# CederGroupHub/sparse-lm

Hardware: AMD Instinct MI355X
Metric: fits/sec over 50-alpha Lasso path at n=100k p=5k (higher is better)
Workload: dtype f64

## Files before the change

sparse-lm_amd/csrc/engine.hip:

```cpp
#include "engine_internal.hpp"

static thread_local std::string g_last_error;

int fail(int code, const char* fmt, ...) {
  char buf[1024];
  va_list ap;
  va_start(ap, fmt);
  vsnprintf(buf, sizeof(buf), fmt, ap);
  va_end(ap);
  g_last_error = buf;
  return code;
}

RcclApi g_rccl;

int load_rccl() {
  if (g_rccl.lib) return SLM_OK;
  const char* names[] = {"librccl.so.1", "librccl.so", "/opt/rocm/lib/librccl.so.1"};
  void* lib = nullptr;
  for (const char* nm : names) {
    lib = dlopen(nm, RTLD_NOW | RTLD_GLOBAL);
    if (lib) break;
  }
  if (!lib) return fail(SLM_ERR_COMM, "cannot load librccl: %s", dlerror());
// ... 172 lines not shown
    return fail(SLM_ERR_NO_DEVICE, "no HIP device visible (%s); this engine has no CPU fallback",
                e == hipSuccess ? "device count is 0" : hipGetErrorString(e));
  if (device_id < 0 || device_id >= n)
    return fail(SLM_ERR_BAD_ARG, "device_id %d out of range [0, %d)", device_id, n);
  HIP_TRY(hipSetDevice(device_id));
  slm_engine* eng = new slm_engine();
  eng->device = device_id;
  e = hipGetDeviceProperties(&eng->prop, device_id);
  if (e != hipSuccess) {
    delete eng;
    return fail(SLM_ERR_HIP, "hipGetDeviceProperties: %s", hipGetErrorString(e));
  }
  if (strncmp(eng->prop.gcnArchName, "gfx950", 6) != 0 && !knobs().allow_any_arch) {
    std::string arch = eng->prop.gcnArchName;
    delete eng;
    return fail(SLM_ERR_NO_DEVICE, "device %d is %s; this library only carries gfx950 (MI355X) code",
                device_id, arch.c_str());
  }
  eng->cus = eng->prop.multiProcessorCount;
  e = hipStreamCreateWithFlags(&eng->stream, hipStreamNonBlocking);
  if (e != hipSuccess) {
    delete eng;
    return fail(SLM_ERR_HIP, "hipStreamCreate: %s", hipGetErrorString(e));
  }
  *out = eng;
  return SLM_OK;
}

extern "C" int slm_comm_destroy(slm_engine* eng);

extern "C" int slm_engine_destroy(slm_engine* eng) {
  if (!eng) return SLM_OK;
  (void)hipSetDevice(eng->device);
  if (eng->sharded()) (void)slm_comm_destroy(eng);
  if (eng->comm_ev) (void)hipEventDestroy(eng->comm_ev);
  if (eng->comm_stream) (void)hipStreamDestroy(eng->comm_stream);
  if (eng->stream) (void)hipStreamDestroy(eng->stream);
  {
    std::lock_guard<std::mutex> lk(g_pool.m);
    for (void* q : g_pool.book.retire_device(eng->device)) (void)hipFree(q);
  }
  delete eng;
  return SLM_OK;
}

extern "C" int slm_engine_synchronize(slm_engine* eng) {
  if (!eng) return fail(SLM_ERR_BAD_ARG, "engine is NULL");
  HIP_TRY(hipSetDevice(eng->device));
  HIP_TRY(hipStreamSynchronize(eng->stream));
  return SLM_OK;
}

extern "C" int slm_engine_device_info(slm_engine* eng, int64_t out[6], char* name_out, int name_len) {
  if (!eng || !out) return fail(SLM_ERR_BAD_ARG, "NULL argument");
  HIP_TRY(hipSetDevice(eng->device));
  size_t free_b = 0, total_b = 0;
  HIP_TRY(hipMemGetInfo(&free_b, &total_b));
  out[0] = eng->prop.multiProcessorCount;
  out[1] = (int64_t)eng->prop.maxSharedMemoryPerMultiProcessor;
  out[2] = (int64_t)total_b;
  out[3] = (int64_t)free_b;
  out[4] = eng->prop.warpSize;
  out[5] = eng->prop.clockRate;
  if (name_out && name_len > 0) {
    snprintf(name_out, (size_t)name_len, "%s (%s)", eng->prop.name, eng->prop.gcnArchName);
  }
  return SLM_OK;
}

static void dataset_free(slm_dataset* ds) {
  if (!ds) return;
  dfree(ds->X); dfree(ds->y); dfree(ds->rw); dfree(ds->yzero); dfree(ds->rw_lanes); dfree(ds->rvec);
  dfree(ds->order); dfree(ds->gid); dfree(ds->gstart);
  dfree(ds->partial); dfree(ds->loss_partial); dfree(ds->R);
  dfree(ds->g); dfree(ds->z); dfree(ds->beta); dfree(ds->zprev); dfree(ds->gprev);
  dfree(ds->u); dfree(ds->gscale); dfree(ds->a0); dfree(ds->b0); dfree(ds->d0);
  dfree(ds->lambda); dfree(ds->dctl);
  dfree(ds->pts); dfree(ds->betas_out); dfree(ds->gn_out); dfree(ds->infos);
  dfree(ds->ws_idx); dfree(ds->ws_pos); dfree(ds->ws_gs); dfree(ds->ws_gl);
  dfree(ds->ws_score); dfree(ds->ws_XW); dfree(ds->ws_part); dfree(ds->ws_G); dfree(ds->ws_Gx); dfree(ds->XT); dfree(ds->X32s); dfree(ds->ws_owner);
  dfree(ds->ws_nt); dfree(ds->stop_words); dfree(ds->sse_Z); dfree(ds->sse_part); dfree(ds->split_state);
  dfree(ds->cons_state); dfree(ds->cons_buf);
  dfree(ds->colnorm); dfree(ds->lt_dR); dfree(ds->lt_d2); dfree(ds->lt_part); dfree(ds->lt_cols); dfree(ds->lt_stamp);
  cov_pending_drop(ds);
  ds->cov.clear();
  ds->cov_all_hold.reset();
  ds->cov_all = nullptr;
  dfree(ds->cov_Z); dfree(ds->cov_fp); dfree(ds->cov_partial);
  mg_free(ds);
  if (ds->h_split) (void)hipHostFree(ds->h_split);
  if (ds->hctl) (void)hipHostFree(ds->hctl);
  if (ds->h_small_out) (void)hipHostFree(ds->h_small_out);
  if (ds->h_vec) (void)hipHostFree(ds->h_vec);
  if (ds->h_stage) (void)hipHostFree(ds->h_stage);
  if (ds->h_pts) (void)hipHostFree(ds->h_pts);
  for (auto& e : ds->ev)
    if (e) (void)hipEventDestroy(e);
  for (auto& e : ds->prof) (void)hipEventDestroy(e);
  delete ds;
}

int set_singleton_groups(slm_dataset* ds) {
  const int p = (int)ds->p;
  std::vector<int> ident(p), start(p + 1);
  std::iota(ident.begin(), ident.end(), 0);
  std::iota(start.begin(), start.end(), 0);
  dfree(ds->order); dfree(ds->gid); dfree(ds->gstart); dfree(ds->gscale);
  SLM_TRY(dalloc(&ds->order, p));
  SLM_TRY(dalloc(&ds->gid, p));
  SLM_TRY(dalloc(&ds->gstart, p + 1));
  SLM_TRY(dalloc(&ds->gscale, (size_t)ds->lane_cap * p));
  HIP_TRY(hipMemcpy(ds->order, ident.data(), sizeof(int) * p, hipMemcpyHostToDevice));
  HIP_TRY(hipMemcpy(ds->gid, ident.data(), sizeof(int) * p, hipMemcpyHostToDevice));
  HIP_TRY(hipMemcpy(ds->gstart, start.data(), sizeof(int) * (p + 1), hipMemcpyHostToDevice));
  ds->G = p;
  ds->singleton = 1;
  ds->team = 1;
  ds->max_group = 1;
  return SLM_OK;
}

static int dataset_alloc(const slm_host::Knobs& kn, slm_engine* eng, int64_t n, int64_t p, slm_dataset** out) {
  if (n <= 0 || p <= 0) return fail(SLM_ERR_BAD_ARG, "n and p must be positive (got %lld x %lld)",
                                    (long long)n, (long long)p);
  if (p > (int64_t)TAIL_THREADS * kMaxTailE)
    return fail(SLM_ERR_UNSUPPORTED, "p = %lld exceeds the supported %d columns", (long long)p,
                TAIL_THREADS * kMaxTailE);
  if (n > (int64_t)2000000000) return fail(SLM_ERR_UNSUPPORTED, "n too large");
  slm_dataset* ds = new slm_dataset();
  ds->eng = eng;
  ds->n = n;
  ds->p = p;
  ds->n_global = n;
  ds->ld = (p + 15) / 16 * 16;
  const int64_t ld = ds->ld;
  size_t partial_elems = 0, loss_elems = 0;
  for (int B = 1; B <= kMaxLanes; ++B) {
    const GradKernel* gk = pick_grad_kernel(kn, ld / 2, B);
    ds->gk[B - 1] = gk;
    if (!gk) continue;
    int occ = 2;
    if (gk->D >= 0) {
      hipError_t e = hipOccupancyMaxActiveBlocksPerMultiprocessor(&occ, (const void*)gk->fn, gk->W * 64, 0);
      if (e != hipSuccess || occ < 1) occ = 1;
    }
    int64_t nblk = (int64_t)eng->cus * occ;
    const int64_t steps = (n + gk->R - 1) / gk->R;
    nblk = std::max<int64_t>(1, std::min<int64_t>(nblk, steps));
    ds->nblk[B - 1] = (int)nblk;
    partial_elems = std::max(partial_elems, (size_t)nblk * B * (size_t)ld);
    loss_elems = std::max(loss_elems, (size_t)nblk * B);
  }
  if (!ds->gk[0]) {
    delete ds;
    return fail(SLM_ERR_UNSUPPORTED, "no gradient kernel covers p = %lld", (long long)p);
  }
  ds->sk = pick_split_kernel(kn, ld / 2);
  if (ds->sk) {
    ds->split_nblk = (int)std::max<int64_t>(1, std::min<int64_t>(eng->cus, n));
    partial_elems = std::max(partial_elems, (size_t)xtr_max_row_blocks(eng->cus, ld) * SPLIT_LANES * (size_t)ld);
    loss_elems = std::max(loss_elems, (size_t)ds->split_nblk * SPLIT_LANES * SPLIT_HALVES);
  }

  int rc = SLM_OK;
  auto A = [&](int r) { if (rc == SLM_OK) rc = r; };
  ds->lane_cap = (p <= SM_PMAX && (double)n * (double)ld <= 131072.0) ? kMaxCells : kMaxLanes;
// ... 492 lines not shown
```

sparse-lm_amd/csrc/engine_internal.hpp:

```cpp
#pragma once
#include <hip/hip_runtime.h>

#include <dlfcn.h>
#include <stdarg.h>
#include <stdio.h>
#include <stdlib.h>
#include <string.h>

#include <algorithm>
#include <cmath>
#include <chrono>
#include <condition_variable>
#include <memory>
#include <mutex>
#include <numeric>
#include <string>
#include <vector>

#include "../../include/slm_engine.h"
#include "host_logic.hpp"
#include "data_kernels.hpp"
#include "grad_kernel.hpp"
#include "tail_kernels.hpp"
#include "ws_kernels.hpp"
#include "split_kernels.hpp"
#include "sample_kernels.hpp"
#include "light_kernels.hpp"
#include "small_kernels.hpp"
#include "small_split_kernels.hpp"
#include "small_constrained_kernels.hpp"
#include "cov_kernels.hpp"
#include "mg_kernels.hpp"

using namespace slm;


int fail(int code, const char* fmt, ...);
slm_host::Knobs knobs();

#define HIP_TRY(expr)                                                                       \
  do {                                                                                      \
    hipError_t e__ = (expr);                                                                \
    if (e__ != hipSuccess)                                                                  \
      return fail(e__ == hipErrorOutOfMemory ? SLM_ERR_OOM : SLM_ERR_HIP, "%s failed: %s (%s:%d)", \
                  #expr, hipGetErrorString(e__), __FILE__, __LINE__);                       \
  } while (0)

#define SLM_TRY(expr)            \
  do {                           \
    int rc__ = (expr);           \
    if (rc__ != SLM_OK) return rc__; \
  } while (0)

typedef struct { char internal[SLM_COMM_ID_BYTES]; } rcclUniqueId_t;
typedef void* rcclComm_t;
struct RcclApi {
  void* lib = nullptr;
  int (*GetUniqueId)(rcclUniqueId_t*) = nullptr;
  int (*CommInitRank)(rcclComm_t*, int, rcclUniqueId_t, int) = nullptr;
  int (*AllReduce)(const void*, void*, size_t, int, int, rcclComm_t, hipStream_t) = nullptr;
  int (*CommDestroy)(rcclComm_t) = nullptr;
  int (*CommCount)(rcclComm_t, int*) = nullptr;
  int (*CommUserRank)(rcclComm_t, int*) = nullptr;
  const char* (*GetErrorString)(int) = nullptr;
};
extern RcclApi g_rccl;
static const int kNcclFloat64 = 8;
static const int kNcclSum = 0;
int load_rccl();

#define RCCL_TRY(expr)                                                                      \
  do {                                                                                      \
    int e__ = (expr);                                                                       \
    if (e__ != 0)                                                                           \
      return fail(SLM_ERR_COMM, "%s failed: %s", #expr,                                     \
                  g_rccl.GetErrorString ? g_rccl.GetErrorString(e__) : "rccl error");       \
  } while (0)

struct GradKernel {
  int W, C, R, B;
  int D;
  void (*fn)(GradArgs);
  const char* name;
};
struct SplitKernel {
  int W, C, B, D;
  void (*rowdot)(SplitArgs);
  void (*resid)(SplitArgs);
  const char* rowdot_name;
};
struct GradNames {
  const char* resid = nullptr;
  const char* ws_resid = nullptr;
  const char* product = nullptr;
  int cov_rows_ws = 0;
  int cov_row_blocks = 0;
};
static const int kMaxTailE = 64;
static const int64_t kMaxChunks = 64 * 8 * 10;
const SplitKernel* pick_split_kernel(const slm_host::Knobs& kn, int64_t p2);
int xtr_max_row_blocks(int cus, int64_t ld);
int launch_xtr(const slm_host::Knobs& kn, int cus, SplitArgs& a, hipStream_t s, bool sample = false, const char** name = nullptr);
const GradKernel* pick_grad_kernel(const slm_host::Knobs& kn, int64_t p2, int B);

struct LocalComm {
  static const int kMaxRanks = 8;
  int n_ranks = 0;
  int device = 0;
  size_t cap = 0;
  double* stage[kMaxRanks] = {};
  hipEvent_t ready[kMaxRanks][2] = {};
  hipEvent_t consumed[kMaxRanks][2] = {};
  std::mutex m;
  std::condition_variable cv;
  long arrived[2] = {0, 0};
  long round_of[kMaxRanks] = {};
  int refs = 0;
  double timeout_s = 30.0;
};

struct slm_engine {
  int device = 0;
  hipStream_t stream = nullptr;
  hipDeviceProp_t prop;
  int cus = 0;
  rcclComm_t comm = nullptr;
  LocalComm* local = nullptr;
  int rank = 0, n_ranks = 1;
  long collectives = 0;
  hipStream_t comm_stream = nullptr;
  hipEvent_t comm_ev = nullptr;
  bool sharded() const { return comm != nullptr || local != nullptr; }
};

int all_reduce_sum(slm_engine* eng, double* buf, size_t count, hipStream_t s = nullptr);

static const int kMaxLanes = SLM_MAX_LANES;
static const int kMaxCells = SLM_MAX_CELLS;

struct GlobalCtl {
  int32_t done;
  int32_t lanes_done;
  int32_t hard;
  int32_t done_local;
  int32_t diverged;
  int32_t pad_[3];
};
static const int kWsMaxBuilds = 24;
static const int kWsLateIters = 12;

static const int kSnapInfos = 64;
struct DevCtl {
  GlobalCtl g;
  MgCtl mg;
  LightCtl lt;
  WsCtl ws;
  PathCtl lane[SLM_MAX_CELLS];
  slm_point_info infos[kSnapInfos];
};
struct HostCtl {
  DevCtl c;
};

void pool_free(void* p);

constexpr size_t kSmallOutDoubles = 32768;

struct slm_dataset {
  slm_engine* eng = nullptr;
  int64_t n = 0, p = 0, ld = 0, n_global = 0;
  bool replicated = false;
  int lane_cap = SLM_MAX_LANES;
  double *X = nullptr, *y = nullptr, *rw = nullptr, *yzero = nullptr;
  double rw_max = 1.0;
  double* rw_lanes = nullptr;
  double* rvec = nullptr;
  int G = 0, singleton = 1, team = 1, max_group = 1;
  std::vector<int32_t> h_gid;
  int *order = nullptr, *gid = nullptr, *gstart = nullptr;
  WsCtl* ws_ctl = nullptr;
  int32_t *ws_idx = nullptr, *ws_pos = nullptr, *ws_gs = nullptr, *ws_gl = nullptr;
  double *ws_score = nullptr, *ws_XW = nullptr, *ws_part = nullptr, *ws_G = nullptr, *ws_Gx = nullptr;
  int32_t* ws_owner = nullptr;
  double* ws_nt = nullptr;
  double *sse_Z = nullptr, *sse_part = nullptr;
  size_t sse_cap = 0;
  PathCtl* h_stage = nullptr;
  double* h_vec = nullptr;
  slm_path_point* h_pts = nullptr;
  int64_t h_pts_cap = 0;
  struct CovBlocks {
    double *G = nullptr, *c = nullptr;
    ~CovBlocks() {
      if (G) pool_free(G);
      if (c) pool_free(c);
    }
  };
  struct CovEntry {
    std::shared_ptr<CovBlocks> hold;
    double *G = nullptr, *c = nullptr;
    double yy = 0.0, n_eff = 0.0, fp1 = 0.0, fp2 = 0.0;
  };
  std::vector<CovEntry> cov;
  struct CovPending;
  CovPending* cov_pend = nullptr;
  std::shared_ptr<CovBlocks> cov_all_hold;
  double* cov_all = nullptr;
  double* cov_Z = nullptr;
  double* cov_partial = nullptr;
  int cov_partial_sets = 0;
  size_t partial_elems = 0;
  double* cov_fp = nullptr;
  double* split_state = nullptr;
  double* h_split = nullptr;
  double* cons_state = nullptr;
  double* cons_buf = nullptr;
  size_t cons_buf_doubles = 0;
  double* stop_words = nullptr;
  double* XT = nullptr;
  bool XT_ready = false, XT_failed = false;
  float* X32s = nullptr;
  int64_t rows32 = 0, ld32 = 0;
  bool x32_failed = false, x32_lossy = false;
  double* colnorm = nullptr;
  bool colnorm_ready = false;
  double *lt_dR = nullptr, *lt_d2 = nullptr, *lt_part = nullptr;
  int32_t *lt_cols = nullptr, *lt_stamp = nullptr;
  struct MgEntry {
    float* G = nullptr;
    double fp1 = 0.0, fp2 = 0.0, n_eff = 0.0;
    bool own = false;
  };
  std::vector<MgEntry> mg;
  double* mg_vec = nullptr;
  double* mg_Z = nullptr;
  bool mg_failed = false;
  double mg_build_ms = 0.0;
  int ws_sets = 0;
  const GradKernel* gk[SLM_MAX_LANES] = {};
  int nblk[SLM_MAX_LANES] = {};
  const SplitKernel* sk = nullptr;
  int split_nblk = 0;
  double* R = nullptr;
  double *partial = nullptr, *loss_partial = nullptr;
  double *g = nullptr, *z = nullptr, *beta = nullptr, *zprev = nullptr, *gprev = nullptr;
  double *u = nullptr, *gscale = nullptr, *a0 = nullptr, *b0 = nullptr, *d0 = nullptr;
  double* lambda = nullptr;
  DevCtl* dctl = nullptr;
  PathCtl* ctl = nullptr;
  GlobalCtl* gctl = nullptr;
  HostCtl* hctl = nullptr;
  double* h_small_out = nullptr;
  hipEvent_t ev[2] = {nullptr, nullptr};
  int64_t cap_points = 0, cap_gn = 0;
  slm_path_point* pts = nullptr;
  double *betas_out = nullptr, *gn_out = nullptr;
  slm_point_info* infos = nullptr;
  std::vector<hipEvent_t> prof;
  double L = 0.0;
  int L_iters = 0;
  bool L_valid = false;
  bool sketch_valid = false;
  struct CarryLane {
    int64_t n_eff = 0;
    bool has_rw = false;
    double fp[2] = {0.0, 0.0};
    double loss = 0.0;
  };
  bool carry_valid = false;
  int carry_lanes = 0;
  bool ws_carry_valid = false;
  bool ws_carry_cov = false;
  int ws_carry_sets = 0;
  int ws_carry_set_of[SLM_MAX_LANES] = {};
  CarryLane carry_lane[SLM_MAX_LANES];
  std::vector<double> carry_out;
};

static inline bool row_sharded(const slm_dataset* ds) { return ds->eng->sharded() && !ds->replicated; }

hipError_t pool_malloc(void** out, size_t bytes);

template <typename T>
static int dalloc(T** out, size_t count) {
  *out = nullptr;
  if (count == 0) count = 1;
  HIP_TRY(pool_malloc((void**)out, count * sizeof(T)));
  return SLM_OK;
}
template <typename T>
static void dfree(T*& p) {
  if (p) pool_free(p);
  p = nullptr;
}

struct LaneSetup {
  int B = 1;
  const double* rw = nullptr;
  int64_t rw_stride = 0;
  double n_eff[SLM_MAX_CELLS] = {};
};
LaneSetup default_lanes(slm_dataset* ds, int B);
int enqueue_gradient(slm_dataset* ds, const LaneSetup& ls, const double* y, const int* done, hipEvent_t ev_start, hipEvent_t ev_stop,
                     int64_t n_rows = 0, const int* skip = nullptr, GradNames* names = nullptr);
int enqueue_gradient_split(const slm_host::Knobs& kn, slm_dataset* ds, const LaneSetup& ls, const double* y, const int* done, const PathCtl* ctl, const WsArgs* wa,
                           hipEvent_t ev_start, hipEvent_t ev_stop, int64_t n_rows = 0, bool unit_bracket = false, const int* skip = nullptr,
                           GradNames* names = nullptr);
bool split_usable(const slm_host::Knobs& kn, slm_dataset* ds);
int ensure_xt(const slm_host::Knobs& kn, slm_dataset* ds);
int ensure_x32s(slm_dataset* ds, int64_t n_rows, bool* usable);
void x32_drop(slm_dataset* ds);
int enqueue_sample_f32(slm_dataset* ds, int64_t n_rows, double n_eff, int n_lanes, const int* done, bool* queued);
int check_launch();
void launch_rowdot(const slm_host::Knobs& kn, slm_dataset* ds, const SplitKernel* sk, int nblk, int B, SplitArgs& a, hipStream_t s,
                  const char** name = nullptr);
int enqueue_gradient_cov(slm_dataset* ds, int B, const int* entry_of, const int* done, hipEvent_t ev_start, hipEvent_t ev_stop,
                         const PathCtl* ctl = nullptr, const WsArgs* wa = nullptr, GradNames* names = nullptr);
void launch_tail(const TailArgs& ta, hipStream_t s);
int64_t sketch_rows(int64_t n);
int power_iteration(const slm_host::Knobs& kn, slm_dataset* ds, const LaneSetup& ls_in, double* L_out , int iters, int64_t n_rows = 0);
int estimate_lipschitz(const slm_host::Knobs& kn, slm_dataset* ds, double* L_out, int iters);
int allow_big_lds(const void* fn, int device);
static const int kProfStride = 3;
static const int kPowerItersSolve = 2;
int cov_fingerprints(slm_dataset* ds, const double* const* w, int count, double* out );
int cov_find(const slm_dataset* ds, double fp1, double fp2, double n_eff);
void cov_pending_drop(slm_dataset* ds);
int set_singleton_groups(slm_dataset* ds);
static const int kMgEntries = 8;
bool mg_possible(const slm_host::Knobs& kn, const slm_dataset* ds);
int mg_ensure(const slm_host::Knobs& kn, slm_dataset* ds, const double* w, double n_eff, bool own, double fp1, double fp2, int* entry_out);
void mg_invalidate(slm_dataset* ds);
void mg_free(slm_dataset* ds);
int mg_enqueue_round(slm_dataset* ds, const TailArgs& ta, int n_lanes, int inner_iters, const int* done, int n_sets, const int* entry_of_set,
                     const int* set_of);
```

sparse-lm_amd/csrc/engine_path.hip:

```cpp
#include "engine_internal.hpp"
#include "ws_solve_kernels.hpp"

static int ws_policy(const slm_host::Knobs& kn, const slm_dataset* ds, uint32_t flags) {
  if (ds->max_group > WS_KCAP / 2 || ds->n < 4) return 0;
  if (kn.ws == 0 || (flags & SLM_FLAG_NO_WORKING_SET)) return 0;
  const bool big = (double)ds->n * (double)ds->ld >= 67108864.0;
  return (big || (flags & SLM_FLAG_WORKING_SET) || kn.ws == 1) ? 2 : 1;
}

static bool small_ok(const slm_host::Knobs& kn, const slm_dataset* ds, uint32_t flags) {
  if (!(flags & SLM_FLAG_ON_CHIP)) return false;
  if (flags & (SLM_FLAG_NO_RESTART | SLM_FLAG_PROFILE | SLM_FLAG_FISTA_ONLY | SLM_FLAG_WORKING_SET | SLM_FLAG_NO_WORKING_SET))
    return false;
  if (!kn.on_chip) return false;
  return ds->p <= SM_PMAX && (double)ds->n * (double)ds->ld <= 131072.0 && !row_sharded(ds);
}
static bool split_possible(const slm_dataset* ds) {
  return ds->sk != nullptr && (ds->sk->rowdot != nullptr || !ds->XT_failed);
}
static int max_lanes_for(const slm_host::Knobs& kn, const slm_dataset* ds, uint32_t flags) {
  if (small_ok(kn, ds, flags)) return ds->lane_cap;
  if ((ws_policy(kn, ds, flags) == 2 || (double)ds->n * (double)ds->ld >= 67108864.0) && split_possible(ds)) {
    if (ws_policy(kn, ds, flags) == 2 && !row_sharded(ds) && ds->sk->rowdot != nullptr && !ds->XT_failed)
      return kMaxLanes;
// ... 8 lines not shown
  if (want <= SPLIT_LANES || small_ok(kn, ds, flags)) return SLM_OK;
  HIP_TRY(hipSetDevice(ds->eng->device));
  SLM_TRY(ensure_xt(kn, ds));
  if (ds->XT == nullptr) *lanes_out = SPLIT_LANES;
  return SLM_OK;
}

static int solve_core(const slm_host::Knobs& kn, slm_dataset* ds, const slm_lane* lanes, int32_t n_lanes, const slm_solve_opts* opts,
                      slm_solve_stats* stats, bool shared_path, const slm_reweight* rules = nullptr, int32_t* rounds_out = nullptr);

static int solve_without_chip(const slm_host::Knobs& kn, slm_dataset* ds, const slm_lane* lanes, int32_t B, const slm_solve_opts& o, slm_solve_stats* stats,
                              bool shared_path) {
  slm_solve_opts again = o;
  again.flags &= ~SLM_FLAG_ON_CHIP;
  const int per_call = shared_path ? B : std::min<int>(B, max_lanes_for(kn, ds, again.flags));
  if (per_call >= B) return solve_core(kn, ds, lanes, B, &again, stats, shared_path);
  slm_solve_stats sum, part;
  memset(&sum, 0, sizeof(sum));
  for (int l0 = 0; l0 < B; l0 += per_call) {
    SLM_TRY(solve_core(kn, ds, lanes + l0, std::min(per_call, B - l0), &again, &part, false));
    sum.grad_launches += part.grad_launches;
    sum.wall_ms += part.wall_ms;
    sum.lipschitz_ms += part.lipschitz_ms;
    sum.ws_builds += part.ws_builds; sum.ws_appends += part.ws_appends; sum.ws_refined += part.ws_refined;
    sum.ws_misses += part.ws_misses; sum.ws_columns = std::max(sum.ws_columns, part.ws_columns);
    sum.ws_inner_iters += part.ws_inner_iters; sum.ws_direct_steps += part.ws_direct_steps;
  }
  if (stats) *stats = sum;
  return SLM_OK;
}

struct PathCall {
  explicit PathCall(const slm_host::Knobs& k) : kn(k) {}
  const slm_host::Knobs kn;
  slm_dataset* ds = nullptr;
  const slm_lane* lanes = nullptr;
  int B = 0;
  slm_solve_opts o;
  slm_solve_stats* stats = nullptr;
  bool shared_path = false;
  const slm_reweight* rules = nullptr;
  int32_t* rounds_out = nullptr;
  slm_engine* eng = nullptr;
  hipStream_t s = nullptr;
  int64_t n = 0, p = 0, ld = 0;
  int G = 0;
  bool big_x = false, split = false, want_cov = false, interleave = false, sharded = false, small = false, profile = false;
  int64_t total_points = 0;
  bool any_rw = false, any_gn = false, custom_scale = false;
  std::chrono::steady_clock::time_point t_begin;
  double tr[6] = {0, 0, 0, 0, 0, 0}, tr_rw = 0.0;
  double t_mark() const { return std::chrono::duration<double, std::milli>(std::chrono::steady_clock::now() - t_begin).count(); }
  LaneSetup ls;
  double wmax[SLM_MAX_CELLS];
  double rw_fp[SLM_MAX_CELLS][2];
  int cov_entry[SLM_MAX_CELLS];
  bool cov_on = false;
  double L[SLM_MAX_CELLS], L_factor[SLM_MAX_CELLS];
  double lipschitz_ms = 0.0;
  bool L_on_device = false;
  bool L_kept = false;
  bool carry = false, ws_carry = false;
  bool ws_begun = false;
  int ws_set_of[SLM_MAX_LANES], ws_set_lane[SLM_MAX_LANES], ws_n_sets = 0;
  PathCtl* h = nullptr;
  bool infos_in_snap = false;
  slm_point_info* d_infos = nullptr;
  TailArgs ta;
  bool use_ws = false, ws_late = false;
  WsArgs wa;
  const int* done_flag = nullptr;
  int ws_comm_rc = 0;
  bool mg_handover = false;
  bool fix_start = false;
  bool sample_f32 = false;
  int chunk = 0;
  int64_t max_total = 0, enq = 0, expected = 0, n_sample = 0, prof_off = 0;
  int64_t planned_end = 0;
  int slot = 0, final_slot = 0;
  bool pending[2] = {false, false};
  bool done = false, results_queued = false, results_final = false, deferred = false, trace3 = false;
  bool light_begun = false;
  const int* light_skip = nullptr;
  std::vector<char> prof_rec;
  bool mg_forced = false, mg_ok = false, mg_on = false;
  int mg_cap = 0, mg_inner = 20, mg_built = 0;
  double mg_build_ms = 0.0;
  int mg_entry_of_set[SLM_MAX_LANES];

  int run();
  int shape(const slm_solve_opts* opts);
  int stage_row_weights();
  int find_covariance();
  int kept_sketch();
  int seed_lipschitz();
  int stage_lanes();
  int enqueue_result_copies();
  int run_on_chip();
  int ws_setup(bool late);
  void ws_release();
  int prepare_working_set();
  int enqueue_pass_gradient(hipEvent_t e0, hipEvent_t e1);
  void enqueue_tail();
  void enqueue_refinement();
  void plan_queue();
  int mg_sets();
  bool mg_wanted(const DevCtl& c) const;
  int mg_consider(const DevCtl& c);
  void trace_pass(const DevCtl& now) const;
  bool light_eligible();
  int enqueue_light_attempt();
  int queue_chunk();
  int pass_loop();
  int finish();
  void report(const DevCtl& snap, int64_t passes);
};

static int solve_core(const slm_host::Knobs& kn, slm_dataset* ds, const slm_lane* lanes, int32_t n_lanes, const slm_solve_opts* opts,
                      slm_solve_stats* stats, bool shared_path, const slm_reweight* rules, int32_t* rounds_out) {
  if (!ds || !lanes) return fail(SLM_ERR_BAD_ARG, "NULL argument");
  HIP_TRY(hipSetDevice(ds->eng->device));
  std::unique_ptr<PathCall> c(new PathCall(kn));
  c->ds = ds; c->lanes = lanes; c->B = n_lanes; c->stats = stats; c->shared_path = shared_path; c->rules = rules; c->rounds_out = rounds_out;
  memset(&c->o, 0, sizeof(c->o));
  if (opts) c->o = *opts;
  memset(c->cov_entry, 0, sizeof(c->cov_entry));
  memset(c->rw_fp, 0, sizeof(c->rw_fp));
  memset(c->ws_set_of, 0, sizeof(c->ws_set_of));
  memset(c->ws_set_lane, 0, sizeof(c->ws_set_lane));
  memset(c->mg_entry_of_set, 0, sizeof(c->mg_entry_of_set));
  memset(&c->wa, 0, sizeof(c->wa));
  SLM_TRY(c->shape(opts));
  struct DrainOnExit {
    hipStream_t s;
    ~DrainOnExit() { (void)hipStreamSynchronize(s); }
  } drain_on_exit{c->s};
  return c->run();
}

int PathCall::run() {
  SLM_TRY(stage_row_weights());
  SLM_TRY(find_covariance());
  SLM_TRY(seed_lipschitz());
  SLM_TRY(stage_lanes());
  if (small) return run_on_chip();
  SLM_TRY(prepare_working_set());
  plan_queue();
  if (n_sample > 0 && !kn.sample_f64) SLM_TRY(ensure_x32s(ds, n_sample, &sample_f32));
  SLM_TRY(pass_loop());
  return finish();
}

int PathCall::shape(const slm_solve_opts* opts) {
  if (rules) {
    if (!rounds_out) return fail(SLM_ERR_BAD_ARG, "rounds_out is NULL");
    if (shared_path || !small_ok(kn, ds, opts ? opts->flags : 0u))
      return fail(SLM_ERR_UNSUPPORTED, "re-weighted rounds need a problem the on-chip solver takes (p <= %d, n * ld <= 131072)", SM_PMAX);
    for (int l = 0; l < B && l < SLM_MAX_CELLS; ++l) {
      const slm_reweight& r = rules[l];
      if (!(r.eps >= 0.0) || !(r.tol >= 0.0) || !std::isfinite(r.coef_scale) || !std::isfinite(r.numerator) || !std::isfinite(r.eps) ||
          r.n_coef < 0 || r.n_coef > ds->p || r.n_group < 0 || r.n_group > ds->G)
        return fail(SLM_ERR_BAD_ARG, "lane %d: bad re-weighting rule", l);
      if (r.group_scale)
        for (int g = 0; g < r.n_group; ++g)
          if (!(r.group_scale[g] >= 0.0) || !std::isfinite(r.group_scale[g]))
            return fail(SLM_ERR_BAD_ARG, "lane %d: group_scale[%d] is negative or not finite", l, g);
    }
  }
  {
    const int cap = small_ok(kn, ds, opts ? opts->flags : 0u) ? ds->lane_cap : kMaxLanes;
    if (B < 1 || B > cap) return fail(SLM_ERR_BAD_ARG, "n_lanes must be in [1, %d] (got %d)", cap, B);
  }
  big_x = (double)ds->n * (double)ds->ld >= 67108864.0;
  const bool wide = ds->sk != nullptr && ds->sk->rowdot == nullptr;
  const GradKernel* gk_B = B <= kMaxLanes ? ds->gk[B - 1] : nullptr;
  const bool two_pass_only = gk_B != nullptr && gk_B->D < 0;
  const bool want_split = (ws_policy(kn, ds, opts ? opts->flags : 0u) == 2 && (!wide || two_pass_only)) ? (big_x || !gk_B) : (big_x && !gk_B);
  want_cov = opts && (opts->flags & SLM_FLAG_COVARIANCE) && !ds->cov.empty() && !row_sharded(ds) && B <= kMaxLanes;
  split = (want_split || want_cov) && split_usable(kn, ds);
  interleave = shared_path && ds->singleton && ws_policy(kn, ds, opts ? opts->flags : 0u) == 2 &&
                          kn.interleave;
  if (!split && !gk_B && !small_ok(kn, ds, opts ? opts->flags : 0u))
    return fail(SLM_ERR_UNSUPPORTED, "no %d-lane gradient kernel covers p = %lld", B, (long long)ds->p);
  if (B > SPLIT_LANES && !small_ok(kn, ds, opts ? opts->flags : 0u) && (!split || row_sharded(ds) || ws_policy(kn, ds, opts ? opts->flags : 0u) != 2))
    return fail(SLM_ERR_UNSUPPORTED, "%d lanes: more than %d need a working-set solve on the split pass of an unsharded dataset", B, SPLIT_LANES);
  if (split && B > ROWDOT_LANES) SLM_TRY(ensure_xt(kn, ds));
  for (int l = 0; l < B; ++l) {
    const slm_lane& ln = lanes[l];
    if (!ln.points || !ln.betas_out) return fail(SLM_ERR_BAD_ARG, "lane %d: NULL points or betas_out", l);
    if (ln.n_points <= 0) return fail(SLM_ERR_BAD_ARG, "lane %d: n_points must be positive", l);
    for (int k = 0; k < ln.n_points; ++k) {
      const slm_path_point& q = ln.points[k];
      if (!(q.sa >= 0.0) || !(q.sb >= 0.0) || !(q.sd >= 0.0) || !std::isfinite(q.sa + q.sb + q.sd))
        return fail(SLM_ERR_BAD_ARG, "path point %d has a negative or non-finite scale", k);
      if (!std::isfinite(q.extrap) || std::fabs(q.extrap) > 1e3)
        return fail(SLM_ERR_BAD_ARG, "path point %d has an unreasonable extrapolation factor", k);
    }
    total_points += ln.n_points;
    any_rw = any_rw || ln.row_weight != nullptr;
    any_gn = any_gn || ln.group_norms_out != nullptr;
  }
  eng = ds->eng;
  sharded = row_sharded(ds);
  HIP_TRY(hipSetDevice(eng->device));
  s = eng->stream;
  t_begin = std::chrono::steady_clock::now();
  p = ds->p; ld = ds->ld; n = ds->n;
  G = ds->G;
  if (!(o.tol > 0.0)) o.tol = 1e-8;
  if (o.max_iter <= 0) o.max_iter = 10000;
  profile = (o.flags & SLM_FLAG_PROFILE) != 0;

  return SLM_OK;
}

int PathCall::stage_row_weights() {
  ls = default_lanes(ds, B);
  for (int l = 0; l < kMaxCells; ++l) wmax[l] = ds->rw ? ds->rw_max : 1.0;
  if (any_rw) {
    if (!ds->rw_lanes) SLM_TRY(dalloc(&ds->rw_lanes, (size_t)ds->lane_cap * n));
    for (int l = 0; l < B; ++l) {
      double* dst = ds->rw_lanes + (size_t)l * n;
      if (lanes[l].row_weight) {
        const double* w = lanes[l].row_weight;
        int same = -1;
        for (int m = 0; m < l && same < 0; ++m)
          if (lanes[m].row_weight == w) same = m;
        if (same >= 0) {
          wmax[l] = wmax[same];
          rw_fp[l][0] = rw_fp[same][0];
// ... 485 lines not shown
    ds->ws_sets = n_sets;
  }
  return ensure_xt(kn, ds);
}

static int ws_bind(const slm_host::Knobs& kn, slm_dataset* ds, const LaneSetup& ls, const int* set_of, const int* set_lane, int n_sets,
                   int nblk, bool sharded, WsArgs& wa, hipStream_t s) {
  const int B = ls.B;
  wa.ws = ds->ws_ctl;
  wa.idx = ds->ws_idx; wa.pos = ds->ws_pos; wa.gs = ds->ws_gs; wa.gl = ds->ws_gl;
  wa.score = ds->ws_score; wa.XW = ds->ws_XW; wa.part = ds->ws_part; wa.Gm = ds->ws_G;
  wa.nt = ds->ws_nt;
  if (sharded && !ds->ws_Gx) SLM_TRY(dalloc(&ds->ws_Gx, (size_t)ds->ws_sets * WS_KCAP * WS_KCAP + STOP_WORDS));
  wa.Gx = sharded ? ds->ws_Gx : nullptr;
  wa.X = ds->X; wa.XT = ds->XT; wa.n = ds->n; wa.ld = ds->ld;
  wa.rw = ls.rw; wa.rw_stride = ls.rw_stride;
  for (int l = 0; l < kMaxLanes; ++l) {
    wa.set_of[l] = l < B ? set_of[l] : 0;
    wa.set_lane[l] = l < n_sets ? set_lane[l] : 0;
    const int rep = wa.set_lane[l];
    wa.inv_n[l] = 1.0 / (ls.n_eff[rep] > 0 ? ls.n_eff[rep] : (double)ds->n_global);
  }
  wa.n_sets = n_sets;
  wa.nblk = nblk;
  wa.owner = nullptr;
  if (ls.rw != nullptr && !sharded && kn.gram_owner && nblk <= 512) {
    if (!ds->ws_owner) SLM_TRY(dalloc(&ds->ws_owner, (size_t)kMaxLanes * 512));
    hipLaunchKernelGGL(ws_block_owner_kernel, dim3((unsigned)nblk), dim3(256), 0, s, ls.rw, ls.rw_stride, wa, ds->ws_owner);
    wa.owner = ds->ws_owner;
  }
  return SLM_OK;
}

int PathCall::ws_setup(bool late) {
  const int n_sets = ws_n_sets;
  const WsBlocks wb = ws_row_blocks(ds, ls.rw != nullptr && !sharded && n_sets > 1, n_sets);
  SLM_TRY(ws_alloc(kn, ds, n_sets, wb.most, sharded));
  if (late) HIP_TRY(hipMemsetAsync(ds->ws_ctl, 0, sizeof(WsCtl), s));
  if (ws_carry && !late) hipLaunchKernelGGL(ws_ctl_carry_kernel, dim3(1), dim3(256), 0, s, ds->ws_ctl, kWsMaxBuilds);
  else if (late || !ws_begun) hipLaunchKernelGGL(ws_ctl_init_kernel, dim3(1), dim3(64), 0, s, ds->ws_ctl, kWsMaxBuilds);
  SLM_TRY(ws_bind(kn, ds, ls, ws_set_of, ws_set_lane, n_sets, wb.nblk, sharded, wa, s));
  wa.theta = kn.ws_theta;
  wa.lookahead = slm_host::kWsLookahead;
  wa.append_max = kn.ws_append;
  wa.k_init = kn.ws_kinit > 0 ? kn.ws_kinit : (ds->singleton ? (shared_path ? 112 : 256) : 384);
  wa.bb_steps = kn.ws_bb;
  wa.one_solver = kn.ws_one_solver;
  wa.hard_call = kn.hard_callwide;
  wa.power_iters = slm_host::kWsPowerIters;
  wa.miss_factor = kn.ws_miss_factor;
  wa.miss_div = kn.ws_miss_div;
  wa.fill = kn.ws_fill > 0.0 ? kn.ws_fill : ((ds->singleton && shared_path) ? 0.75 : 0.5);
  return SLM_OK;
}

void PathCall::ws_release() {
  ds->ws_carry_valid = false;
  dfree(ds->ws_idx); dfree(ds->ws_pos); dfree(ds->ws_gs); dfree(ds->ws_gl);
  dfree(ds->ws_score); dfree(ds->ws_XW); dfree(ds->ws_part); dfree(ds->ws_G); dfree(ds->ws_Gx); dfree(ds->ws_nt);
  ds->ws_sets = 0;
  (void)hipGetLastError();
}

int PathCall::prepare_working_set() {
  {
    const int pol = ws_policy(kn, ds, o.flags);
    use_ws = pol == 2;
    ws_late = pol == 1 && !sharded;
  }
  if (sharded && !ds->stop_words) SLM_TRY(dalloc(&ds->stop_words, STOP_WORDS));
  if (use_ws) {
    const int rc = ws_setup(false);
    if (rc == SLM_ERR_OOM && !split && !sharded) {
      ws_release();
      use_ws = false;
    } else if (rc != SLM_OK) {
      return rc;
    }
  }
  done_flag = &ds->gctl->done;
  return SLM_OK;
}

int PathCall::enqueue_pass_gradient(hipEvent_t e0, hipEvent_t e1) {
  if (cov_on) return enqueue_gradient_cov(ds, B, cov_entry, done_flag, e0, e1, ds->ctl, use_ws ? &wa : nullptr);
  if (split) return enqueue_gradient_split(kn, ds, ls, ds->y, done_flag, ds->ctl, &wa, e0, e1, 0, (o.flags & SLM_FLAG_PROFILE_UNIT) != 0, light_skip);
  return enqueue_gradient(ds, ls, ds->y, done_flag, e0, e1, 0, light_skip);
}

void PathCall::enqueue_tail() {
  launch_tail(ta, s);
  if (shared_path && !interleave) hipLaunchKernelGGL(steal_kernel, dim3(1), dim3(256), 0, s, ta);
  if (shared_path && interleave && mg_handover) hipLaunchKernelGGL(tail_handover_kernel, dim3(1), dim3(64), 0, s, ta);
  else if (shared_path && interleave && use_ws && !ws_late && !sharded && planned_end > 0 && kn.lag_handover)
    hipLaunchKernelGGL(lag_handover_kernel, dim3(1), dim3(64), 0, s, ta, &ds->ws_ctl->builds, &ds->ws_ctl->stale, (int)(planned_end - enq - 1));
  if (sharded) {
    if (use_ws && wa.Gx) {
      hipLaunchKernelGGL(stop_pack_kernel, dim3(1), dim3(64), 0, s, ta.gdone, ds->ctl, B,
                         wa.Gx + (size_t)wa.n_sets * WS_KCAP * WS_KCAP);
    } else {
      hipLaunchKernelGGL(stop_pack_kernel, dim3(1), dim3(64), 0, s, ta.gdone, ds->ctl, B, ds->stop_words);
      if (ws_comm_rc == 0) ws_comm_rc = all_reduce_sum(eng, ds->stop_words, STOP_WORDS);
      hipLaunchKernelGGL(stop_apply_kernel, dim3(1), dim3(64), 0, s, ta.gdone, ds->stop_words);
    }
  }
}

struct WsNames {
  const char* k[8];
  int n = 0;
  void add(const char* name) { if (n < 8) k[n++] = name; }
};
static void ws_enqueue_build(slm_dataset* ds, const WsArgs& wa, const CovSets* cs, bool xty, const int* done, int n_lanes, hipStream_t s,
                             WsNames* names = nullptr) {
  const int64_t n = ds->n;
  if (cs) {
    hipLaunchKernelGGL(ws_gram_cov_kernel, dim3(WS_TILES * WS_TILES, (unsigned)wa.n_sets), dim3(256), 0, s, wa, *cs);
    if (names) names->add("ws_gram_cov_kernel");
    return;
  }
  hipLaunchKernelGGL(ws_gather_kernel, dim3((unsigned)std::min<int64_t>((n + 31) / 32, 1024), WS_KCAP / 32), dim3(256), 0, s, wa);
  if (names) names->add("ws_gather_kernel");
  if (xty) {
    XtyArgs xa;
    xa.ws = wa.ws; xa.idx = wa.idx; xa.XW = wa.XW; xa.y = ds->y; xa.part = wa.part; xa.g = ds->g; xa.gprev = ds->gprev; xa.z = ds->z;
    xa.ctl = ds->ctl; xa.done = done; xa.n = n; xa.ld = ds->ld; xa.inv_n = 1.0 / (double)ds->n_global; xa.n_lanes = n_lanes;
    xa.nblk = (int)std::max<int64_t>(1, std::min<int64_t>(2 * ds->eng->cus, n / 64));
    hipLaunchKernelGGL(ws_xty_partial_kernel, dim3((unsigned)xa.nblk), dim3(512), 0, s, xa);
    hipLaunchKernelGGL(ws_xty_apply_kernel, dim3(WS_KCAP / 128), dim3(512), 0, s, xa);
    if (names) { names->add("ws_xty_partial_kernel"); names->add("ws_xty_apply_kernel"); }
  }
  hipLaunchKernelGGL(ws_gram_kernel, dim3((unsigned)wa.nblk, (unsigned)wa.n_sets, 1), dim3(WS_GRAM_THREADS), 0, s,
                     wa);
  if (wa.Gx)
    (void)hipMemsetAsync(wa.Gx, 0, sizeof(double) * (size_t)wa.n_sets * WS_KCAP * WS_KCAP, s);
  hipLaunchKernelGGL(ws_gram_reduce_kernel, dim3(WS_TILES * WS_TILES, (unsigned)wa.n_sets), dim3(256),
                     0, s, wa);
  if (names) { names->add("ws_gram_kernel"); names->add("ws_gram_reduce_kernel"); }
}

static void ws_enqueue_solvers(const slm_dataset* ds, const TailArgs& ta, const WsArgs& wa, int B, hipStream_t s, WsNames* names = nullptr) {
  if (wa.one_solver && wa.nt) {
  } else if (ds->singleton) {
    hipLaunchKernelGGL((ws_solve_kernel<false, 0>), dim3(B), dim3(WS_THREADS), 0, s, ta, wa);
    if (names) names->add("ws_solve_kernel<false,0>");
  } else {
    hipLaunchKernelGGL((ws_solve_kernel<true, 0>), dim3(B), dim3(WS_THREADS), 0, s, ta, wa);
    if (names) names->add("ws_solve_kernel<true,0>");
  }
  if (wa.nt) {
    if (ds->singleton) hipLaunchKernelGGL((ws_solve_kernel<false, 1>), dim3(B), dim3(WS_THREADS), 0, s, ta, wa);
    else hipLaunchKernelGGL((ws_solve_kernel<true, 1>), dim3(B), dim3(WS_THREADS), 0, s, ta, wa);
    if (names) names->add(ds->singleton ? "ws_solve_kernel<false,1>" : "ws_solve_kernel<true,1>");
  }
}

void PathCall::enqueue_refinement() {
  if (use_ws) {
    {
      const int bs = ds->singleton ? 256 : 64;
      const int64_t items = ds->singleton ? p : 16 * (int64_t)G;
      hipLaunchKernelGGL(ws_score_kernel, dim3((unsigned)((items + bs - 1) / bs)), dim3(bs), 0, s, ta, wa);
      hipLaunchKernelGGL(ws_select_kernel, dim3(1), dim3(WS_THREADS), 0, s, ta, wa);
    }
    if (cov_on) {
      CovSets cs;
      for (int st = 0; st < kMaxLanes; ++st) cs.G[st] = st < wa.n_sets ? ds->cov[(size_t)cov_entry[wa.set_lane[st]]].G : nullptr;
      ws_enqueue_build(ds, wa, &cs, false, done_flag, B, s);
    } else {
      ws_enqueue_build(ds, wa, nullptr, fix_start, done_flag, B, s);
    }
    if (wa.Gx) {
      const size_t gram_words = (size_t)wa.n_sets * WS_KCAP * WS_KCAP;
      if (ws_comm_rc == 0) ws_comm_rc = all_reduce_sum(eng, wa.Gx, gram_words + STOP_WORDS);
      hipLaunchKernelGGL(ws_publish_kernel, dim3(WS_PUBLISH_BLOCKS, (unsigned)wa.n_sets), dim3(256), 0, s, wa);
      hipLaunchKernelGGL(stop_apply_kernel, dim3(1), dim3(64), 0, s, ta.gdone, wa.Gx + gram_words);
    }
    ws_enqueue_solvers(ds, ta, wa, B, s);
  }
}

void PathCall::plan_queue() {
  chunk = o.check_every;
  if (chunk <= 0) {
    const double est_us = std::max(12.0, (double)n * (double)ld * 8.0 / 5.0e6);
    chunk = est_us > 150.0 ? 2 : 4;
  }
  if (use_ws) chunk = std::min(chunk, 8);
  int max_points = 0;
  for (int l = 0; l < B; ++l) max_points = std::max(max_points, (int)lanes[l].n_points);
  if (shared_path) max_points = (int)total_points;
  max_total = (int64_t)max_points * o.max_iter;

  tr[2] = t_mark();
  if (use_ws && !ws_late && o.check_every <= 0) {
    int64_t most = 0;
    for (int l = 0; l < B; ++l) {
      int64_t mine = lanes[l].n_points;
      if (shared_path && interleave) mine = slm_host::interleaved_points(slm_host::LaneWalk{h[l].pt_lo, h[l].n_points, h[l].stride, h[l].tail_pt});
      most = std::max<int64_t>(most, mine);
    }
    expected = 1 + most;
    planned_end = expected;
  }
  {
    bool cold = true;
    for (int l = 0; l < B; ++l) cold = cold && lanes[l].beta0 == nullptr;
    if (cold && shared_path && use_ws && !ws_late && !sharded && !cov_on && split && !any_rw && !ds->rw &&
        !custom_scale && expected > 0 && o.max_iter >= 4 && !(o.flags & SLM_FLAG_FISTA_ONLY) && kn.sample_start) {
      const int64_t least = kn.sample_min_rows;
      if (n >= least) n_sample = n / kn.sample_div;
    }
  }
  mg_forced = kn.mg == 2;
  mg_cap = slm_host::model_gram_cap(ld, 3.0e9, kMgEntries);
  mg_ok = use_ws && split && (big_x || mg_forced) && !sharded && !cov_on && !(o.flags & SLM_FLAG_NO_MODEL_GRAM) &&
                     (size_t)ds->lane_cap >= (size_t)kMaxLanes && ws_n_sets <= mg_cap && mg_possible(kn, ds);
  if (mg_ok && mg_forced) expected = 0;
  if (mg_ok && !mg_forced && !ds->mg.empty()) {
    bool all = ws_n_sets > 0;
    for (int st = 0; st < ws_n_sets && all; ++st) {
      const int l = ws_set_lane[st];
      all = lanes[l].row_weight == nullptr;
      const double ne = ls.n_eff[l] > 0 ? ls.n_eff[l] : (double)ds->n_global;
      bool have = false;
      for (const auto& e : ds->mg) have = have || (e.own && e.n_eff == ne);
      all = all && have;
    }
    if (all) wa.keep_full = 1;
  }
  prof_off = n_sample > 0 ? 1 : 0;
  trace3 = kn.trace == 3;
  if (trace3 && kn.trace_poll && expected > 0) expected = n_sample > 0 ? 2 : 1;
}

int PathCall::mg_sets() {
  const double* wdev[SLM_MAX_LANES];
  double fp[2 * SLM_MAX_LANES] = {};
  int n_fp = 0, fp_at[SLM_MAX_LANES];
  for (int st = 0; st < ws_n_sets; ++st) {
    const int l = ws_set_lane[st];
    fp_at[st] = -1;
    if (lanes[l].row_weight != nullptr) {
      fp_at[st] = n_fp;
      wdev[n_fp++] = ls.rw + (int64_t)l * ls.rw_stride;
    }
  }
  if (n_fp > 0) SLM_TRY(cov_fingerprints(ds, wdev, n_fp, fp));
  int missing = 0;
  for (int pass = 0; pass < 2; ++pass) {
    if (pass == 1 && (int)ds->mg.size() + missing > mg_cap) mg_invalidate(ds);
    if (pass == 1) mg_built += missing;
    for (int st = 0; st < ws_n_sets; ++st) {
      const int l = ws_set_lane[st];
      const bool own = lanes[l].row_weight == nullptr;
      const double ne = ls.n_eff[l] > 0 ? ls.n_eff[l] : (double)ds->n_global;
      const double f1 = own ? 0.0 : fp[2 * fp_at[st]], f2 = own ? 0.0 : fp[2 * fp_at[st] + 1];
      if (pass == 0) {
        bool have = false;
        for (const auto& e : ds->mg) have = have || (e.n_eff == ne && (own ? e.own : (!e.own && e.fp1 == f1 && e.fp2 == f2)));
        missing += have ? 0 : 1;
      } else {
        SLM_TRY(mg_ensure(kn, ds, own ? nullptr : ls.rw + (int64_t)l * ls.rw_stride, ne, own, f1, f2, &mg_entry_of_set[st]));
      }
    }
  }
  return SLM_OK;
}

bool PathCall::mg_wanted(const DevCtl& c) const {
  if (mg_forced) return true;
  return c.ws.outgrown > 0 || c.ws.overflows > 0 || c.ws.disabled != 0;
}

int PathCall::mg_consider(const DevCtl& c) {
  if (!mg_ok || mg_on || !mg_wanted(c)) return SLM_OK;
  const auto t0 = std::chrono::steady_clock::now();
  const int rc = mg_sets();
  if (rc == SLM_OK) {
    mg_on = true;
    mg_handover = kn.handover;
    wa.keep_full = 1;
    if (mg_built > 0) mg_build_ms += std::chrono::duration<double, std::milli>(std::chrono::steady_clock::now() - t0).count();
  } else if (rc != SLM_ERR_OOM) {
    return rc;
  }
  return SLM_OK;
}

void PathCall::trace_pass(const DevCtl& now) const {
  if (!trace3) return;
  fprintf(stderr, "[slm] pass %lld at %.3f ms: K %d builds %d appends %d misses %d stale %d refined %d | mg on %d rounds %d inner %d most %d rej %d | light %d of %d (last: %d columns, why %d, D %.3g) | lanes (point.iter/flags):",
          (long long)enq, t_mark(), now.ws.Kreal, now.ws.builds, now.ws.appends, now.ws.misses, now.ws.stale, now.ws.refined, (int)mg_on,
          now.mg.rounds, now.mg.inner_iters, now.mg.most_iters, now.mg.rejected, now.lt.used, now.lt.attempts, now.lt.n_cols, now.lt.why, now.lt.D[0]);
  for (int l = 0; l < B; ++l)
    fprintf(stderr, " %d.%d%s%s%s", now.lane[l].point, now.lane[l].iter, now.lane[l].done ? "d" : "", now.lane[l].zsup ? "w" : "",
            l < SLM_MAX_LANES && now.mg.lane[l].active ? "m" : "");
  fprintf(stderr, " | lt id %d ok %d | lanes (rejects/epoch/slack):", now.lt.id, now.lt.ok);
  for (int l = 0; l < B && l < SLM_MAX_LANES; ++l) fprintf(stderr, " %d/%d/%.3g", now.lane[l].rejects, now.lt.epoch[l], now.lt.slack[l]);
  fprintf(stderr, "\n");
}

bool PathCall::light_eligible() {
  if (!kn.light_pass || !shared_path || !use_ws || ws_late || cov_on || sharded || mg_on) return false;
  if (any_rw || ds->rw || custom_scale || B > kMaxLanes || !(expected > 0 && enq >= expected)) return false;
  return ds->XT != nullptr && ds->XT_ready && ds->colnorm != nullptr && ds->colnorm_ready;
}

int PathCall::enqueue_light_attempt() {
  const int nblk = (int)std::max<int64_t>(std::max<int64_t>(1, std::min<int64_t>(eng->cus, n)), (n + 959) / 960);
  if (!ds->lt_dR) SLM_TRY(dalloc(&ds->lt_dR, (size_t)n * LT_LANES));
  if (!ds->lt_d2) SLM_TRY(dalloc(&ds->lt_d2, (size_t)nblk * (LT_LANES + kMaxLanes)));
  if (!ds->lt_part) SLM_TRY(dalloc(&ds->lt_part, (size_t)nblk * LT_CAP * LT_LANES));
  if (!ds->lt_cols) SLM_TRY(dalloc(&ds->lt_cols, (size_t)LT_CAP));
  if (!ds->lt_stamp) SLM_TRY(dalloc(&ds->lt_stamp, (size_t)ld));
  if (!light_begun) {
    HIP_TRY(hipMemsetAsync(ds->lt_stamp, 0, sizeof(int32_t) * (size_t)ld, s));
    light_begun = true;
  }
  LightArgs la;
  memset(&la, 0, sizeof(la));
  la.lt = &ds->dctl->lt; la.ctl = ds->ctl; la.done = done_flag; la.pts = ds->pts; la.ws = wa.ws; la.idx = wa.idx; la.pos = wa.pos;
  la.XW = wa.XW; la.XT = ds->XT; la.Gm = wa.Gm; la.y = ds->y; la.colnorm = ds->colnorm;
  la.z = ds->z; la.zprev = ds->zprev; la.gprev = ds->gprev; la.a0 = ds->a0; la.b0 = ds->b0; la.g = ds->g;
  la.loss_partial = ds->lt_d2 + (size_t)nblk * LT_LANES; la.dR = ds->lt_dR; la.d2_part = ds->lt_d2; la.cols = ds->lt_cols; la.stamp = ds->lt_stamp; la.part = ds->lt_part;
  la.n = n; la.ld = ld; la.rows_base = n / nblk; la.rows_rem = n % nblk;
  la.p = (int)p; la.n_lanes = B; la.slots = SPLIT_LANES * ((B + SPLIT_LANES - 1) / SPLIT_LANES); la.nblk = nblk;
  la.inv_n = 1.0 / (double)ds->n_global;
  la.order = ds->order; la.gstart = ds->gstart; la.G = G; la.singleton = ds->singleton;
  hipLaunchKernelGGL(light_prepare_kernel, dim3(1), dim3(1024), 0, s, la);
  hipLaunchKernelGGL(light_resid_kernel, dim3((unsigned)nblk), dim3(LT_WAVES * 64), 0, s, la);
  hipLaunchKernelGGL(light_select_kernel, dim3(1), dim3(1024), 0, s, la);
  const size_t lds = sizeof(double) * (size_t)(la.rows_base + 1) * LT_LANES;
  hipLaunchKernelGGL(light_coldot_kernel, dim3((unsigned)nblk), dim3(256), lds, s, la);
  hipLaunchKernelGGL(light_assemble_kernel, dim3(LT_LANES), dim3(1024), 0, s, la);
  return SLM_OK;
}

int PathCall::queue_chunk() {
  const int this_chunk = mg_on ? 1 : (expected <= 0 ? chunk : (enq < expected ? (int)std::min<int64_t>(64, expected - enq) : 1));
  for (int i = 0; i < this_chunk; ++i) {
    hipEvent_t e0 = nullptr, e1 = nullptr;
    const bool light = light_eligible();
    if (profile && !light && enq >= prof_off && (enq - prof_off) % kProfStride == 0) {
      const int64_t slot_id = (enq - prof_off) / kProfStride;
      while ((int64_t)ds->prof.size() < 2 * (slot_id + 1)) {
        hipEvent_t ev;
        HIP_TRY(hipEventCreate(&ev));
        ds->prof.push_back(ev);
      }
      e0 = ds->prof[2 * slot_id];
      e1 = ds->prof[2 * slot_id + 1];
      if ((int64_t)prof_rec.size() <= slot_id) prof_rec.resize((size_t)slot_id + 1, 0);
      prof_rec[(size_t)slot_id] = 1;
    }
    if (light) SLM_TRY(enqueue_light_attempt());
    light_skip = light ? &ds->dctl->lt.ok : nullptr;
    ta.light = light ? 1 : 0;
    const bool sample_pass = n_sample > 0 && enq == 0;
    if (sample_pass) {
      LaneSetup part = ls;
      for (int l = 0; l < kMaxLanes; ++l) part.n_eff[l] = (double)ds->n_global * (double)n_sample / (double)n;
      bool on_image = false;
      if (sample_f32) SLM_TRY(enqueue_sample_f32(ds, n_sample, part.n_eff[0], B, done_flag, &on_image));
      if (!on_image) SLM_TRY(enqueue_gradient_split(kn, ds, part, ds->y, done_flag, ds->ctl, &wa, nullptr, nullptr, n_sample));
      TailArgs first = ta;
      first.provisional = 1;
      launch_tail(first, s);
    } else {
      if (!(carry && enq == 0)) SLM_TRY(enqueue_pass_gradient(e0, e1));
      enqueue_tail();
    }
    fix_start = sample_pass;
    ++enq;
    deferred = (expected > 0 && enq >= expected && enq < expected + 4 && !sharded) || mg_on;
    if (!deferred) enqueue_refinement();
    fix_start = false;
  }
  SLM_TRY(check_launch());
  if (ws_comm_rc != 0) return ws_comm_rc;
  HIP_TRY(hipMemcpyAsync(&ds->hctl[slot].c, ds->dctl, sizeof(DevCtl), hipMemcpyDeviceToHost, s));
  return SLM_OK;
}

int PathCall::pass_loop() {
  while (!done) {
    SLM_TRY(queue_chunk());
    const bool at_end = mg_on || (expected > 0 && enq >= expected && (enq < expected + 4 || (trace3 && kn.trace_poll)));
    HIP_TRY(hipEventRecord(ds->ev[slot], s));
    if (expected > 0 && enq == expected && !results_queued) {
      SLM_TRY(enqueue_result_copies());
      results_queued = true;
    }
    pending[slot] = true;
    const int other = slot ^ 1;
    if (at_end) {
      if (pending[other]) HIP_TRY(hipEventSynchronize(ds->ev[other]));
      const auto t_spin = std::chrono::steady_clock::now();
      for (;;) {
        const hipError_t q = hipEventQuery(ds->ev[slot]);
        if (q == hipSuccess) break;
        if (q != hipErrorNotReady) HIP_TRY(q);
        if (std::chrono::steady_clock::now() - t_spin > std::chrono::milliseconds(20)) {
          HIP_TRY(hipEventSynchronize(ds->ev[slot]));
          break;
        }
      }
      pending[slot] = pending[other] = false;
      if (ds->hctl[slot].c.g.done) {
        done = true;
        final_slot = slot;
        results_final = results_queued && enq == expected;
      } else {
        const DevCtl& now = ds->hctl[slot].c;
        trace_pass(now);
        SLM_TRY(mg_consider(now));
        if (deferred) {
          bool ws_serves = !(mg_on && now.ws.stale != 0 && wa.keep_full != 0);
          for (int l = 0; l < B && !ws_serves; ++l) ws_serves = !now.lane[l].done && !now.lane[l].idle && now.lane[l].zsup != 0;
          if (ws_serves) enqueue_refinement();
          deferred = false;
        }
        if (mg_on) {
          if (now.mg.rounds > 0) mg_inner = now.mg.most_iters >= mg_inner ? std::min(96, 2 * mg_inner) : std::max(6, std::min(96, (int)now.mg.most_iters + 2));
          SLM_TRY(mg_enqueue_round(ds, ta, B, mg_inner, done_flag, ws_n_sets, mg_entry_of_set, ws_set_of));
        }
      }
    } else if (pending[other]) {
      HIP_TRY(hipEventSynchronize(ds->ev[other]));
      pending[other] = false;
      if (ds->hctl[other].c.g.done) {
        done = true;
        final_slot = other;
      }
      if (!done) SLM_TRY(mg_consider(ds->hctl[other].c));
      if (!done && ws_late && ds->hctl[other].c.g.hard >= kWsLateIters) {
        const int rc = ws_setup(true);
        ws_late = false;
        if (rc == SLM_OK) {
          use_ws = true;
          chunk = std::min(chunk, 8);
        } else if (rc == SLM_ERR_OOM) {
          ws_release();
        } else {
          return rc;
        }
      }
    }
    slot = other;
    if (!done && enq >= max_total + 2 * (int64_t)chunk) {
      HIP_TRY(hipStreamSynchronize(s));
      return fail(SLM_ERR_HIP, "internal error: path state machine did not terminate");
    }
  }
  return SLM_OK;
}

int PathCall::finish() {
  if (!results_final) SLM_TRY(enqueue_result_copies());
  HIP_TRY(hipStreamSynchronize(s));
  tr[3] = t_mark();
  const DevCtl& snap = ds->hctl[final_slot].c;
  if (sharded && snap.g.diverged)
    return fail(SLM_ERR_COMM, "row-sharded solve aborted: the ranks' solver states differ (different arguments on "
                "different ranks, or an all-reduce that is not bit-identical on every rank)");
  const PathCtl* fin = snap.lane;
  if (infos_in_snap) {
    int64_t at = 0;
    for (int l = 0; l < B; ++l) {
      if (lanes[l].infos) memcpy(lanes[l].infos, snap.infos + at, sizeof(slm_point_info) * (size_t)lanes[l].n_points);
      at += lanes[l].n_points;
    }
  }
  int64_t passes = 0;
  bool nonfinite = false;
  for (int l = 0; l < B; ++l) {
    passes = std::max<int64_t>(passes, fin[l].total_iter);
    nonfinite = nonfinite || fin[l].nonfinite;
  }
  if (stats) {
    stats->grad_launches = passes - (carry ? 1 : 0) - prof_off - snap.lt.used;
    stats->light_passes = snap.lt.used;
    stats->light_columns = snap.lt.cols_total;
    stats->grad_ms_total = 0.0;
    stats->grad_timed = 0;
    if (profile) {
      double tot = 0.0;
      int64_t cnt = 0;
      for (int64_t k = 0; k * kProfStride < passes - prof_off && 2 * k + 1 < (int64_t)ds->prof.size(); ++k) {
        if (k >= (int64_t)prof_rec.size() || !prof_rec[(size_t)k]) continue;
        float ms = 0.f;
        if (hipEventElapsedTime(&ms, ds->prof[2 * k], ds->prof[2 * k + 1]) == hipSuccess) {
          tot += ms;
          ++cnt;
        }
      }
      stats->grad_ms_total = tot;
      stats->grad_timed = cnt;
    }
    stats->lipschitz_ms = lipschitz_ms;
    stats->ws_builds = stats->ws_appends = stats->ws_refined = stats->ws_misses = stats->ws_columns = 0;
    stats->ws_inner_iters = stats->ws_direct_steps = 0;
    stats->mg_rounds = snap.mg.rounds;
    stats->mg_inner_iters = snap.mg.inner_iters;
    stats->mg_rejected = snap.mg.rejected;
    stats->mg_build_ms = mg_build_ms;
    if (use_ws) {
      const WsCtl& wc = snap.ws;
      stats->ws_builds = wc.builds;
      stats->ws_appends = wc.appends;
      stats->ws_refined = wc.refined;
      stats->ws_misses = wc.misses;
      stats->ws_columns = wc.Kreal;
      stats->ws_inner_iters = wc.inner_iters;
      stats->ws_direct_steps = wc.newton_steps;
      if (kn.trace == 2) {
        fprintf(stderr, "[slm] working set: %d model-solver iterations over %d refinements, %d direct steps (%d refused, %d of them not positive definite), K = %d, lambda_max bound of the first Gram %.4g (seed L %.4g)\n",
                wc.inner_iters, wc.refined, wc.newton_steps, wc.newton_fails, wc.newton_nopd, wc.K, wc.Lw[0], fin[0].L);
        fprintf(stderr, "[slm] model solver, lane 0, ms over the solve: set-up %.3f, lambda_max of a new Gram %.3f, start value %.3f, "
                "iteration %.3f, acceptance + write-back %.3f\n", wc.solve_ticks[0] * 1e-5, wc.solve_ticks[1] * 1e-5,
                wc.solve_ticks[2] * 1e-5, wc.solve_ticks[3] * 1e-5, wc.solve_ticks[4] * 1e-5);
        fprintf(stderr, "[slm] model solves by iterations:");
        for (int i = 0; i < 32; ++i)
          if (wc.iters_hist[i]) fprintf(stderr, " %d:%d", i, wc.iters_hist[i]);
        fprintf(stderr, "\n");
        fprintf(stderr, "[slm] model solver, ms per lane over the solve:");
        for (int l = 0; l < B; ++l) fprintf(stderr, " %.3f", wc.lane_ticks[l] * 1e-5);
        fprintf(stderr, "\n");
        if (wc.newton_factors) {
          fprintf(stderr, "[slm] direct steps: accepted at t = 1: %d, 1/2: %d, 1/4: %d, first sign change: %d; %d factorisations, %.0f unknowns on average\n",
                  wc.newton_trial[0], wc.newton_trial[1], wc.newton_trial[2], wc.newton_trial[3], wc.newton_factors,
                  (double)wc.newton_unknowns / wc.newton_factors);
          fprintf(stderr, "[slm] direct steps without a usable segment: t = 0: %d, slope <= 0: %d, curvature <= 0: %d; no decrease on it: %d\n",
                  wc.newton_ref[0], wc.newton_ref[1], wc.newton_ref[2], wc.newton_ref[3]);
          int worst = 0;
          double worst_ms = -1.0;
          for (int l = 0; l < B; ++l) {
            double t = 0.0;
            for (int k = 0; k < 6; ++k) t += wc.nt_ticks[l][k] * 1e-5;
            if (t > worst_ms) {
              worst_ms = t;
              worst = l;
            }
          }
          const unsigned long long* tk = wc.nt_ticks[worst];
// ... 40 lines not shown
  return SLM_OK;
}

extern "C" int slm_solve_lanes(slm_dataset* ds, const slm_lane* lanes, int32_t n_lanes,
                               const slm_solve_opts* opts, slm_solve_stats* stats) {
  return solve_core(knobs(), ds, lanes, n_lanes, opts, stats, false);
}

extern "C" int slm_solve_lanes_reweighted(slm_dataset* ds, const slm_lane* lanes, const slm_reweight* rules, int32_t n_lanes,
                                          const slm_solve_opts* opts, slm_solve_stats* stats, int32_t* rounds_out) {
  if (!rules) return fail(SLM_ERR_BAD_ARG, "rules is NULL");
  return solve_core(knobs(), ds, lanes, n_lanes, opts, stats, false, rules, rounds_out);
}

static int auto_lanes(const slm_host::Knobs& kn, const slm_dataset* ds, int32_t n_points, uint32_t fl) {
  const int cap = max_lanes_for(kn, ds, fl);
  const bool big = ws_policy(kn, ds, fl) == 2 && (double)ds->n * (double)ds->ld >= 67108864.0 && !small_ok(kn, ds, fl);
  const bool interleaved = ds->singleton && kn.interleave;
  int B = slm_host::auto_path_lanes(n_points, cap, big, !interleaved);
  if (kn.auto_lanes > 0) B = std::max(1, std::min<int>(std::min(kn.auto_lanes, cap), n_points));
  return B;
}
extern "C" int slm_dataset_path_lanes(slm_dataset* ds, int32_t n_points, uint32_t flags, int32_t* lanes_out) {
  if (!ds || !lanes_out) return fail(SLM_ERR_BAD_ARG, "NULL argument");
  if (n_points <= 0) return fail(SLM_ERR_BAD_ARG, "n_points must be positive");
  *lanes_out = auto_lanes(knobs(), ds, n_points, flags);
  return SLM_OK;
}

extern "C" int slm_solve_path_lanes(slm_dataset* ds, const slm_penalty* pen, const slm_path_point* points,
                                    int32_t n_points, int32_t n_lanes, const slm_solve_opts* opts,
                                    const double* beta0, double* betas_out, double* group_norms_out,
                                    slm_point_info* infos, slm_solve_stats* stats) {
  if (!ds || !points || !betas_out) return fail(SLM_ERR_BAD_ARG, "NULL argument");
  if (n_points <= 0) return fail(SLM_ERR_BAD_ARG, "n_points must be positive");
  const uint32_t fl = opts ? opts->flags : 0u;
  const slm_host::Knobs kn = knobs();
  int B;
  if (n_lanes == 0) {
    B = auto_lanes(kn, ds, n_points, fl);
  } else {
    B = std::max(1, std::min<int>(std::min<int>(n_lanes, kMaxLanes), n_points));
    B = std::min(B, max_lanes_for(kn, ds, fl));
  }
  SLM_TRY(lanes_with_copy(kn, ds, fl, B, &B));
  slm_lane lanes[SLM_MAX_LANES];
  memset(lanes, 0, sizeof(lanes));
  int64_t lo = 0;
  for (int l = 0; l < B; ++l) {
    const int64_t hi = (int64_t)n_points * (l + 1) / B;
    lanes[l].pen = pen;
    lanes[l].points = points + lo;
    lanes[l].n_points = (int32_t)(hi - lo);
    lanes[l].beta0 = (l == 0) ? beta0 : nullptr;
    lanes[l].betas_out = betas_out + lo * ds->p;
    lanes[l].group_norms_out = group_norms_out ? group_norms_out + lo * ds->G : nullptr;
    lanes[l].infos = infos ? infos + lo : nullptr;
    lo = hi;
  }
  return solve_core(kn, ds, lanes, B, opts, stats, B > 1);
}

extern "C" int slm_solve_path(slm_dataset* ds, const slm_penalty* pen, const slm_path_point* points,
                              int32_t n_points, const slm_solve_opts* opts, const double* beta0,
                              double* betas_out, double* group_norms_out, slm_point_info* infos,
                              slm_solve_stats* stats) {
  if (!ds || !points || !betas_out) return fail(SLM_ERR_BAD_ARG, "NULL argument");
  slm_lane lane;
  memset(&lane, 0, sizeof(lane));
  lane.pen = pen;
  lane.points = points;
  lane.n_points = n_points;
  lane.beta0 = beta0;
  lane.betas_out = betas_out;
  lane.group_norms_out = group_norms_out;
  lane.infos = infos;
  return slm_solve_lanes(ds, &lane, 1, opts, stats);
}

extern "C" int slm_working_set_lanes(slm_dataset* ds, const slm_ws_lanes_opts* o, double* G_out, double* loss_out, int32_t* set_of_out,
                                     int32_t* n_sets_out, double* gram_out, double* xw_out, double* xty_out, char* kernels_out,
                                     int32_t kernels_len) {
  if (!ds || !o || !o->Z || !o->cols || !o->k_end || !G_out) return fail(SLM_ERR_BAD_ARG, "NULL argument");
  const int route = o->route, B = o->n_lanes, nb = o->n_builds;
  const bool gather_x = (o->flags & SLM_WSL_GATHER_X) != 0, xty = (o->flags & SLM_WSL_XTY) != 0;
  if (route != 1 && route != 2) return fail(SLM_ERR_BAD_ARG, "route must be 1 (split pass) or 2 (covariance), got %d", route);
  if (B < 1 || B > kMaxLanes) return fail(SLM_ERR_BAD_ARG, "between 1 and %d lanes, got %d", kMaxLanes, B);
  if (o->flags & ~(SLM_WSL_GATHER_X | SLM_WSL_XTY)) return fail(SLM_ERR_BAD_ARG, "unknown flags %#x", o->flags);
  if (xty != (xty_out != nullptr)) return fail(SLM_ERR_BAD_ARG, "xty_out goes with SLM_WSL_XTY");
  if (row_sharded(ds)) return fail(SLM_ERR_UNSUPPORTED, "slm_working_set_lanes: row-sharded datasets");
  if (B > ds->lane_cap) return fail(SLM_ERR_UNSUPPORTED, "%d lanes: the dataset holds %d", B, ds->lane_cap);
  const int64_t n = ds->n, p = ds->p, ld = ds->ld;
  if (nb < 1) return fail(SLM_ERR_BAD_ARG, "at least one build");
  for (int b = 0; b < nb; ++b)
    if (o->k_end[b] <= (b > 0 ? o->k_end[b - 1] : 0) || o->k_end[b] > WS_KCAP)
      return fail(SLM_ERR_BAD_ARG, "k_end must increase from above 0 to at most %d (build %d: %d)", WS_KCAP, b, o->k_end[b]);
  const int kreal = o->k_end[nb - 1];
  const int K = std::max(16, (kreal + 15) & ~15);
  std::vector<int32_t> pos((size_t)ld, -1);
  for (int k = 0; k < kreal; ++k) {
    const int32_t j = o->cols[k];
    if (j < 0 || j >= p) return fail(SLM_ERR_BAD_ARG, "cols[%d] = %d outside [0, %lld)", k, j, (long long)p);
    if (pos[(size_t)j] >= 0) return fail(SLM_ERR_BAD_ARG, "cols[%d] = %d repeats cols[%d]", k, j, pos[(size_t)j]);
    pos[(size_t)j] = k;
  }
  std::vector<int32_t> zzero((size_t)B, 1);
  for (int l = 0; l < B; ++l)
    for (int64_t j = 0; j < p; ++j) {
      const double v = o->Z[(size_t)l * p + j];
      if (!std::isfinite(v)) return fail(SLM_ERR_BAD_ARG, "Z contains a non-finite value");
      if (v != 0.0) {
        zzero[(size_t)l] = 0;
        if (o->on_ws && o->on_ws[l] && pos[(size_t)j] < 0)
          return fail(SLM_ERR_BAD_ARG, "lane %d is marked on the working set but Z[%d][%lld] != 0 is outside it", l, l, (long long)j);
      }
    }
  if (o->row_weights)
    for (int64_t k = 0; k < (int64_t)B * n; ++k)
      if (!(o->row_weights[k] >= 0.0) || !std::isfinite(o->row_weights[k]))
        return fail(SLM_ERR_BAD_ARG, "row_weights[%lld] is negative or not finite", (long long)k);
  if (o->n_eff)
    for (int l = 0; l < B; ++l)
      if (!(o->n_eff[l] > 0.0) || !std::isfinite(o->n_eff[l])) return fail(SLM_ERR_BAD_ARG, "n_eff[%d] must be positive and finite", l);
  if (route == 2) {
    if (o->row_weights || o->n_eff) return fail(SLM_ERR_UNSUPPORTED, "route 2 takes its rows from the covariance entries: no row_weights or n_eff");
    if (gather_x || xty || xw_out) return fail(SLM_ERR_UNSUPPORTED, "route 2 gathers no columns: no XW, no X_W^T y");
    if (ds->cov.empty()) return fail(SLM_ERR_UNSUPPORTED, "route 2: the dataset has no covariance entries");
    if (!o->cov_index) return fail(SLM_ERR_BAD_ARG, "route 2 needs cov_index");
    for (int l = 0; l < B; ++l)
      if (o->cov_index[l] < 0 || o->cov_index[l] >= (int32_t)ds->cov.size())
        return fail(SLM_ERR_BAD_ARG, "cov_index[%d] = %d: the dataset has %d entries", l, o->cov_index[l], (int)ds->cov.size());
  }
  const slm_host::Knobs kn = knobs();
  HIP_TRY(hipSetDevice(ds->eng->device));
  hipStream_t s = ds->eng->stream;
  if (route == 1) {
    if (!ds->sk) return fail(SLM_ERR_UNSUPPORTED, "route 1: no split pass for p = %lld", (long long)p);
    SLM_TRY(ensure_xt(kn, ds));
    if (!split_usable(kn, ds) || (B > SPLIT_LANES && !(ds->XT && ds->XT_ready)))
      return fail(SLM_ERR_UNSUPPORTED, "route 1: no residual kernel for %d lanes at p = %lld without the column-major copy", B, (long long)p);
    if (!gather_x && !(ds->XT && ds->XT_ready)) return fail(SLM_ERR_UNSUPPORTED, "no column-major copy of X to gather from");
  }
  auto put = [&](void* dst, const void* src, size_t bytes) -> int {
    HIP_TRY(hipMemcpyAsync(dst, src, bytes, hipMemcpyHostToDevice, s));
    HIP_TRY(hipStreamSynchronize(s));
    return SLM_OK;
  };
  auto get = [&](void* dst, const void* src, size_t bytes) -> int {
    HIP_TRY(hipMemcpyAsync(dst, src, bytes, hipMemcpyDeviceToHost, s));
    HIP_TRY(hipStreamSynchronize(s));
    return SLM_OK;
  };
  LaneSetup ls = default_lanes(ds, B);
  if (o->row_weights) {
    if (!ds->rw_lanes) SLM_TRY(dalloc(&ds->rw_lanes, (size_t)ds->lane_cap * n));
    SLM_TRY(put(ds->rw_lanes, o->row_weights, sizeof(double) * (size_t)B * n));
    ls.rw = ds->rw_lanes;
    ls.rw_stride = n;
  }
  if (o->n_eff)
    for (int l = 0; l < B; ++l) ls.n_eff[l] = o->n_eff[l];
  int set_of[kMaxLanes], set_lane[kMaxLanes], n_sets = 0;
  for (int l = 0; l < B; ++l) {
    int found = -1;
    for (int m = 0; m < l && found < 0; ++m) {
      const bool same = route == 2 ? o->cov_index[m] == o->cov_index[l]
                                   : ls.n_eff[m] == ls.n_eff[l] &&
                                         (!o->row_weights || memcmp(o->row_weights + (size_t)m * n, o->row_weights + (size_t)l * n,
                                                                    sizeof(double) * (size_t)n) == 0);
// ... 6 lines not shown
    set_of[l] = found;
  }
  const WsBlocks wb = ws_row_blocks(ds, ls.rw != nullptr && n_sets > 1, n_sets);
  SLM_TRY(ws_alloc(kn, ds, n_sets, wb.most, false));
  WsArgs wa;
  memset(&wa, 0, sizeof(wa));
  SLM_TRY(ws_bind(kn, ds, ls, set_of, set_lane, n_sets, wb.nblk, false, wa, s));
  if (gather_x) wa.XT = nullptr;
  std::string names;
  auto named = [&](const char* k) {
    if (!names.empty()) names += ';';
    names += k;
  };
  if (wa.owner) named("ws_block_owner_kernel");
  CovSets cs;
  memset(&cs, 0, sizeof(cs));
  if (route == 2)
    for (int st = 0; st < n_sets; ++st) cs.G[st] = ds->cov[(size_t)o->cov_index[set_lane[st]]].G;
  HIP_TRY(hipMemsetAsync(ds->ws_XW, 0xff, sizeof(double) * (size_t)n * WS_KCAP, s));
  HIP_TRY(hipMemsetAsync(ds->ws_G, 0xff, sizeof(double) * (size_t)n_sets * WS_KCAP * WS_KCAP, s));
  HIP_TRY(hipMemsetAsync(ds->g, 0xff, sizeof(double) * (size_t)(ld + 16) * B, s));
  HIP_TRY(hipMemsetAsync(&ds->gctl->done, 0, sizeof(int32_t), s));
  WsCtl* h = new WsCtl;
  std::unique_ptr<WsCtl> h_hold(h);
  memset(h, 0, sizeof(WsCtl));
  h->request = 1;
  h->max_builds = kWsMaxBuilds;
  for (int l = 0; l < SLM_MAX_LANES; ++l) h->last_point[l] = -1;
  std::vector<int32_t> h_idx(WS_KCAP), h_gs(WS_KCAP), h_gl(WS_KCAP, 1), h_pos((size_t)ld, -1);
  for (int k = 0; k < WS_KCAP; ++k) h_gs[(size_t)k] = k;
  for (int b = 0; b < nb; ++b) {
    const int k_old = b > 0 ? o->k_end[b - 1] : 0, kr = o->k_end[b];
    for (int k = 0; k < WS_KCAP; ++k) h_idx[(size_t)k] = k < kr ? o->cols[k] : -1;
    for (int k = k_old; k < kr; ++k) h_pos[(size_t)o->cols[k]] = k;
    h->Kreal = kr;
    h->K = std::max(16, (kr + 15) & ~15);
    h->k_new = k_old;
    h->building = 1;
    h->valid = 0;
    h->stale = 0;
    h->counter = 0;
    if (b > 0) h->appends += 1;
    else h->builds += 1;
    SLM_TRY(put(ds->ws_idx, h_idx.data(), sizeof(int32_t) * WS_KCAP));
    SLM_TRY(put(ds->ws_gs, h_gs.data(), sizeof(int32_t) * WS_KCAP));
    SLM_TRY(put(ds->ws_gl, h_gl.data(), sizeof(int32_t) * WS_KCAP));
    SLM_TRY(put(ds->ws_pos, h_pos.data(), sizeof(int32_t) * (size_t)ld));
    SLM_TRY(put(ds->ws_ctl, h, sizeof(WsCtl)));
    WsNames wn;
    ws_enqueue_build(ds, wa, route == 2 ? &cs : nullptr, xty, &ds->gctl->done, B, s, &wn);
    for (int u = 0; u < wn.n; ++u) named(wn.k[u]);
    SLM_TRY(check_launch());
    SLM_TRY(get(h, ds->ws_ctl, sizeof(WsCtl)));
    if (h->valid != 1 || h->building != 0 || h->counter != 0)
      return fail(SLM_ERR_HIP, "build %d: the Gram was not published (valid %d, building %d, counter %d)", b, h->valid, h->building,
                  h->counter);
  }
  if (gram_out)
    for (int st = 0; st < n_sets; ++st)
      HIP_TRY(hipMemcpy2DAsync(gram_out + (size_t)st * K * K, sizeof(double) * K, ds->ws_G + (size_t)st * WS_KCAP * WS_KCAP,
                               sizeof(double) * WS_KCAP, sizeof(double) * K, K, hipMemcpyDeviceToHost, s));
  if (xw_out)
    HIP_TRY(hipMemcpy2DAsync(xw_out, sizeof(double) * K, ds->ws_XW, sizeof(double) * WS_KCAP, sizeof(double) * K, n,
                             hipMemcpyDeviceToHost, s));
  if (xty) {
    std::vector<double> g0((size_t)ld + 16);
    SLM_TRY(get(g0.data(), ds->g, sizeof(double) * (size_t)(ld + 16)));
    for (int k = 0; k < kreal; ++k) xty_out[k] = g0[(size_t)o->cols[k]];
    xty_out[kreal] = g0[(size_t)ld];
  }
  HIP_TRY(hipStreamSynchronize(s));
  std::vector<PathCtl> hc((size_t)B);
  memset(hc.data(), 0, sizeof(PathCtl) * (size_t)B);
  for (int l = 0; l < B; ++l) {
    hc[(size_t)l].zsup = (o->on_ws && o->on_ws[l]) ? 1 : 0;
    hc[(size_t)l].zzero = zzero[(size_t)l];
    hc[(size_t)l].tail_pt = -1;
  }
  SLM_TRY(put(ds->ctl, hc.data(), sizeof(PathCtl) * (size_t)B));
  const int slots = SPLIT_LANES * ((B + SPLIT_LANES - 1) / SPLIT_LANES);
  HIP_TRY(hipMemsetAsync(ds->z, 0, sizeof(double) * (size_t)slots * ld, s));
  HIP_TRY(hipMemcpy2DAsync(ds->z, sizeof(double) * ld, o->Z, sizeof(double) * p, sizeof(double) * p, B, hipMemcpyHostToDevice, s));
  GradNames gn;
  if (route == 1) {
    SLM_TRY(enqueue_gradient_split(kn, ds, ls, ds->y, nullptr, ds->ctl, &wa, nullptr, nullptr, 0, false, nullptr, &gn));
  } else {
    if (!ds->cov_Z) SLM_TRY(dalloc(&ds->cov_Z, (size_t)ld * SPLIT_RSTRIDE * SPLIT_HALVES));
    SLM_TRY(enqueue_gradient_cov(ds, B, o->cov_index, nullptr, nullptr, nullptr, ds->ctl, &wa, &gn));
  }
  SLM_TRY(check_launch());
  HIP_TRY(hipStreamSynchronize(s));
  const size_t lane_bytes = sizeof(double) * (size_t)(ld + 16);
  HIP_TRY(hipMemcpy2D(G_out, sizeof(double) * p, ds->g, lane_bytes, sizeof(double) * p, B, hipMemcpyDeviceToHost));
  if (loss_out) HIP_TRY(hipMemcpy2D(loss_out, sizeof(double), ds->g + ld, lane_bytes, sizeof(double), B, hipMemcpyDeviceToHost));
  if (set_of_out)
    for (int l = 0; l < B; ++l) set_of_out[l] = set_of[l];
  if (n_sets_out) *n_sets_out = n_sets;
  if (route == 1) {
    if (gn.resid) named(gn.resid);
    if (gn.ws_resid) named(gn.ws_resid);
    if (gn.product) named(gn.product);
  } else if (gn.product) {
    bool listed = gn.cov_rows_ws > 0 && (int64_t)gn.cov_rows_ws * gn.cov_row_blocks >= K;
    for (int l = 0; l < B; ++l) listed = listed && o->on_ws && o->on_ws[l];
    named(gn.product);
    if (listed) names += "+listed";
  }
  if (kernels_out && kernels_len > 0) snprintf(kernels_out, (size_t)kernels_len, "%s", names.c_str());
  return SLM_OK;
}

extern "C" int slm_working_set_model_solve(slm_dataset* ds, const slm_ws_model_opts* o, slm_ws_model_out* out) {
  if (!ds || !o || !out) return fail(SLM_ERR_BAD_ARG, "NULL argument");
  if (!o->cols || !o->gram || !o->zprev || !o->gprev || !o->z || !o->a0 || !o->b0 || !o->d0 || !o->points || !o->tol || !o->mode)
    return fail(SLM_ERR_BAD_ARG, "NULL input");
  if (!out->z || !out->beta || !out->served || !out->mu || !out->zsup || !out->t || !out->have_base || !out->zzero ||
      !out->want_full || !out->repeats || !out->hard_lane || !out->last_point || !out->Lw || !out->counters)
    return fail(SLM_ERR_BAD_ARG, "NULL output");
  const uint32_t known = SLM_WMS_DIRECT | SLM_WMS_HARD | SLM_WMS_INVALID | SLM_WMS_BUILDING | SLM_WMS_DISABLED | SLM_WMS_STALE |
                         SLM_WMS_NONFINITE;
  if (o->flags & ~known) return fail(SLM_ERR_BAD_ARG, "unknown flags %#x", o->flags);
  const int B = o->n_lanes, kreal = o->kreal, n_sets = o->n_sets;
  if (B < 1 || B > kMaxLanes) return fail(SLM_ERR_BAD_ARG, "between 1 and %d lanes, got %d", kMaxLanes, B);
  if (kreal < 1 || kreal > WS_KCAP) return fail(SLM_ERR_BAD_ARG, "between 1 and %d columns, got %d", WS_KCAP, kreal);
  if (n_sets < 1 || n_sets > B) return fail(SLM_ERR_BAD_ARG, "between 1 and n_lanes Grams, got %d", n_sets);
  if (row_sharded(ds)) return fail(SLM_ERR_UNSUPPORTED, "slm_working_set_model_solve: row-sharded datasets");
  if (B > ds->lane_cap) return fail(SLM_ERR_UNSUPPORTED, "%d lanes: the dataset holds %d", B, ds->lane_cap);
  const int64_t p = ds->p, ld = ds->ld;
  const int G = ds->singleton ? (int)p : ds->G;
  const int K = std::max(16, (kreal + 15) & ~15);
  const bool loose = (o->flags & SLM_WMS_NONFINITE) != 0;
  std::vector<int32_t> h_pos((size_t)ld, -1), h_idx(WS_KCAP, -1), h_gs(WS_KCAP), h_gl(WS_KCAP, 1);
  for (int k = 0; k < WS_KCAP; ++k) h_gs[(size_t)k] = k;
  for (int k = 0; k < kreal; ++k) {
    const int32_t j = o->cols[k];
    if (j < 0 || j >= p) return fail(SLM_ERR_BAD_ARG, "cols[%d] = %d outside [0, %lld)", k, j, (long long)p);
    if (h_pos[(size_t)j] >= 0) return fail(SLM_ERR_BAD_ARG, "cols[%d] = %d repeats cols[%d]", k, j, h_pos[(size_t)j]);
    h_pos[(size_t)j] = k;
    h_idx[(size_t)k] = j;
  }
  if (!ds->singleton) {
    std::vector<int> size((size_t)G, 0);
    for (int64_t j = 0; j < p; ++j) size[(size_t)ds->h_gid[(size_t)j]] += 1;
    for (int k = 0; k < kreal;) {
      const int g = ds->h_gid[(size_t)o->cols[k]], len = size[(size_t)g];
      if (k + len > kreal) return fail(SLM_ERR_BAD_ARG, "cols: group %d (%d members) is split at position %d", g, len, k);
      for (int m = 0; m < len; ++m) {
        if (ds->h_gid[(size_t)o->cols[k + m]] != g) return fail(SLM_ERR_BAD_ARG, "cols: group %d (%d members) is split at position %d", g, len, k + m);
        h_gs[(size_t)(k + m)] = k;
        h_gl[(size_t)(k + m)] = len;
      }
      k += len;
    }
  }
  auto finite = [](const double* v, size_t count) {
    for (size_t e = 0; e < count; ++e)
      if (!std::isfinite(v[e])) return false;
    return true;
  };
  if (!loose && (!finite(o->gram, (size_t)n_sets * K * K) || !finite(o->gprev, (size_t)B * p)))
    return fail(SLM_ERR_BAD_ARG, "gram / gprev contain a non-finite value");
  if (!finite(o->zprev, (size_t)B * p) || !finite(o->z, (size_t)B * p) || !finite(o->a0, (size_t)B * p) ||
      !finite(o->b0, (size_t)B * G) || !finite(o->d0, (size_t)B * G) || !finite(o->points, (size_t)B * 3) || !finite(o->tol, (size_t)B))
    return fail(SLM_ERR_BAD_ARG, "zprev / z / a0 / b0 / d0 / points / tol contain a non-finite value");
  if (o->Lw && !finite(o->Lw, (size_t)n_sets)) return fail(SLM_ERR_BAD_ARG, "Lw contains a non-finite value");
  for (int st = 0; st < n_sets; ++st)
    for (int r = 0; r < K; ++r)
// ... 146 lines not shown
```

sparse-lm_amd/csrc/engine_solve.hip:

```cpp
#include "engine_internal.hpp"

#define SLM_GK(W, C, R, B) {W, C, R, B, 0, grad_fused_kernel<W, C, R, B>, "grad_fused_kernel<" #W "," #C "," #R "," #B ">"}
#define SLM_RK(W, C, B, D) {W, C, 1, B, D, grad_ring_kernel<W, C, B, D>, "grad_ring_kernel<" #W "," #C "," #B "," #D ">"}
static const GradKernel kGradRing[] = {
    SLM_RK(8, 1, 1, 3), SLM_RK(8, 2, 1, 3), SLM_RK(8, 3, 1, 3), SLM_RK(8, 4, 1, 3), SLM_RK(8, 5, 1, 2),
    SLM_RK(8, 1, 2, 3), SLM_RK(8, 2, 2, 3), SLM_RK(8, 3, 2, 3), SLM_RK(8, 4, 2, 3), SLM_RK(8, 5, 2, 2),
    SLM_RK(8, 1, 3, 3), SLM_RK(8, 2, 3, 3), SLM_RK(8, 3, 3, 3), SLM_RK(8, 4, 3, 3), SLM_RK(8, 5, 3, 2),
    SLM_RK(8, 1, 4, 3), SLM_RK(8, 2, 4, 3), SLM_RK(8, 3, 4, 3), SLM_RK(8, 4, 4, 3), SLM_RK(8, 5, 4, 2),
    SLM_RK(8, 1, 5, 3), SLM_RK(8, 2, 5, 3), SLM_RK(8, 3, 5, 3), SLM_RK(8, 4, 5, 3),
    SLM_RK(8, 1, 6, 3), SLM_RK(8, 2, 6, 3), SLM_RK(8, 3, 6, 3),
};
static const GradKernel kGradDefault[] = {
    SLM_GK(1, 1, 4, 1), SLM_GK(2, 1, 4, 1), SLM_GK(4, 1, 4, 1), SLM_GK(8, 1, 4, 1), SLM_GK(8, 2, 4, 1),
    SLM_GK(8, 3, 4, 1), SLM_GK(8, 4, 2, 1), SLM_GK(8, 5, 2, 1), SLM_GK(8, 6, 2, 1), SLM_GK(8, 8, 2, 1),
    SLM_GK(8, 10, 1, 1),
    SLM_GK(1, 1, 4, 2), SLM_GK(2, 1, 4, 2), SLM_GK(4, 1, 4, 2), SLM_GK(8, 1, 4, 2), SLM_GK(8, 2, 4, 2),
    SLM_GK(8, 3, 4, 2), SLM_GK(8, 4, 2, 2), SLM_GK(8, 5, 2, 2), SLM_GK(8, 6, 2, 2), SLM_GK(8, 8, 1, 2),
    SLM_GK(1, 1, 4, 3), SLM_GK(2, 1, 4, 3), SLM_GK(4, 1, 4, 3), SLM_GK(8, 1, 4, 3), SLM_GK(8, 2, 4, 3),
    SLM_GK(8, 3, 4, 3), SLM_GK(8, 4, 2, 3), SLM_GK(8, 5, 2, 3), SLM_GK(8, 6, 1, 3),
    SLM_GK(1, 1, 4, 4), SLM_GK(2, 1, 4, 4), SLM_GK(4, 1, 4, 4), SLM_GK(8, 1, 4, 4), SLM_GK(8, 2, 4, 4),
    SLM_GK(8, 3, 2, 4), SLM_GK(8, 4, 2, 4), SLM_GK(8, 5, 1, 4),
};
static const GradKernel kGradExtra[] = {
    SLM_GK(8, 5, 1, 1), SLM_GK(8, 5, 3, 1), SLM_GK(8, 5, 4, 1), SLM_GK(8, 4, 4, 1), SLM_GK(8, 6, 1, 1),
    SLM_GK(8, 8, 1, 1), SLM_GK(8, 5, 1, 2), SLM_GK(8, 5, 1, 3), SLM_GK(8, 4, 4, 2), SLM_GK(8, 6, 1, 2),
};

static const int kTwoPassC = 4;
static const GradKernel kGradTwoPass = {8, 4, 2, 1, -1, nullptr, "rowdot_kernel;xtr_kernel<4>"};
static_assert(kTwoPassC == 4, "the name of kGradTwoPass");

#define SLM_SK(C, D)                                                                                   \
  {8, C, SPLIT_LANES, D, rowdot_ring_kernel<8, C, ROWDOT_LANES, D>, resid_ws_kernel<SPLIT_LANES>, "rowdot_ring_kernel<8," #C ",5," #D ">"}
static_assert(ROWDOT_LANES == 5 && SPLIT_LANES == 16, "the names of kSplit and of its residual kernel");
static const SplitKernel kSplit[] = {SLM_SK(1, 3), SLM_SK(2, 3), SLM_SK(3, 3), SLM_SK(4, 3), SLM_SK(5, 2)};
static const SplitKernel kSplitAnyWidth = {8, 0, SPLIT_LANES, 0, nullptr, resid_ws_kernel<SPLIT_LANES>, nullptr};
const SplitKernel* pick_split_kernel(const slm_host::Knobs& kn, int64_t p2) {
  if (!kn.split) return nullptr;
  for (const auto& k : kSplit)
    if (64LL * k.W * k.C >= p2) return &k;
  return &kSplitAnyWidth;
}

int xtr_max_row_blocks(int cus, int64_t ld) {
  return slm_host::xtr_row_blocks_most(cus, ld, XTR_CB);
}
int launch_xtr(const slm_host::Knobs& kn, int cus, SplitArgs& a, hipStream_t s, bool sample, const char** name) {
  double per_cu = kn.xtr_wgs_per_cu;
  const bool wide = a.lane_slots > SPLIT_LANES;
  if (wide) per_cu = 1.0;
  const slm_host::XtrGrid g = slm_host::xtr_grid(a.n, a.ld, XTR_CB, (int64_t)(xtr_max_row_blocks(cus, a.ld) * per_cu / 2.0));
  const int xb = g.xb, yb = g.yb;
  a.xrows = g.rows;
  const int extra = wide ? a.n_lanes - SPLIT_LANES : 0;
  const char* nm;
  if (wide && extra >= 1 && extra <= 2) {
    if (sample) { hipLaunchKernelGGL(xtr18_sample_kernel, dim3(xb, yb), dim3(XTR_WAVES * 64), 0, s, a); nm = "xtr18_sample_kernel"; }
    else { hipLaunchKernelGGL(xtr18_mfma_kernel, dim3(xb, yb), dim3(XTR_WAVES * 64), 0, s, a); nm = "xtr18_mfma_kernel"; }
  } else if (wide && extra >= 3 && extra <= 4) {
    if (sample) { hipLaunchKernelGGL(xtr20_sample_kernel, dim3(xb, yb), dim3(XTR_WAVES * 64), 0, s, a); nm = "xtr20_sample_kernel"; }
    else { hipLaunchKernelGGL(xtr20_mfma_kernel, dim3(xb, yb), dim3(XTR_WAVES * 64), 0, s, a); nm = "xtr20_mfma_kernel"; }
  } else if (wide) {
    if (sample) { hipLaunchKernelGGL(xtr32_sample_kernel, dim3(xb, yb), dim3(XTR_WAVES * 64), 0, s, a); nm = "xtr32_sample_kernel"; }
    else { hipLaunchKernelGGL(xtr32_mfma_kernel, dim3(xb, yb), dim3(XTR_WAVES * 64), 0, s, a); nm = "xtr32_mfma_kernel"; }
  } else {
    if (sample) { hipLaunchKernelGGL(xtr_sample_kernel, dim3(xb, yb), dim3(XTR_WAVES * 64), 0, s, a); nm = "xtr_sample_kernel"; }
    else { hipLaunchKernelGGL(xtr_mfma_kernel, dim3(xb, yb), dim3(XTR_WAVES * 64), 0, s, a); nm = "xtr_mfma_kernel"; }
  }
  if (name) *name = nm;
  return yb;
}

static int launch_cov_gz(int cus, SplitArgs& a, hipStream_t s, const CovBatch& cb, int n_sets, GradNames* names) {
  const slm_host::XtrGrid g = slm_host::xtr_grid(a.n, a.ld, XTR_CB, xtr_max_row_blocks(cus, a.ld) / 2);
  const int xb = g.xb, yb = g.yb;
  a.xrows = g.rows;
  const int per = ((WS_KCAP + yb - 1) / yb + 3) / 4 * 4;
  a.xrows_ws = (a.ctl != nullptr && per <= 32) ? per : 0;
  if (names) {
    names->product = a.r_plane != 0 ? "cov_gz32_mfma_kernel" : "cov_gz_mfma_kernel";
    names->cov_rows_ws = a.xrows_ws;
    names->cov_row_blocks = yb;
  }
  if (a.r_plane != 0) hipLaunchKernelGGL(cov_gz32_mfma_kernel, dim3(xb, yb, (unsigned)n_sets), dim3(XTR_WAVES * 64), 0, s, a, cb);
  else hipLaunchKernelGGL(cov_gz_mfma_kernel, dim3(xb, yb, (unsigned)n_sets), dim3(XTR_WAVES * 64), 0, s, a, cb);
  return yb;
}

const GradKernel* pick_grad_kernel(const slm_host::Knobs& kn, int64_t p2, int B) {
  if (p2 > kMaxChunks) return B == 1 ? &kGradTwoPass : nullptr;
  const bool ring_off = kn.grad_ring == 0, ring_all = kn.grad_ring == 1;
  if (!ring_off && p2 > 256 && (B >= 3 || ring_all)) {
    for (const auto& k : kGradRing)
      if (k.B == B && 64LL * k.W * k.C >= p2) return &k;
  }
  if (kn.grad_cfg[0] > 0) {
    const int W = kn.grad_cfg[0], C = kn.grad_cfg[1], R = kn.grad_cfg[2];
    for (const auto& k : kGradDefault)
      if (k.B == B && k.W == W && k.C == C && k.R == R && 64LL * W * C >= p2) return &k;
    for (const auto& k : kGradExtra)
      if (k.B == B && k.W == W && k.C == C && k.R == R && 64LL * W * C >= p2) return &k;
  }
  for (const auto& k : kGradDefault)
    if (k.B == B && 64LL * k.W * k.C >= p2) return &k;
  return nullptr;
}

LaneSetup default_lanes(slm_dataset* ds, int B) {
  LaneSetup ls;
  ls.B = B;
  ls.rw = ds->rw;
  ls.rw_stride = 0;
  for (int l = 0; l < kMaxCells; ++l) ls.n_eff[l] = (double)ds->n_global;
  return ls;
}

int enqueue_gradient(slm_dataset* ds, const LaneSetup& ls, const double* y, const int* done,
                     hipEvent_t ev_start, hipEvent_t ev_stop, int64_t n_rows, const int* skip, GradNames* names) {
  hipStream_t s = ds->eng->stream;
  const int B = ls.B;
  const GradKernel* gk = ds->gk[B - 1];
  if (!gk) return fail(SLM_ERR_UNSUPPORTED, "no %d-lane gradient kernel covers p = %lld", B, (long long)ds->p);
  if (names) names->product = gk->name;
  const int nblk = ds->nblk[B - 1];
  GradArgs a;
  a.X = ds->X;
  a.y = y;
  a.rw = ls.rw;
  a.z = ds->z;
  a.partial = ds->partial;
  a.loss_partial = ds->loss_partial;
  a.done = done;
  a.skip = skip;
  const int64_t nr = n_rows > 0 ? n_rows : ds->n;
  a.n = nr;
  a.ld = ds->ld;
  a.rows_base = nr / nblk;
  a.rows_rem = nr % nblk;
  a.rw_stride = ls.rw_stride;
  a.p2 = (int)(ds->ld / 2);
  if (ev_start) HIP_TRY(hipEventRecord(ev_start, s));
  if (gk->D >= 0) {
    hipLaunchKernelGGL(gk->fn, dim3(nblk), dim3(gk->W * 64), 0, s, a);
  } else {
    TwoPassArgs t;
    t.X = ds->X; t.y = y; t.rw = ls.rw; t.z = a.z; t.r = ds->rvec; t.partial = a.partial;
    t.loss_partial = a.loss_partial; t.done = done; t.skip = skip; t.n = nr; t.ld = ds->ld;
    t.rows_base = a.rows_base; t.rows_rem = a.rows_rem; t.p2 = a.p2;
    hipLaunchKernelGGL(rowdot_kernel, dim3(nblk), dim3(256), 0, s, t);
    const unsigned tiles = (unsigned)((a.p2 + 512 * kTwoPassC - 1) / (512 * kTwoPassC));
    hipLaunchKernelGGL(xtr_kernel<kTwoPassC>, dim3(nblk, tiles), dim3(512), 0, s, t);
  }
  if (ev_stop) HIP_TRY(hipEventRecord(ev_stop, s));
  ReduceArgs ra;
  ra.partial = a.partial;
  ra.loss_partial = a.loss_partial;
  ra.g = ds->g;
  ra.done = done;
  ra.skip = skip;
  ra.nblk = nblk;
  ra.nblk_loss = nblk;
  ra.n_lanes = B;
  ra.ld = ds->ld;
  for (int l = 0; l < kMaxLanes; ++l) {
    const double ne = ls.n_eff[l] > 0 ? ls.n_eff[l] : (double)ds->n_global;
    ra.scale[l] = 1.0 / ne;
    ra.loss_scale[l] = 0.5 / ne;
  }
  hipLaunchKernelGGL(reduce_partials_kernel, dim3((unsigned)(ds->ld / 16 + 1), B), dim3(256), 0, s, ra);
  if (row_sharded(ds))
    SLM_TRY(all_reduce_sum(ds->eng, ds->g, (size_t)B * (size_t)(ds->ld + 16)));
  return SLM_OK;
}

void launch_rowdot(const slm_host::Knobs& kn, slm_dataset* ds, const SplitKernel* sk, int nblk, int B, SplitArgs& a, hipStream_t s,
                  const char** name) {
  const int halves = (B + SPLIT_LANES - 1) / SPLIT_LANES;
  const bool ring = sk->rowdot != nullptr && halves == 1 && (kn.rowdot_ring >= 0 ? kn.rowdot_ring == 1 : B <= ROWDOT_LANES);
  a.lane0 = 0;
  if ((!ring || sk->rowdot == nullptr) && ds->XT && ds->XT_ready) {
    a.XT = ds->XT;
    const bool extras = halves == 2 && B <= SPLIT_LANES + 4;
    const char* nm;
    if (extras && B <= SPLIT_LANES + 2) { hipLaunchKernelGGL(rowdot18_mfma_kernel, dim3(nblk, 1), dim3(XZ_WAVES * 64), 0, s, a); nm = "rowdot18_mfma_kernel"; }
    else if (extras) { hipLaunchKernelGGL(rowdot20_mfma_kernel, dim3(nblk, 1), dim3(XZ_WAVES * 64), 0, s, a); nm = "rowdot20_mfma_kernel"; }
    else if (halves == 2) { hipLaunchKernelGGL(rowdot32_mfma_kernel, dim3(nblk, 1), dim3(XZ_WAVES * 64), 0, s, a); nm = "rowdot32_mfma_kernel"; }
    else { hipLaunchKernelGGL(rowdot_mfma_kernel, dim3(nblk, halves), dim3(XZ_WAVES * 64), 0, s, a); nm = "rowdot_mfma_kernel"; }
    if (name) *name = nm;
  } else if (sk->rowdot != nullptr) {
    hipLaunchKernelGGL(sk->rowdot, dim3(nblk, (B + ROWDOT_LANES - 1) / ROWDOT_LANES), dim3(sk->W * 64), 0, s, a);
    if (name) *name = sk->rowdot_name;
  }
}

bool split_usable(const slm_host::Knobs& kn, slm_dataset* ds) {
  if (!ds->sk) return false;
  if (ds->sk->rowdot != nullptr) return true;
  if (ensure_xt(kn, ds) != SLM_OK) return false;
  return ds->XT != nullptr;
}

int enqueue_gradient_split(const slm_host::Knobs& kn, slm_dataset* ds, const LaneSetup& ls, const double* y, const int* done,
                           const PathCtl* ctl, const WsArgs* wa, hipEvent_t ev_start,
                           hipEvent_t ev_stop, int64_t n_rows, bool unit_bracket, const int* skip, GradNames* names) {
  hipStream_t s = ds->eng->stream;
  const SplitKernel* sk = ds->sk;
  const int nblk = ds->split_nblk;
  if (!ds->R) {
    SLM_TRY(dalloc(&ds->R, (size_t)ds->n * SPLIT_RSTRIDE * SPLIT_HALVES));
    HIP_TRY(hipMemsetAsync(ds->R, 0, sizeof(double) * (size_t)ds->n * SPLIT_RSTRIDE * SPLIT_HALVES, s));
  }
  const int halves = (ls.B + SPLIT_LANES - 1) / SPLIT_LANES;
  if (halves > 1 && !(ds->XT && ds->XT_ready)) return fail(SLM_ERR_UNSUPPORTED, "more than %d lanes need the column-major copy of X", SPLIT_LANES);
  SplitArgs a;
  memset(&a, 0, sizeof(a));
  a.X = ds->X; a.y = y; a.rw = ls.rw; a.rw_stride = ls.rw_stride; a.z = ds->z; a.R = ds->R;
  a.lane_slots = SPLIT_LANES * halves; a.r_plane = (int64_t)ds->n * SPLIT_RSTRIDE;
  a.partial = ds->partial; a.loss_partial = ds->loss_partial; a.done = done; a.ctl = ctl; a.skip = skip;
  if (wa) { a.XW = wa->XW; a.idx = wa->idx; a.ws = wa->ws; }
  const int64_t nr = n_rows > 0 ? n_rows : ds->n;
  a.n = nr; a.ld = ds->ld; a.rows_base = nr / nblk; a.rows_rem = nr % nblk;
  a.p2 = (int)(ds->ld / 2);
  a.n_lanes = ls.B;
  const bool unit = ev_start != nullptr && unit_bracket;
  if (unit) HIP_TRY(hipEventRecord(ev_start, s));
  launch_rowdot(kn, ds, sk, nblk, ls.B, a, s, names ? &names->resid : nullptr);
  if (wa && ctl) {
    const char* nm;
    if (kn.resid_vec && halves == 1) { hipLaunchKernelGGL(sk->resid, dim3(nblk), dim3(256), 0, s, a); nm = "resid_ws_kernel<16>"; }
    else if (halves == 2) { hipLaunchKernelGGL(resid32_mfma_kernel, dim3(nblk, 1), dim3(RM_WAVES * 64), 0, s, a); nm = "resid32_mfma_kernel"; }
    else { hipLaunchKernelGGL(resid_mfma_kernel, dim3(nblk, halves), dim3(RM_WAVES * 64), 0, s, a); nm = "resid_mfma_kernel"; }
    if (names) names->ws_resid = nm;
  }
  if (ev_start && !unit) HIP_TRY(hipEventRecord(ev_start, s));
  const int xblk = launch_xtr(kn, ds->eng->cus, a, s, n_rows > 0 && ctl != nullptr,
                              names ? &names->product : nullptr);
  if (ev_stop) HIP_TRY(hipEventRecord(ev_stop, s));
  ReduceArgs ra;
  ra.partial = ds->partial;
  ra.loss_partial = ds->loss_partial;
  ra.g = ds->g;
  ra.done = done;
  ra.nblk = xblk;
  ra.nblk_loss = nblk;
  ra.skip = skip;
  ra.n_lanes = a.lane_slots;
  ra.ld = ds->ld;
  for (int l = 0; l < kMaxLanes; ++l) {
    const double ne = ls.n_eff[l] > 0 ? ls.n_eff[l] : (double)ds->n_global;
    ra.scale[l] = 1.0 / ne;
    ra.loss_scale[l] = 0.5 / ne;
  }
  hipLaunchKernelGGL(reduce_partials_kernel, dim3((unsigned)(ds->ld / 16 + 1), ls.B), dim3(256), 0, s, ra);
  if (row_sharded(ds))
    SLM_TRY(all_reduce_sum(ds->eng, ds->g, (size_t)ls.B * (size_t)(ds->ld + 16)));
  return SLM_OK;
}

int enqueue_gradient_cov(slm_dataset* ds, int B, const int* entry_of, const int* done, hipEvent_t ev_start,
                         hipEvent_t ev_stop, const PathCtl* ctl, const WsArgs* wa, GradNames* names) {
  hipStream_t s = ds->eng->stream;
  const int64_t ld = ds->ld;
  const int halves = (B + SPLIT_LANES - 1) / SPLIT_LANES;
  hipLaunchKernelGGL(cov_pack_kernel, dim3((unsigned)((ld * SPLIT_RSTRIDE + 255) / 256), (unsigned)halves), dim3(256), 0, s, ds->z, ld, B, ds->cov_Z, done);
  if (ev_start) HIP_TRY(hipEventRecord(ev_start, s));
  CovBatch cb;
  memset(&cb, 0, sizeof(cb));
  int n_sets = 0, entry_of_set[SLM_MAX_LANES];
  for (int l = 0; l < B; ++l) {
    int st = -1;
    for (int k = 0; k < n_sets && st < 0; ++k)
      if (entry_of_set[k] == entry_of[l]) st = k;
    if (st < 0) {
      st = n_sets++;
      entry_of_set[st] = entry_of[l];
      const slm_dataset::CovEntry& e = ds->cov[(size_t)entry_of[l]];
      cb.G[st] = e.G; cb.c[st] = e.c; cb.yy[st] = e.yy;
    }
    cb.set_of[l] = st;
  }
  const int64_t blocks_most = std::max<int64_t>(1, xtr_max_row_blocks(ds->eng->cus, ld) / 2);
  cb.part_stride = blocks_most * SPLIT_LANES * ld;
  cb.half_stride = (int64_t)n_sets * cb.part_stride;
  const int blocks = halves * n_sets;
  double* partial = ds->partial;
  if ((size_t)blocks * (size_t)cb.part_stride > ds->partial_elems) {
    if (ds->cov_partial_sets < blocks) {
      dfree(ds->cov_partial);
      ds->cov_partial_sets = 0;
      SLM_TRY(dalloc(&ds->cov_partial, (size_t)blocks * (size_t)cb.part_stride));
      ds->cov_partial_sets = blocks;
    }
    partial = ds->cov_partial;
  }
  SplitArgs a;
  memset(&a, 0, sizeof(a));
  a.R = ds->cov_Z; a.partial = partial; a.done = done;
  a.n = ld; a.ld = ld; a.p2 = (int)(ld / 2); a.n_lanes = B;
  if (ctl && wa && wa->ws) { a.ctl = ctl; a.ws = wa->ws; a.idx = wa->idx; }
  a.lane0 = 0;
  a.r_plane = halves > 1 ? ld * SPLIT_RSTRIDE : 0;
  const int xblk = launch_cov_gz(ds->eng->cus, a, s, cb, n_sets, names);
  CovFinishArgs f;
  f.partial = partial; f.z = ds->z; f.g = ds->g; f.done = done; f.nblk = xblk; f.ld = ld;
  hipLaunchKernelGGL(cov_reduce_kernel, dim3((unsigned)(ld / 16), (unsigned)B), dim3(256), 0, s, f, cb);
  hipLaunchKernelGGL(cov_loss_kernel, dim3((unsigned)B), dim3(256), 0, s, f, cb);
  if (ev_stop) HIP_TRY(hipEventRecord(ev_stop, s));
  return SLM_OK;
}

int cov_fingerprints(slm_dataset* ds, const double* const* w, int count, double* out ) {
  hipStream_t s = ds->eng->stream;
  if (!ds->cov_fp) SLM_TRY(dalloc(&ds->cov_fp, 2 * (size_t)kMaxLanes + 2));
  CovFpArgs fa;
  memset(&fa, 0, sizeof(fa));
  for (int u = 0; u < count; ++u) fa.w[u] = w[u];
  hipLaunchKernelGGL(cov_fingerprint_kernel, dim3((unsigned)count), dim3(1024), 0, s, fa, ds->n, ds->cov_fp);
  HIP_TRY(hipMemcpyAsync(out, ds->cov_fp, sizeof(double) * 2 * (size_t)count, hipMemcpyDeviceToHost, s));
  HIP_TRY(hipStreamSynchronize(s));
  return SLM_OK;
}

int cov_find(const slm_dataset* ds, double fp1, double fp2, double n_eff) { return slm_host::find_by_fingerprint(ds->cov, fp1, fp2, n_eff); }

void launch_tail(const TailArgs& ta, hipStream_t s) {
  const int E = (ta.p + TAIL_THREADS - 1) / TAIL_THREADS;
  const dim3 grid(ta.n_lanes);
#define SLM_TAIL_LAUNCH(N) hipLaunchKernelGGL(fista_tail_kernel<N>, grid, dim3(TAIL_THREADS), 0, s, ta)
  switch (E) {
    case 1: SLM_TAIL_LAUNCH(1); break;
    case 2: SLM_TAIL_LAUNCH(2); break;
    case 3: SLM_TAIL_LAUNCH(3); break;
    case 4: SLM_TAIL_LAUNCH(4); break;
    case 5: SLM_TAIL_LAUNCH(5); break;
    case 6: SLM_TAIL_LAUNCH(6); break;
    case 7: hipLaunchKernelGGL(fista_tail_stream_kernel<7>, grid, dim3(TAIL_THREADS), 0, s, ta); break;
// ... 149 lines not shown
    LaneSetup part = default_lanes(ds, 1);
    for (int l = 0; l < kMaxLanes; ++l) part.n_eff[l] = (double)ds->n_global * (double)n_s / (double)ds->n;
    bool usable = false, on_image = false;
    if (!kn.sample_f64 && !ds->rw) SLM_TRY(ensure_x32s(ds, n_s, &usable));
    if (usable) SLM_TRY(enqueue_sample_f32(ds, n_s, part.n_eff[0], 1, nullptr, &on_image));
    if (!on_image) {
      if (split_usable(kn, ds)) SLM_TRY(enqueue_gradient_split(kn, ds, part, ds->y, nullptr, nullptr, nullptr, nullptr, nullptr, n_s));
      else SLM_TRY(enqueue_gradient(ds, part, ds->y, nullptr, nullptr, nullptr, n_s));
    }
    SLM_TRY(check_launch());
    HIP_TRY(hipStreamSynchronize(s));
    if (g_out) HIP_TRY(hipMemcpy(g_out, ds->g, sizeof(double) * ds->p, hipMemcpyDeviceToHost));
    if (loss_out) HIP_TRY(hipMemcpy(loss_out, ds->g + ds->ld, sizeof(double), hipMemcpyDeviceToHost));
    if (ms_out) *ms_out = 0.0;
    return SLM_OK;
  }
  if (z) HIP_TRY(hipMemcpyAsync(ds->z, z, sizeof(double) * ds->p, hipMemcpyHostToDevice, s));
  const bool use_split = o.route == 1 && split_usable(kn, ds);
  if (use_split) SLM_TRY(ensure_xt(kn, ds));
  int lanes_run = 1, lane_out = 0;
  if (use_split && ds->XT && ds->XT_ready && (size_t)ds->lane_cap >= (size_t)kMaxLanes) {
    lanes_run = std::max(1, (int)o.n_lanes);
    lane_out = std::min(lanes_run - 1, std::max(0, (int)o.lane_out));
  }
  auto spread_z = [&](int B) -> int {
    for (int l = 1; l < B; ++l)
      HIP_TRY(hipMemcpyAsync(ds->z + (size_t)l * ds->ld, ds->z, sizeof(double) * ds->ld, hipMemcpyDeviceToDevice, s));
    return SLM_OK;
  };
  const LaneSetup ls = default_lanes(ds, lanes_run);
  SLM_TRY(spread_z(lanes_run));
  if (use_split) SLM_TRY(enqueue_gradient_split(kn, ds, ls, ds->y, nullptr, nullptr, nullptr, nullptr, nullptr));
  else SLM_TRY(enqueue_gradient(ds, ls, ds->y, nullptr, nullptr, nullptr));
  SLM_TRY(check_launch());
  HIP_TRY(hipStreamSynchronize(s));
  const double* g_lane = ds->g + (size_t)lane_out * (size_t)(ds->ld + 16);
  if (g_out) HIP_TRY(hipMemcpy(g_out, g_lane, sizeof(double) * ds->p, hipMemcpyDeviceToHost));
  if (loss_out) HIP_TRY(hipMemcpy(loss_out, g_lane + ds->ld, sizeof(double), hipMemcpyDeviceToHost));
  if (!ms_out) return SLM_OK;
  *ms_out = 0.0;
  if (reps < 1) reps = 1;
  const int B = std::max(1, (int)o.probe_lanes);
  SLM_TRY(spread_z(B));
  const LaneSetup lb = default_lanes(ds, B);
  if (use_split) {
    SLM_TRY(enqueue_gradient_split(kn, ds, lb, ds->y, nullptr, nullptr, nullptr, nullptr, nullptr));
    SplitArgs a;
    memset(&a, 0, sizeof(a));
    a.X = ds->X; a.y = ds->y; a.rw = lb.rw; a.rw_stride = 0; a.z = ds->z; a.R = ds->R;
    a.partial = ds->partial; a.loss_partial = ds->loss_partial;
    a.n = ds->n; a.ld = ds->ld; a.rows_base = ds->n / ds->split_nblk; a.rows_rem = ds->n % ds->split_nblk;
    a.p2 = (int)(ds->ld / 2); a.n_lanes = B;
    a.lane_slots = SPLIT_LANES * ((B + SPLIT_LANES - 1) / SPLIT_LANES); a.r_plane = (int64_t)ds->n * SPLIT_RSTRIDE;
    return timed_launches(s, reps, ms_out, [&]() -> int {
      if (!o.xtr_only) launch_rowdot(kn, ds, ds->sk, ds->split_nblk, B, a, s);
      (void)launch_xtr(kn, ds->eng->cus, a, s);
      return SLM_OK;
    });
  }
  const GradKernel* gk = ds->gk[B - 1];
  if (!gk) return fail(SLM_ERR_UNSUPPORTED, "no %d-lane kernel for p = %lld", B, (long long)ds->p);
  if (gk->D < 0)
    return timed_launches(s, reps, ms_out, [&]() -> int { return enqueue_gradient(ds, lb, ds->y, nullptr, nullptr, nullptr); });
  const int nblk = ds->nblk[B - 1];
  GradArgs a;
  a.X = ds->X; a.y = ds->y; a.rw = lb.rw; a.z = ds->z; a.partial = ds->partial;
  a.loss_partial = ds->loss_partial; a.done = nullptr; a.n = ds->n; a.ld = ds->ld;
  a.rows_base = ds->n / nblk; a.rows_rem = ds->n % nblk; a.rw_stride = 0; a.p2 = (int)(ds->ld / 2);
  hipLaunchKernelGGL(gk->fn, dim3(nblk), dim3(gk->W * 64), 0, s, a);
  return timed_launches(s, reps, ms_out, [&]() -> int {
    hipLaunchKernelGGL(gk->fn, dim3(nblk), dim3(gk->W * 64), 0, s, a);
    return SLM_OK;
  });
}

extern "C" int slm_gradient(slm_dataset* ds, const double* z, double* g_out, double* loss_out, int32_t reps, double* ms_out) {
  return slm_gradient_ex(ds, z, nullptr, g_out, loss_out, reps, ms_out);
}

extern "C" int slm_gradient_lanes(slm_dataset* ds, int32_t route, int32_t n_lanes, const double* Z, const double* row_weights,
                                  const double* n_eff, const int32_t* cov_index, int64_t n_rows, double* G_out, double* loss_out,
                                  char* kernels_out, int32_t kernels_len) {
  if (!ds || !Z || !G_out) return fail(SLM_ERR_BAD_ARG, "NULL argument");
  if (route < 0 || route > 2) return fail(SLM_ERR_BAD_ARG, "route must be 0 (fused), 1 (split pass) or 2 (covariance), got %d", route);
  if (n_lanes < 1 || n_lanes > kMaxLanes) return fail(SLM_ERR_BAD_ARG, "between 1 and %d lanes, got %d", kMaxLanes, n_lanes);
  if (n_rows < 0 || n_rows > ds->n) return fail(SLM_ERR_BAD_ARG, "n_rows = %lld outside [0, %lld]", (long long)n_rows, (long long)ds->n);
  if (row_sharded(ds)) return fail(SLM_ERR_UNSUPPORTED, "slm_gradient_lanes: row-sharded datasets");
  if (n_lanes > ds->lane_cap) return fail(SLM_ERR_UNSUPPORTED, "%d lanes: the dataset holds %d", n_lanes, ds->lane_cap);
  const int B = n_lanes;
  const int64_t n = ds->n, p = ds->p, ld = ds->ld;
  for (int64_t k = 0; k < (int64_t)B * p; ++k)
    if (!std::isfinite(Z[k])) return fail(SLM_ERR_BAD_ARG, "Z contains a non-finite value");
  if (row_weights)
    for (int64_t k = 0; k < (int64_t)B * n; ++k)
      if (!(row_weights[k] >= 0.0) || !std::isfinite(row_weights[k]))
        return fail(SLM_ERR_BAD_ARG, "row_weights[%lld] is negative or not finite", (long long)k);
  if (n_eff)
    for (int l = 0; l < B; ++l)
      if (!(n_eff[l] > 0.0) || !std::isfinite(n_eff[l])) return fail(SLM_ERR_BAD_ARG, "n_eff[%d] must be positive and finite", l);
  if (route == 2) {
    if (row_weights || n_rows > 0) return fail(SLM_ERR_UNSUPPORTED, "route 2 takes its rows from the covariance entries: no row_weights or n_rows");
    if (ds->cov.empty()) return fail(SLM_ERR_UNSUPPORTED, "route 2: the dataset has no covariance entries");
    if (!cov_index) return fail(SLM_ERR_BAD_ARG, "route 2 needs cov_index");
    for (int l = 0; l < B; ++l)
      if (cov_index[l] < 0 || cov_index[l] >= (int32_t)ds->cov.size())
        return fail(SLM_ERR_BAD_ARG, "cov_index[%d] = %d: the dataset has %d entries", l, cov_index[l], (int)ds->cov.size());
  }
  const slm_host::Knobs kn = knobs();
  HIP_TRY(hipSetDevice(ds->eng->device));
  hipStream_t s = ds->eng->stream;
  if (route == 0 && !ds->gk[B - 1]) return fail(SLM_ERR_UNSUPPORTED, "route 0: no %d-lane kernel covers p = %lld", B, (long long)p);
  if (route == 1) {
    if (!ds->sk) return fail(SLM_ERR_UNSUPPORTED, "route 1: no split pass for p = %lld", (long long)p);
    SLM_TRY(ensure_xt(kn, ds));
    if (!split_usable(kn, ds) || (B > SPLIT_LANES && !(ds->XT && ds->XT_ready)))
      return fail(SLM_ERR_UNSUPPORTED, "route 1: no residual kernel for %d lanes at p = %lld without the column-major copy", B, (long long)p);
  }
  const int slots = route == 0 ? B : SPLIT_LANES * ((B + SPLIT_LANES - 1) / SPLIT_LANES);
  HIP_TRY(hipMemsetAsync(ds->z, 0, sizeof(double) * (size_t)slots * ld, s));
  HIP_TRY(hipMemcpy2DAsync(ds->z, sizeof(double) * ld, Z, sizeof(double) * p, sizeof(double) * p, B, hipMemcpyHostToDevice, s));
  LaneSetup ls = default_lanes(ds, B);
  if (row_weights) {
    if (!ds->rw_lanes) SLM_TRY(dalloc(&ds->rw_lanes, (size_t)ds->lane_cap * n));
    HIP_TRY(hipMemcpyAsync(ds->rw_lanes, row_weights, sizeof(double) * (size_t)B * n, hipMemcpyHostToDevice, s));
    ls.rw = ds->rw_lanes;
    ls.rw_stride = n;
  }
  if (n_eff)
    for (int l = 0; l < B; ++l) ls.n_eff[l] = n_eff[l];
  GradNames names;
  if (route == 0) {
    SLM_TRY(enqueue_gradient(ds, ls, ds->y, nullptr, nullptr, nullptr, n_rows, nullptr, &names));
  } else if (route == 1) {
    SLM_TRY(enqueue_gradient_split(kn, ds, ls, ds->y, nullptr, nullptr, nullptr, nullptr, nullptr, n_rows, false, nullptr, &names));
  } else {
    if (!ds->cov_Z) SLM_TRY(dalloc(&ds->cov_Z, (size_t)ld * SPLIT_RSTRIDE * SPLIT_HALVES));
    SLM_TRY(enqueue_gradient_cov(ds, B, cov_index, nullptr, nullptr, nullptr, nullptr, nullptr, &names));
  }
  SLM_TRY(check_launch());
  HIP_TRY(hipStreamSynchronize(s));
  const size_t lane_bytes = sizeof(double) * (size_t)(ld + 16);
  HIP_TRY(hipMemcpy2D(G_out, sizeof(double) * p, ds->g, lane_bytes, sizeof(double) * p, B, hipMemcpyDeviceToHost));
  if (loss_out) HIP_TRY(hipMemcpy2D(loss_out, sizeof(double), ds->g + ld, lane_bytes, sizeof(double), B, hipMemcpyDeviceToHost));
  if (kernels_out && kernels_len > 0) {
    if (names.resid && names.product) snprintf(kernels_out, (size_t)kernels_len, "%s;%s", names.resid, names.product);
    else snprintf(kernels_out, (size_t)kernels_len, "%s", names.resid ? names.resid : names.product ? names.product : "");
  }
  return SLM_OK;
}

extern "C" int slm_dataset_read_ceiling(slm_dataset* ds, int32_t reps, double* gbs_out, double* ms_out) {
  if (!ds || !gbs_out) return fail(SLM_ERR_BAD_ARG, "NULL argument");
  if (reps < 1) reps = 1;
  HIP_TRY(hipSetDevice(ds->eng->device));
  hipStream_t s = ds->eng->stream;
  const int64_t count2 = ds->n * ds->ld / 2;
  const int cus = ds->eng->cus;
  double* sink = nullptr;
  SLM_TRY(dalloc(&sink, (size_t)cus * 16));
  hipEvent_t e0, e1;
  HIP_TRY(hipEventCreate(&e0));
  HIP_TRY(hipEventCreate(&e1));
  typedef void (*Kernel)(const double*, int64_t, double*);
  struct Form { Kernel fn; int per_cu; const char* name; };
  const Form forms[] = {
      {read_stream_kernel<8, true>, 1, "1 workgroup per CU, 8 loads in flight, non-temporal"},
      {read_stream_kernel<8, true>, 2, "2 per CU, 8, non-temporal"},
      {read_stream_kernel<8, true>, 4, "4 per CU, 8, non-temporal"},
      {read_stream_kernel<16, true>, 1, "1 per CU, 16, non-temporal"},
      {read_stream_kernel<16, true>, 2, "2 per CU, 16, non-temporal"},
      {read_stream_kernel<8, false>, 2, "2 per CU, 8, cached"},
      {read_stream_kernel<8, false>, 4, "4 per CU, 8, cached"},
      {read_stream_kernel<4, true>, 8, "8 per CU, 4, non-temporal"},
      {read_stream_kernel<8, true, true>, 1, "1 per CU, 8, non-temporal, chunks in turn"},
      {read_stream_kernel<8, true, true>, 2, "2 per CU, 8, non-temporal, chunks in turn"},
      {read_stream_kernel<8, true, true>, 4, "4 per CU, 8, non-temporal, chunks in turn"},
      {read_stream_kernel<16, true, true>, 2, "2 per CU, 16, non-temporal, chunks in turn"},
      {read_stream_kernel<4, false, true>, 8, "8 per CU, 4, cached, chunks in turn"},
  };
  double best = 1e300;
  const char* best_name = "";
  const bool trace = knobs().trace != 0;
  for (const Form& f : forms) {
    const int blocks = cus * f.per_cu;
    hipLaunchKernelGGL(f.fn, dim3(blocks), dim3(256), 0, s, (const double*)ds->X, count2, sink);
    HIP_TRY(hipEventRecord(e0, s));
    for (int r = 0; r < reps; ++r) hipLaunchKernelGGL(f.fn, dim3(blocks), dim3(256), 0, s, (const double*)ds->X, count2, sink);
    HIP_TRY(hipEventRecord(e1, s));
    HIP_TRY(hipEventSynchronize(e1));
    float ms = 0.f;
    HIP_TRY(hipEventElapsedTime(&ms, e0, e1));
    const double per = (double)ms / reps;
    if (trace) fprintf(stderr, "[slm] read stream, %s: %.4f ms per sweep = %.0f GB/s\n", f.name, per, 16.0 * (double)count2 / (per * 1e-3) / 1e9);
    if (per < best) {
      best = per;
      best_name = f.name;
    }
  }
  (void)best_name;
  (void)hipEventDestroy(e0);
  (void)hipEventDestroy(e1);
  dfree(sink);
  SLM_TRY(check_launch());
  if (ms_out) *ms_out = best;
  *gbs_out = 16.0 * (double)count2 / (best * 1e-3) / 1e9;
  return SLM_OK;
}

extern "C" int slm_eval_sse(slm_dataset* ds, const double* Z, int32_t m, const double* row_weight,
                            double* sse_out) {
  if (!ds || !Z || !sse_out) return fail(SLM_ERR_BAD_ARG, "NULL argument");
  if (m <= 0) return fail(SLM_ERR_BAD_ARG, "m must be positive");
  const slm_host::Knobs kn = knobs();
  HIP_TRY(hipSetDevice(ds->eng->device));
  hipStream_t s = ds->eng->stream;
  const int64_t n = ds->n, p = ds->p, ld = ds->ld;
  for (int64_t k = 0; k < (int64_t)m * p; ++k)
    if (!std::isfinite(Z[k])) return fail(SLM_ERR_BAD_ARG, "Z contains a non-finite value");
  LaneSetup ls = default_lanes(ds, 1);
  if (row_weight) {
    for (int64_t i = 0; i < n; ++i)
      if (!(row_weight[i] >= 0.0) || !std::isfinite(row_weight[i]))
        return fail(SLM_ERR_BAD_ARG, "row_weight[%lld] is negative or not finite", (long long)i);
    if (!ds->rw_lanes) SLM_TRY(dalloc(&ds->rw_lanes, (size_t)ds->lane_cap * n));
    HIP_TRY(hipMemcpyAsync(ds->rw_lanes, row_weight, sizeof(double) * n, hipMemcpyHostToDevice, s));
    HIP_TRY(hipStreamSynchronize(s));
    ls.rw = ds->rw_lanes;
    ls.rw_stride = 0;
  }
  for (int l = 0; l < kMaxLanes; ++l) ls.n_eff[l] = 0.5;
  int maxB = SPLIT_LANES;
  while (maxB > 1 && !ds->gk[maxB - 1]) --maxB;
  std::vector<double> losses(kMaxLanes);
  if (m > maxB && ds->sk != nullptr && !row_sharded(ds) && split_usable(kn, ds) && !kn.eval_fused &&
      (ds->sk->rowdot != nullptr || (ensure_xt(kn, ds) == SLM_OK && ds->XT && ds->XT_ready))) {
    const int nblk = ds->split_nblk;
    if (!ds->R) {
      SLM_TRY(dalloc(&ds->R, (size_t)n * SPLIT_RSTRIDE * SPLIT_HALVES));
      HIP_TRY(hipMemsetAsync(ds->R, 0, sizeof(double) * (size_t)n * SPLIT_RSTRIDE * SPLIT_HALVES, s));
    }
    for (int32_t k0 = 0; k0 < m; k0 += SPLIT_LANES) {
      const int B = std::min<int32_t>(SPLIT_LANES, m - k0);
      HIP_TRY(hipMemsetAsync(ds->z, 0, sizeof(double) * SPLIT_LANES * ld, s));
      HIP_TRY(hipMemcpy2DAsync(ds->z, sizeof(double) * ld, Z + (size_t)k0 * p, sizeof(double) * p, sizeof(double) * p, B, hipMemcpyHostToDevice, s));
      SplitArgs a;
      memset(&a, 0, sizeof(a));
      a.X = ds->X; a.y = ds->y; a.rw = ls.rw; a.rw_stride = ls.rw_stride; a.z = ds->z; a.R = ds->R;
      a.partial = ds->partial; a.loss_partial = ds->loss_partial;
      a.n = n; a.ld = ld; a.rows_base = n / nblk; a.rows_rem = n % nblk;
      a.p2 = (int)(ld / 2);
      a.n_lanes = B;
      a.lane_slots = SPLIT_LANES; a.r_plane = (int64_t)n * SPLIT_RSTRIDE;
      launch_rowdot(kn, ds, ds->sk, nblk, B, a, s);
      hipLaunchKernelGGL(sse_from_blocks_kernel, dim3(1), dim3(64), 0, s, ds->loss_partial, nblk, SPLIT_LANES, ds->partial);
      SLM_TRY(check_launch());
      HIP_TRY(hipMemcpyAsync(losses.data(), ds->partial, sizeof(double) * SPLIT_LANES, hipMemcpyDeviceToHost, s));
      HIP_TRY(hipStreamSynchronize(s));
      for (int l = 0; l < B; ++l) sse_out[k0 + l] = losses[l];
    }
    return SLM_OK;
  }
  for (int32_t k0 = 0; k0 < m; k0 += maxB) {
    const int B = std::min<int32_t>(maxB, m - k0);
    ls.B = B;
    HIP_TRY(hipMemsetAsync(ds->z, 0, sizeof(double) * SPLIT_LANES * ld, s));
    for (int l = 0; l < B; ++l)
      HIP_TRY(hipMemcpyAsync(ds->z + (size_t)l * ld, Z + (size_t)(k0 + l) * p, sizeof(double) * p,
                             hipMemcpyHostToDevice, s));
    SLM_TRY(enqueue_gradient(ds, ls, ds->y, nullptr, nullptr, nullptr));
    SLM_TRY(check_launch());
    for (int l = 0; l < B; ++l)
      HIP_TRY(hipMemcpyAsync(&losses[l], ds->g + (size_t)l * (ld + 16) + ld, sizeof(double),
                             hipMemcpyDeviceToHost, s));
    HIP_TRY(hipStreamSynchronize(s));
    for (int l = 0; l < B; ++l) sse_out[k0 + l] = losses[l];
  }
  return SLM_OK;
}

int ensure_xt(const slm_host::Knobs& kn, slm_dataset* ds) {
  hipStream_t s = ds->eng->stream;
  const int64_t n = ds->n, ld = ds->ld;
  const int64_t row_tiles = (n + 31) / 32;
  if (!ds->XT && !ds->XT_failed) {
    if (pool_malloc((void**)&ds->XT, sizeof(double) * (size_t)ld * (size_t)row_tiles * 32) != hipSuccess) {
      (void)hipGetLastError();
      ds->XT = nullptr;
      ds->XT_failed = true;
    }
  }
  if (ds->XT && !ds->XT_ready) {
    ds->XT_ready = true;
    ds->colnorm_ready = false;
    const dim3 grid((unsigned)row_tiles, (unsigned)((ld + 31) / 32));
    hipLaunchKernelGGL(tile_columns_kernel, grid, dim3(256), 0, s, (const double*)ds->X, n, ld, ds->XT);
  }
  if (ds->XT && ds->XT_ready && !ds->colnorm_ready && !ds->rw && !row_sharded(ds) && kn.light_pass) {
    if (!ds->colnorm && pool_malloc((void**)&ds->colnorm, sizeof(double) * (size_t)ld) != hipSuccess) {
      (void)hipGetLastError();
      ds->colnorm = nullptr;
    }
    if (ds->colnorm) {
      hipLaunchKernelGGL(colnorm_kernel, dim3((unsigned)((ld + 7) / 8)), dim3(256), 0, s, (const double*)ds->XT, n, ld, 1.0 / (double)ds->n_global,
                         ds->colnorm);
      ds->colnorm_ready = true;
    }
  }
  return SLM_OK;
}

void x32_drop(slm_dataset* ds) {
  dfree(ds->X32s);
  ds->rows32 = 0;
  ds->ld32 = 0;
  ds->x32_lossy = false;
}
int ensure_x32s(slm_dataset* ds, int64_t n_rows, bool* usable) {
  *usable = false;
  if (ds->x32_failed || ds->x32_lossy || n_rows < 1 || n_rows > ds->n) return SLM_OK;
  if (ds->X32s && ds->rows32 >= n_rows) {
    *usable = true;
    return SLM_OK;
  }
  hipStream_t s = ds->eng->stream;
  HIP_TRY(hipStreamSynchronize(s));
  x32_drop(ds);
  const int64_t ld32 = slm_host::sample_ld32(ds->p);
  unsigned int* lost = nullptr;
  if (pool_malloc((void**)&ds->X32s, sizeof(float) * (size_t)ld32 * (size_t)n_rows) != hipSuccess ||
      pool_malloc((void**)&lost, sizeof(unsigned int)) != hipSuccess) {
    (void)hipGetLastError();
    if (lost) pool_free(lost);
    lost = nullptr;
    dfree(ds->X32s);
    ds->x32_failed = true;
    return SLM_OK;
  }
  unsigned int host = 0;
  hipError_t e = hipMemsetAsync(lost, 0, sizeof(unsigned int), s);
  if (e == hipSuccess) {
    const int64_t work = n_rows * (ld32 / 4);
    const unsigned blocks = (unsigned)std::max<int64_t>(1, std::min<int64_t>((int64_t)ds->eng->cus * 8, (work + 255) / 256));
    hipLaunchKernelGGL(x32_convert_kernel, dim3(blocks), dim3(256), 0, s, (const double*)ds->X, n_rows, ds->ld, ld32, ds->X32s, lost);
    e = hipGetLastError();
  }
  if (e == hipSuccess) e = hipMemcpyAsync(&host, lost, sizeof(unsigned int), hipMemcpyDeviceToHost, s);
  if (e == hipSuccess) e = hipStreamSynchronize(s);
  pool_free(lost);
  if (e != hipSuccess) {
    dfree(ds->X32s);
    return fail(SLM_ERR_HIP, "fp32 image of the sample rows: %s", hipGetErrorString(e));
  }
  if (host != 0) {
    dfree(ds->X32s);
    ds->x32_lossy = true;
    return SLM_OK;
  }
  ds->rows32 = n_rows;
  ds->ld32 = ld32;
  *usable = true;
  return SLM_OK;
}

int enqueue_sample_f32(slm_dataset* ds, int64_t n_rows, double n_eff, int n_lanes, const int* done, bool* queued) {
  *queued = false;
  if (!ds->X32s || n_rows < 1 || n_rows > ds->rows32 || n_lanes < 1 || n_lanes > ds->lane_cap) return SLM_OK;
  const slm_host::SamplePlan g = slm_host::sample_plan(n_rows, ds->p, ds->ld32, ds->eng->cus);
  if ((size_t)g.yb * (size_t)ds->ld + (size_t)g.yb > ds->partial_elems) return SLM_OK;
  SampleArgs a;
  a.X32 = ds->X32s; a.y = ds->y; a.partial = ds->partial; a.g = ds->g; a.done = done;
  a.n_s = n_rows; a.ld32 = ds->ld32; a.ld = ds->ld; a.rows = g.rows; a.pstride = ds->ld;
  a.p = (int)ds->p; a.yb = g.yb; a.n_lanes = n_lanes;
  a.scale = 1.0 / n_eff;
  hipStream_t s = ds->eng->stream;
  hipLaunchKernelGGL(sample_xty_kernel<8>, dim3((unsigned)g.xb, (unsigned)g.yb), dim3(slm_host::kSampleThreads), 0, s, a);
  hipLaunchKernelGGL(sample_finish_kernel, dim3((unsigned)(ds->ld / 16 + 1)), dim3(256), 0, s, a);
  *queued = true;
  return SLM_OK;
}

// ... 298 lines not shown
```

sparse-lm_amd/csrc/host_logic.hpp:

```cpp
#pragma once
#include <stddef.h>
#include <math.h>
#include <stdint.h>
#include <stdio.h>
#include <stdlib.h>

#include <algorithm>
#include <utility>
#include <vector>

#if defined(__HIPCC__)
#define SLM_HD __host__ __device__
#else
#define SLM_HD
#endif

namespace slm_host {

struct PoolLedger {
  struct Idle { int dev; size_t bytes; void* block; };
  struct Live { void* block; int dev; size_t bytes; };
  std::vector<Idle> idle;
  std::vector<Live> live;
  size_t idle_bytes = 0;
// ... 88 lines not shown
      if (lane >= F) {
        w.n_points = (int32_t)B;
      } else {
        w.n_points = (int32_t)(B + F);
        const int64_t t = B + F + lane;
        if (t < total) w.tail_pt = (int32_t)t;
      }
      return w;
    }
  }
  if (tail_band && rem > 0 && n_reg >= 2 * (int64_t)B) {
    w.n_points = (int32_t)n_reg;
    if (lane >= B - rem) w.tail_pt = (int32_t)(n_reg + (lane - (B - rem)));
  }
  return w;
}
inline int64_t interleaved_points(const LaneWalk& w) {
  const int64_t regular = w.n_points > w.first ? ((int64_t)w.n_points - w.first + w.stride - 1) / w.stride : 0;
  return regular + (w.tail_pt >= 0 ? 1 : 0);
}

struct XtrGrid { int xb, yb, rows; };
inline int auto_path_lanes(int64_t n_points, int cap, bool big, bool wide_ok) {
  if (n_points < 1) n_points = 1;
  const int narrow = (int)std::min<int64_t>(std::min(cap, 16), n_points);
  if (!big || cap < 20 || n_points <= 16) return narrow;
  int best = narrow;
  double best_cost = 1.45 * (double)((n_points + 15) / 16);
  auto offer = [&](int64_t lanes) {
    lanes = std::min(lanes, n_points);
    if (lanes <= 16 || lanes > cap) return;
    const int64_t passes = (n_points + lanes - 1) / lanes;
    const double cost = (double)passes * ((lanes <= 20 ? 1.03 : 1.22) + 0.45);
    if (cost < best_cost - 1e-9) {
      best_cost = cost;
      best = (int)lanes;
    }
  };
  offer(18);
  offer(20);
  if (wide_ok)
    for (int64_t passes = 1; passes <= (n_points + 20) / 21; ++passes) {
      const int64_t lanes = (n_points + passes - 1) / passes;
      if (lanes > 20 && lanes <= 32) offer(lanes);
    }
  return best;
}

inline int xtr_row_blocks_most(int cus, int64_t ld, int col_block) {
  const int xb = (int)((ld + col_block - 1) / col_block);
  return std::max(1, 2 * cus / xb);
}
inline XtrGrid xtr_grid(int64_t n, int64_t ld, int col_block, int64_t want) {
  XtrGrid g;
  g.xb = (int)((ld + col_block - 1) / col_block);
  if (want < 1) want = 1;
  int64_t rows = (n + want - 1) / want;
  rows = (rows + 7) / 8 * 8;
  g.rows = (int)rows;
  g.yb = (int)((n + rows - 1) / rows);
  return g;
}

constexpr int kSampleThreads = 256;
constexpr int kSampleWgsPerCu = 4;
constexpr int kSampleMinRows = 16;
struct SamplePlan {
  int xb, yb;
  int64_t rows;
  int64_t ld32;
};
inline int64_t sample_ld32(int64_t p) { return (p + 3) / 4 * 4; }
inline SamplePlan sample_plan(int64_t n_s, int64_t p, int64_t ld32, int cus) {
  SamplePlan g;
  g.ld32 = ld32;
  (void)p;
  const int64_t quads = ld32 / 4;
  g.xb = (int)std::max<int64_t>(1, (quads + kSampleThreads - 1) / kSampleThreads);
  if (n_s < 1) n_s = 1;
  const int64_t want = std::max<int64_t>(1, (int64_t)kSampleWgsPerCu * std::max(1, cus) / g.xb);
  g.rows = std::max<int64_t>(kSampleMinRows, (n_s + want - 1) / want);
  g.yb = (int)((n_s + g.rows - 1) / g.rows);
  return g;
}

template <typename Entry>
inline int find_by_fingerprint(const std::vector<Entry>& entries, double fp1, double fp2, double n_eff) {
  for (size_t i = 0; i < entries.size(); ++i)
    if (entries[i].fp1 == fp1 && entries[i].fp2 == fp2 && entries[i].n_eff == n_eff) return (int)i;
  return -1;
}

inline void triangle_tile(int t, int* I_out, int* J_out) {
  int I = 0;
  while ((I + 1) * (I + 2) / 2 <= t) ++I;
  *I_out = I;
  *J_out = t - I * (I + 1) / 2;
}
inline int triangle_tiles(int side) { return side * (side + 1) / 2; }
SLM_HD inline void triangle_tile_fast(int t, int* I_out, int* J_out) {
  int I = (int)((sqrtf(8.0f * (float)t + 1.0f) - 1.0f) * 0.5f);
  while (I * (I + 1) / 2 > t) --I;
  while ((I + 1) * (I + 2) / 2 <= t) ++I;
  *I_out = I;
  *J_out = t - I * (I + 1) / 2;
}

inline int model_gram_cap(int64_t ld, double budget_bytes, int most) {
  const double each = 4.0 * (double)ld * (double)ld;
  return (int)std::max<double>(1.0, std::min<double>((double)most, budget_bytes / each));
}

constexpr int kSketchPowerIters = 1;
constexpr int kSketchRowDiv = 32;
constexpr int kWsLookahead = 2;
constexpr int kWsPowerIters = 10;

struct Knobs {
  bool split = true;
  double xtr_wgs_per_cu = 1.0;
  int grad_ring = -1;
  int grad_cfg[3] = {0, 0, 0};
  int rowdot_ring = -1;
  bool resid_vec = false;
  int cov_tile = 0;
  int power_iters = 0;
  int ws = -1;
  bool on_chip = true;
  int auto_lanes = 0;
  bool interleave = true;
  bool tail_band = true;
  bool carry = true;
  bool ws_carry = true;
  bool eval_fused = false;
  double ws_theta = 0.85;
  int ws_append = 48;
  int ws_kinit = 0;
  int ws_bb = 1;
  int ws_one_solver = 0;
  bool hard_callwide = false;
  int ws_miss_factor = 4;
  int ws_miss_div = 8;
  double ws_fill = 0.0;
  bool sample_start = true;
  int64_t sample_min_rows = 65536;
  int sample_div = 4;
  bool sample_f64 = false;
  int mg = -1;
  bool handover = true;
  bool light_pass = true;
  bool lag_handover = true;
  bool gram_owner = true;
  double device_pool_gb = -1.0;
  bool allow_any_arch = false;
  int trace = 0;
  bool trace_poll = false;

  template <typename Get>
  static Knobs from(Get get) {
    Knobs k;
    auto text = [&](const char* name) -> const char* { return get(name); };
    auto is_set = [&](const char* name) { return text(name) != nullptr; };
    auto first = [&](const char* name) -> char { const char* e = text(name); return e ? e[0] : '\0'; };
    auto as_int = [&](const char* name, int lo, int hi, int* out) {
      if (const char* e = text(name)) *out = std::max(lo, std::min(hi, atoi(e)));
    };
    k.split = first("SLM_SPLIT") != '0';
    if (const char* e = text("SLM_XTR_WGS_PER_CU")) {
      const double f = atof(e);
      if (f > 0.0 && f <= 2.0) k.xtr_wgs_per_cu = f;
    }
    if (const char c = first("SLM_GRAD_RING")) k.grad_ring = c == '0' ? 0 : (c == '1' ? 1 : -1);
    if (const char* e = text("SLM_GRAD_CONFIG")) {
      int W = 0, C = 0, R = 0;
      if (sscanf(e, "%d,%d,%d", &W, &C, &R) == 3) { k.grad_cfg[0] = W; k.grad_cfg[1] = C; k.grad_cfg[2] = R; }
    }
    if (const char c = first("SLM_ROWDOT_RING")) k.rowdot_ring = c == '1' ? 1 : 0;
    k.resid_vec = first("SLM_RESID_VEC") == '1';
    if (const char* e = text("SLM_COV_TILE")) k.cov_tile = atoi(e);
    if (const char* e = text("SLM_POWER_ITERS")) k.power_iters = std::max(2, atoi(e));
    if (const char c = first("SLM_WS")) k.ws = c == '0' ? 0 : (c == '1' ? 1 : -1);
    k.on_chip = first("SLM_ON_CHIP") != '0';
    if (const char* e = text("SLM_AUTO_LANES")) k.auto_lanes = std::max(1, atoi(e));
    k.interleave = !is_set("SLM_NO_INTERLEAVE");
    k.tail_band = !is_set("SLM_NO_TAIL_BAND");
    k.carry = !is_set("SLM_NO_CARRY");
    k.ws_carry = !is_set("SLM_NO_WS_CARRY");
    k.eval_fused = is_set("SLM_EVAL_FUSED");
    if (const char* e = text("SLM_WS_THETA")) {
      const double v = atof(e);
      if (v > 0.0 && v <= 1.0) k.ws_theta = v;
    }
    as_int("SLM_WS_APPEND", 1, 512, &k.ws_append);
    as_int("SLM_WS_KINIT", 16, 512, &k.ws_kinit);
    if (const char* e = text("SLM_WS_BB")) k.ws_bb = atoi(e) != 0;
    if (const char* e = text("SLM_WS_ONE_SOLVER")) k.ws_one_solver = atoi(e) != 0;
    k.hard_callwide = is_set("SLM_HARD_CALLWIDE");
    as_int("SLM_WS_MISS_FACTOR", 1, 8, &k.ws_miss_factor);
    as_int("SLM_WS_MISS_DIV", 1, 4096, &k.ws_miss_div);
    if (const char* e = text("SLM_WS_FILL")) k.ws_fill = std::max(0.1, std::min(1.0, atof(e)));
    k.sample_start = !is_set("SLM_NO_SAMPLE_START");
    if (const char* e = text("SLM_SAMPLE_START_MIN_ROWS")) k.sample_min_rows = std::max<int64_t>(64, atoll(e));
    as_int("SLM_SAMPLE_DIV", 1, 64, &k.sample_div);
    k.sample_f64 = first("SLM_SAMPLE_F64") == '1';
    if (const char c = first("SLM_MG")) k.mg = c == '0' ? 0 : (c == '2' ? 2 : -1);
    k.handover = !is_set("SLM_NO_HANDOVER");
    k.light_pass = !is_set("SLM_NO_LIGHT_PASS");
    k.gram_owner = !is_set("SLM_NO_GRAM_OWNER");
    k.lag_handover = !is_set("SLM_NO_LAG_HANDOVER");
    if (const char* e = text("SLM_DEVICE_POOL_GB")) k.device_pool_gb = std::max(0.0, atof(e));
    k.allow_any_arch = is_set("SLM_ALLOW_ANY_ARCH");
    if (const char c = first("SLM_TRACE")) k.trace = (c >= '1' && c <= '3') ? c - '0' : 1;
    k.trace_poll = is_set("SLM_TRACE_POLL");
    return k;
  }
};

}
```

sparse-lm_amd/csrc/light_ctl.hpp:

```cpp
#pragma once
#include <stdint.h>

#include "../../include/slm_engine.h"

namespace slm {

constexpr int LT_CAP = 1024;
constexpr int LT_LANES = 8;

struct LightCtl {
  int32_t ok;
  int32_t n_cols;
  int32_t n_live;
  int32_t lane_of[LT_LANES];
  int32_t attempts;
  int32_t used;
  int32_t cols_total;
  int32_t why;
  int32_t id;
  int32_t epoch[SLM_MAX_LANES];
  int32_t pend_epoch[SLM_MAX_LANES];
  double pend_slack[SLM_MAX_LANES];
  double D[LT_LANES];
  double slack[SLM_MAX_LANES];
};

}
```

sparse-lm_amd/sparselm_amd/_engine.py:

```python

from __future__ import annotations

import ctypes as C
import os
import sys
import threading
import weakref

import numpy as np

_LIB_NAME = "libslm_hip.so"
_LIB_DIR = os.path.join(os.path.dirname(os.path.abspath(__file__)), "_lib")

SLM_OK = 0
SLM_ERR_BAD_ARG = 1
SLM_ERR_OOM = 2
SLM_ERR_HIP = 3
SLM_ERR_NO_DEVICE = 4
SLM_ERR_COMM = 5
SLM_ERR_NOT_CONVERGED = 6
SLM_ERR_NON_FINITE = 7
SLM_ERR_UNSUPPORTED = 8

FLAG_NO_RESTART = 1
# ... 673 lines not shown
        eng = Engine(self.engine.device_id) if engine is None else engine
        h = C.c_void_p()
        _check(self._lib.slm_dataset_clone(self._h, eng._h, C.byref(h)))
        return Dataset(eng, h, self.n, self.p)

    def set_targets(self, y):
        yv = _f64(y, "y", (self.n,))
        _check(self._lib.slm_dataset_set_targets(self._h, _ptr(yv)))

    def set_global_rows(self, n_global: int):
        _check(self._lib.slm_dataset_set_global_rows(self._h, int(n_global)))

    def set_groups(self, gidx, n_groups=None):
        if gidx is None:
            _check(self._lib.slm_dataset_set_groups(self._h, None, 0))
            self.n_groups = self.p
            return
        g = np.ascontiguousarray(gidx, dtype=np.int32)
        if g.shape != (self.p,):
            raise ValueError(f"gidx must have shape ({self.p},)")
        G = int(g.max()) + 1 if n_groups is None else int(n_groups)
        _check(self._lib.slm_dataset_set_groups(self._h, _ptr(g), G))
        self.n_groups = G

    def max_lanes(self, flags: int = 0) -> int:
        _sync_knobs()
        out = C.c_int32()
        _check(self._lib.slm_dataset_max_lanes(self._h, int(flags), C.byref(out)))
        return int(out.value)

    def path_lanes(self, n_points: int, flags: int = 0) -> int:
        _sync_knobs()
        out = C.c_int32()
        _check(self._lib.slm_dataset_path_lanes(self._h, int(n_points), int(flags), C.byref(out)))
        return int(out.value)

    def lipschitz(self) -> float:
        _sync_knobs()
        L = C.c_double()
        _check(self._lib.slm_dataset_lipschitz(self._h, C.byref(L)))
        return L.value

    def gradient(self, z=None, reps: int = 0, split: bool = False, lanes: int = 1, lane: int = 0, probe_lanes: int = 1,
                 xtr_only: bool = False):
        _sync_knobs()
        zz = None if z is None else _f64(z, "z", (self.p,))
        g = np.empty(self.p)
        loss = C.c_double()
        ms = C.c_double()
        if not split and lanes == 1 and probe_lanes == 1:
            _check(self._lib.slm_gradient(self._h, _ptr(zz), _ptr(g), C.byref(loss), int(reps), C.byref(ms) if reps > 0 else None))
        else:
            o = _GradientOpts(1 if split else 0, int(lanes), int(lane), int(probe_lanes), 1 if xtr_only else 0)
            _check(self._lib.slm_gradient_ex(self._h, _ptr(zz), C.byref(o), _ptr(g), C.byref(loss), int(reps),
                                             C.byref(ms) if reps > 0 else None))
        return (g, loss.value, ms.value) if reps > 0 else (g, loss.value)

    def sample_product(self):
        _sync_knobs()
        g = np.empty(self.p)
        loss = C.c_double()
        o = _GradientOpts(2, 1, 0, 1, 0)
        _check(self._lib.slm_gradient_ex(self._h, None, C.byref(o), _ptr(g), C.byref(loss), 0, None))
        return g, loss.value

    def gradient_lanes(self, Z, row_weights=None, n_eff=None, route: int = 0, cov_index=None, n_rows: int = 0):
        _sync_knobs()
        Z = _f64(np.atleast_2d(Z), "Z")
        B = Z.shape[0]
        if Z.shape[1] != self.p:
            raise ValueError(f"Z must have {self.p} columns")
        rw = None if row_weights is None else _f64(row_weights, "row_weights", (B, self.n))
        ne = None if n_eff is None else _f64(n_eff, "n_eff", (B,))
        ci = None if cov_index is None else np.ascontiguousarray(cov_index, dtype=np.int32)
        if ci is not None and ci.shape != (B,):
            raise ValueError(f"cov_index has shape {ci.shape}, expected {(B,)}")
        G = np.empty((B, self.p))
        loss = np.empty(B)
        names = C.create_string_buffer(512)
        _check(self._lib.slm_gradient_lanes(self._h, int(route), B, _ptr(Z), _ptr(rw), _ptr(ne), _ptr(ci), int(n_rows),
                                            _ptr(G), _ptr(loss), names, len(names)))
        return G, loss, names.value.decode()

    def working_set_lanes(self, Z, cols, k_end, on_ws=None, row_weights=None, n_eff=None, route: int = 1, cov_index=None,
                          gather_from_x: bool = False, xty: bool = False, want_xw: bool = False):
        import types

        _sync_knobs()
        Z = _f64(np.atleast_2d(Z), "Z")
        B = Z.shape[0]
        if Z.shape[1] != self.p:
            raise ValueError(f"Z must have {self.p} columns")
        cols = np.ascontiguousarray(cols, dtype=np.int32)
        k_end = np.ascontiguousarray(np.atleast_1d(k_end), dtype=np.int32)
        if k_end.size == 0 or cols.size < int(k_end[-1]):
            raise ValueError("cols must hold k_end[-1] feature indices")
        kreal = int(k_end[-1])
        K = max(16, (kreal + 15) // 16 * 16)
        ow = None if on_ws is None else np.ascontiguousarray(np.broadcast_to(np.asarray(on_ws, dtype=np.int32), (B,)))
        rw = None if row_weights is None else _f64(row_weights, "row_weights", (B, self.n))
        ne = None if n_eff is None else _f64(n_eff, "n_eff", (B,))
        ci = None if cov_index is None else np.ascontiguousarray(cov_index, dtype=np.int32)
        if ci is not None and ci.shape != (B,):
            raise ValueError(f"cov_index has shape {ci.shape}, expected {(B,)}")
        opts = _WsLanesOpts(int(route), B, _ptr(Z), _ptr(ow), _ptr(rw), _ptr(ne), _ptr(ci), _ptr(cols), _ptr(k_end),
                            int(k_end.size), (WSL_GATHER_X if gather_from_x else 0) | (WSL_XTY if xty else 0))
        G = np.empty((B, self.p))
        loss = np.empty(B)
        set_of = np.empty(B, dtype=np.int32)
        n_sets = C.c_int32(0)
        gram = np.empty((B, K, K))
        XW = np.empty((self.n, K)) if want_xw else None
        xt = np.empty(kreal + 1) if xty else None
        names = C.create_string_buffer(4096)
        _check(self._lib.slm_working_set_lanes(self._h, C.byref(opts), _ptr(G), _ptr(loss), _ptr(set_of), C.byref(n_sets),
                                               _ptr(gram), _ptr(XW), _ptr(xt), names, len(names)))
        ns = n_sets.value
        return types.SimpleNamespace(G=G, loss=loss, gram=gram[:ns], set_of=set_of, n_sets=ns, K=K, XW=XW,
                                     xty=None if xt is None else xt[:kreal], yy=None if xt is None else float(xt[kreal]),
                                     kernels=names.value.decode())

    def working_set_model_solve(self, cols, gram, zprev, gprev, z, a0, b0, d0, points, tol, mode, set_of=None, Lw=None,
                                direct: bool = True, hard: bool = False, invalid: bool = False, building: bool = False,
                                disabled: bool = False, stale: bool = False, allow_nonfinite: bool = False, repeats=None,
                                last_point=None, last_cols=None, flags: int = 0):
        import types

        _sync_knobs()
        z = _f64(np.atleast_2d(z), "z")
        B = z.shape[0]
        if z.shape[1] != self.p:
            raise ValueError(f"z must have {self.p} columns")
        cols = np.ascontiguousarray(cols, dtype=np.int32).reshape(-1)
        kreal = int(cols.size)
        K = max(16, (kreal + 15) // 16 * 16)
        gram = _f64(gram, "gram")
        if gram.ndim == 2:
            gram = gram[None]
        if gram.ndim != 3 or gram.shape[1:] != (K, K):
            raise ValueError(f"gram has shape {gram.shape}, expected (sets, {K}, {K})")
        gram = np.ascontiguousarray(gram)
        ns = gram.shape[0]
        zprev = _f64(zprev, "zprev", (B, self.p))
        gprev = _f64(gprev, "gprev", (B, self.p))
        a0 = _f64(a0, "a0", (B, self.p))
        b0 = _f64(np.atleast_2d(b0), "b0")
        d0 = _f64(np.atleast_2d(d0), "d0")
        if b0.shape != d0.shape or b0.shape[0] != B:
            raise ValueError("b0 and d0 must have shape (lanes, groups)")
        points = _f64(points, "points", (B, 3))
        tol = _f64(np.broadcast_to(np.asarray(tol, dtype=np.float64), (B,)), "tol", (B,))

        def ints(v, count):
            return None if v is None else np.ascontiguousarray(np.broadcast_to(np.asarray(v, dtype=np.int32), (count,)))

        mode = ints(mode, B)
        so, rp, lp, lc = ints(set_of, B), ints(repeats, B), ints(last_point, B), ints(last_cols, B)
        lw = None if Lw is None else _f64(np.broadcast_to(np.asarray(Lw, dtype=np.float64), (ns,)), "Lw", (ns,))
        fl = int(flags) | (WMS_DIRECT if direct else 0) | (WMS_HARD if hard else 0) | (WMS_INVALID if invalid else 0) | \
            (WMS_BUILDING if building else 0) | (WMS_DISABLED if disabled else 0) | (WMS_STALE if stale else 0) | \
            (WMS_NONFINITE if allow_nonfinite else 0)
        opts = _WsModelOpts(B, kreal, _ptr(cols), ns, fl, _ptr(gram), _ptr(so), _ptr(zprev), _ptr(gprev), _ptr(z), _ptr(a0),
                            _ptr(b0), _ptr(d0), _ptr(points), _ptr(tol), _ptr(mode), _ptr(lw), _ptr(rp), _ptr(lp), _ptr(lc))
        o = types.SimpleNamespace(z=np.empty((B, self.p)), beta=np.empty((B, self.p)))
        for name in ("served", "zsup", "have_base", "zzero", "want_full", "repeats", "hard_lane", "last_point"):
            setattr(o, name, np.zeros(B, dtype=np.int32))
# ... 491 lines not shown
```

Measured before the change: 17110.

## Run X^T R gradient passes on fp32 image with exact f64 patch for borderline columns

```diff
diff --git a/sparse-lm_amd/csrc/engine.hip b/sparse-lm_amd/csrc/engine.hip
--- a/sparse-lm_amd/csrc/engine.hip
+++ b/sparse-lm_amd/csrc/engine.hip
@@ -278,6 +278,7 @@
   dfree(ds->ws_nt); dfree(ds->stop_words); dfree(ds->sse_Z); dfree(ds->sse_part); dfree(ds->split_state);
   dfree(ds->cons_state); dfree(ds->cons_buf);
   dfree(ds->colnorm); dfree(ds->lt_dR); dfree(ds->lt_d2); dfree(ds->lt_part); dfree(ds->lt_cols); dfree(ds->lt_stamp);
+  dfree(ds->pf_list); dfree(ds->pf_part);
   cov_pending_drop(ds);
   ds->cov.clear();
   ds->cov_all_hold.reset();
diff --git a/sparse-lm_amd/csrc/engine_internal.hpp b/sparse-lm_amd/csrc/engine_internal.hpp
--- a/sparse-lm_amd/csrc/engine_internal.hpp
+++ b/sparse-lm_amd/csrc/engine_internal.hpp
@@ -26,6 +26,7 @@
 #include "split_kernels.hpp"
 #include "sample_kernels.hpp"
 #include "light_kernels.hpp"
+#include "pass_f32_kernels.hpp"
 #include "small_kernels.hpp"
 #include "small_split_kernels.hpp"
 #include "small_constrained_kernels.hpp"
@@ -101,6 +102,7 @@
 const SplitKernel* pick_split_kernel(const slm_host::Knobs& kn, int64_t p2);
 int xtr_max_row_blocks(int cus, int64_t ld);
 int launch_xtr(const slm_host::Knobs& kn, int cus, SplitArgs& a, hipStream_t s, bool sample = false, const char** name = nullptr);
+int launch_xtr_f32(const slm_host::Knobs& kn, int cus, SplitArgs& a, const float* X32, int64_t ld32, hipStream_t s, const char** name = nullptr);
 const GradKernel* pick_grad_kernel(const slm_host::Knobs& kn, int64_t p2, int B);
 
 struct LocalComm {
@@ -154,6 +156,7 @@
   GlobalCtl g;
   MgCtl mg;
   LightCtl lt;
+  PassF32Ctl pf;
   WsCtl ws;
   PathCtl lane[SLM_MAX_CELLS];
   slm_point_info infos[kSnapInfos];
@@ -226,6 +229,8 @@
   bool colnorm_ready = false;
   double *lt_dR = nullptr, *lt_d2 = nullptr, *lt_part = nullptr;
   int32_t *lt_cols = nullptr, *lt_stamp = nullptr;
+  int32_t* pf_list = nullptr;
+  double* pf_part = nullptr;
   struct MgEntry {
     float* G = nullptr;
     double fp1 = 0.0, fp2 = 0.0, n_eff = 0.0;
@@ -303,9 +308,14 @@
 LaneSetup default_lanes(slm_dataset* ds, int B);
 int enqueue_gradient(slm_dataset* ds, const LaneSetup& ls, const double* y, const int* done, hipEvent_t ev_start, hipEvent_t ev_stop,
                      int64_t n_rows = 0, const int* skip = nullptr, GradNames* names = nullptr);
+struct PassF32Plan {
+  bool certify = false;
+  PfArgs pa;
+};
 int enqueue_gradient_split(const slm_host::Knobs& kn, slm_dataset* ds, const LaneSetup& ls, const double* y, const int* done, const PathCtl* ctl, const WsArgs* wa,
                            hipEvent_t ev_start, hipEvent_t ev_stop, int64_t n_rows = 0, bool unit_bracket = false, const int* skip = nullptr,
-                           GradNames* names = nullptr);
+                           GradNames* names = nullptr, const PassF32Plan* f32 = nullptr);
+void launch_pf_exact(const PfArgs& pa, hipStream_t s);
 bool split_usable(const slm_host::Knobs& kn, slm_dataset* ds);
 int ensure_xt(const slm_host::Knobs& kn, slm_dataset* ds);
 int ensure_x32s(slm_dataset* ds, int64_t n_rows, bool* usable);
diff --git a/sparse-lm_amd/csrc/engine_path.hip b/sparse-lm_amd/csrc/engine_path.hip
--- a/sparse-lm_amd/csrc/engine_path.hip
+++ b/sparse-lm_amd/csrc/engine_path.hip
@@ -114,6 +114,9 @@
   bool done = false, results_queued = false, results_final = false, deferred = false, trace3 = false;
   bool light_begun = false;
   const int* light_skip = nullptr;
+  bool f32_solve = false;
+  bool last_f32 = false;
+  PassF32Plan f32_plan;
   std::vector<char> prof_rec;
   bool mg_forced = false, mg_ok = false, mg_on = false;
   int mg_cap = 0, mg_inner = 20, mg_built = 0;
@@ -132,7 +135,8 @@
   int ws_setup(bool late);
   void ws_release();
   int prepare_working_set();
-  int enqueue_pass_gradient(hipEvent_t e0, hipEvent_t e1);
+  int enqueue_pass_gradient(hipEvent_t e0, hipEvent_t e1, bool f32);
+  int pass_f32_solve();
   void enqueue_tail();
   void enqueue_refinement();
   void plan_queue();
@@ -178,6 +182,7 @@
   if (small) return run_on_chip();
   SLM_TRY(prepare_working_set());
   plan_queue();
+  SLM_TRY(pass_f32_solve());
   if (n_sample > 0 && !kn.sample_f64) SLM_TRY(ensure_x32s(ds, n_sample, &sample_f32));
   SLM_TRY(pass_loop());
   return finish();
@@ -829,9 +834,10 @@
   return SLM_OK;
 }
 
-int PathCall::enqueue_pass_gradient(hipEvent_t e0, hipEvent_t e1) {
+int PathCall::enqueue_pass_gradient(hipEvent_t e0, hipEvent_t e1, bool f32) {
   if (cov_on) return enqueue_gradient_cov(ds, B, cov_entry, done_flag, e0, e1, ds->ctl, use_ws ? &wa : nullptr);
-  if (split) return enqueue_gradient_split(kn, ds, ls, ds->y, done_flag, ds->ctl, &wa, e0, e1, 0, (o.flags & SLM_FLAG_PROFILE_UNIT) != 0, light_skip);
+  if (split) return enqueue_gradient_split(kn, ds, ls, ds->y, done_flag, ds->ctl, &wa, e0, e1, 0, (o.flags & SLM_FLAG_PROFILE_UNIT) != 0, light_skip,
+                                           nullptr, f32 ? &f32_plan : nullptr);
   return enqueue_gradient(ds, ls, ds->y, done_flag, e0, e1, 0, light_skip);
 }
 
@@ -916,6 +922,12 @@
       ws_enqueue_build(ds, wa, &cs, false, done_flag, B, s);
     } else {
       ws_enqueue_build(ds, wa, nullptr, fix_start, done_flag, B, s);
+      if (last_f32) {
+        PfArgs pa = f32_plan.pa;
+        pa.patch = 1;
+        hipLaunchKernelGGL(pf_new_kernel, dim3(1), dim3(1024), 0, s, pa);
+        launch_pf_exact(pa, s);
+      }
     }
     if (wa.Gx) {
       const size_t gram_words = (size_t)wa.n_sets * WS_KCAP * WS_KCAP;
@@ -1037,9 +1049,10 @@
 
 void PathCall::trace_pass(const DevCtl& now) const {
   if (!trace3) return;
-  fprintf(stderr, "[slm] pass %lld at %.3f ms: K %d builds %d appends %d misses %d stale %d refined %d | mg on %d rounds %d inner %d most %d rej %d | light %d of %d (last: %d columns, why %d, D %.3g) | lanes (point.iter/flags):",
+  fprintf(stderr, "[slm] pass %lld at %.3f ms: K %d builds %d appends %d misses %d stale %d refined %d | mg on %d rounds %d inner %d most %d rej %d | light %d of %d (last: %d columns, why %d, D %.3g) | f32 %d of %d (borderline %d, last %d, why %d) | lanes (point.iter/flags):",
           (long long)enq, t_mark(), now.ws.Kreal, now.ws.builds, now.ws.appends, now.ws.misses, now.ws.stale, now.ws.refined, (int)mg_on,
-          now.mg.rounds, now.mg.inner_iters, now.mg.most_iters, now.mg.rejected, now.lt.used, now.lt.attempts, now.lt.n_cols, now.lt.why, now.lt.D[0]);
+          now.mg.rounds, now.mg.inner_iters, now.mg.most_iters, now.mg.rejected, now.lt.used, now.lt.attempts - now.pf.attempts, now.lt.n_cols, now.lt.why, now.lt.D[0],
+          now.pf.stood, now.pf.attempts, now.pf.cols_total, now.pf.n_cols, now.pf.why);
   for (int l = 0; l < B; ++l)
     fprintf(stderr, " %d.%d%s%s%s", now.lane[l].point, now.lane[l].iter, now.lane[l].done ? "d" : "", now.lane[l].zsup ? "w" : "",
             l < SLM_MAX_LANES && now.mg.lane[l].active ? "m" : "");
@@ -1084,6 +1097,50 @@
   return SLM_OK;
 }
 
+static int pf_bind(slm_dataset* ds, const WsArgs& wa, int B, const int* done, PfArgs* out) {
+  const int64_t n = ds->n;
+  int64_t rows = (n + 127) / 128;
+  rows = std::max<int64_t>(32, (rows + 31) / 32 * 32);
+  const int yb = (int)((n + rows - 1) / rows);
+  if (!ds->pf_list) SLM_TRY(dalloc(&ds->pf_list, (size_t)PF_LIST));
+  if (!ds->pf_part) SLM_TRY(dalloc(&ds->pf_part, (size_t)128 * PF_LIST * SLM_MAX_LANES));
+  if (!ds->lt_stamp) {
+    SLM_TRY(dalloc(&ds->lt_stamp, (size_t)ds->ld));
+    HIP_TRY(hipMemsetAsync(ds->lt_stamp, 0, sizeof(int32_t) * (size_t)ds->ld, ds->eng->stream));
+  }
+  PfArgs a;
+  memset(&a, 0, sizeof(a));
+  a.lt = &ds->dctl->lt; a.pf = &ds->dctl->pf; a.ctl = ds->ctl; a.done = done; a.pts = ds->pts;
+  a.ws = wa.ws; a.idx = wa.idx; a.pos = wa.pos; a.XT = ds->XT; a.R = ds->R; a.r_plane = (int64_t)n * SPLIT_RSTRIDE;
+  a.colnorm = ds->colnorm; a.a0 = ds->a0; a.b0 = ds->b0; a.g = ds->g; a.gprev = ds->gprev;
+  a.list = ds->pf_list; a.stamp = ds->lt_stamp; a.part = ds->pf_part;
+  a.n = n; a.ld = ds->ld; a.p = (int)ds->p; a.n_lanes = B; a.slots = SPLIT_LANES * ((B + SPLIT_LANES - 1) / SPLIT_LANES);
+  a.yb = yb; a.rows = (int)rows;
+  a.inv_n = 1.0 / (double)ds->n_global;
+  *out = a;
+  return SLM_OK;
+}
+
+int PathCall::pass_f32_solve() {
+  slm_host::PassF32Facts f;
+  f.pass_f64 = kn.pass_f64; f.min_rows = kn.pass_f32_min_rows; f.n = n;
+  f.shared_path = shared_path; f.use_ws = use_ws; f.ws_late = ws_late; f.cov_on = cov_on; f.sharded = sharded; f.split = split;
+  f.row_weights = any_rw || ds->rw != nullptr; f.custom_scale = custom_scale; f.singleton = ds->singleton != 0;
+  f.xt_ready = ds->XT != nullptr && ds->XT_ready; f.colnorm_ready = ds->colnorm != nullptr && ds->colnorm_ready;
+  if (!slm_host::pass_f32_eligible(f) || B > kMaxLanes || !(expected > 0)) return SLM_OK;
+  bool usable = false;
+  SLM_TRY(ensure_x32s(ds, n, &usable));
+  if (!usable) return SLM_OK;
+  if (!ds->R) {
+    SLM_TRY(dalloc(&ds->R, (size_t)ds->n * SPLIT_RSTRIDE * SPLIT_HALVES));
+    HIP_TRY(hipMemsetAsync(ds->R, 0, sizeof(double) * (size_t)ds->n * SPLIT_RSTRIDE * SPLIT_HALVES, s));
+  }
+  f32_plan.certify = true;
+  SLM_TRY(pf_bind(ds, wa, B, done_flag, &f32_plan.pa));
+  f32_solve = true;
+  return SLM_OK;
+}
+
 int PathCall::queue_chunk() {
   const int this_chunk = mg_on ? 1 : (expected <= 0 ? chunk : (enq < expected ? (int)std::min<int64_t>(64, expected - enq) : 1));
   for (int i = 0; i < this_chunk; ++i) {
@@ -1103,8 +1160,14 @@
     }
     if (light) SLM_TRY(enqueue_light_attempt());
     light_skip = light ? &ds->dctl->lt.ok : nullptr;
-    ta.light = light ? 1 : 0;
     const bool sample_pass = n_sample > 0 && enq == 0;
+    const bool f32 = f32_solve && !light && !mg_on && enq > 0;
+    if (f32 && !light_begun) {
+      HIP_TRY(hipMemsetAsync(ds->lt_stamp, 0, sizeof(int32_t) * (size_t)ld, s));
+      light_begun = true;
+    }
+    ta.light = (light || f32) ? 1 : 0;
+    last_f32 = f32;
     if (sample_pass) {
       LaneSetup part = ls;
       for (int l = 0; l < kMaxLanes; ++l) part.n_eff[l] = (double)ds->n_global * (double)n_sample / (double)n;
@@ -1115,7 +1178,7 @@
       first.provisional = 1;
       launch_tail(first, s);
     } else {
-      if (!(carry && enq == 0)) SLM_TRY(enqueue_pass_gradient(e0, e1));
+      if (!(carry && enq == 0)) SLM_TRY(enqueue_pass_gradient(e0, e1, f32));
       enqueue_tail();
     }
     fix_start = sample_pass;
@@ -1208,6 +1271,9 @@
   HIP_TRY(hipStreamSynchronize(s));
   tr[3] = t_mark();
   const DevCtl& snap = ds->hctl[final_slot].c;
+  if (trace3)
+    fprintf(stderr, "[slm] end: f32 %d of %d (borderline %d, last %d, why %d, reasons %#x)\n", snap.pf.stood, snap.pf.attempts, snap.pf.cols_total,
+            snap.pf.n_cols, snap.pf.why, snap.pf.why_seen);
   if (sharded && snap.g.diverged)
     return fail(SLM_ERR_COMM, "row-sharded solve aborted: the ranks' solver states differ (different arguments on "
                 "different ranks, or an all-reduce that is not bit-identical on every rank)");
@@ -1414,9 +1480,11 @@
                                      int32_t* n_sets_out, double* gram_out, double* xw_out, double* xty_out, char* kernels_out,
                                      int32_t kernels_len) {
   if (!ds || !o || !o->Z || !o->cols || !o->k_end || !G_out) return fail(SLM_ERR_BAD_ARG, "NULL argument");
-  const int route = o->route, B = o->n_lanes, nb = o->n_builds;
+  const int route = o->route == 3 ? 1 : o->route, B = o->n_lanes, nb = o->n_builds;
   const bool gather_x = (o->flags & SLM_WSL_GATHER_X) != 0, xty = (o->flags & SLM_WSL_XTY) != 0;
-  if (route != 1 && route != 2) return fail(SLM_ERR_BAD_ARG, "route must be 1 (split pass) or 2 (covariance), got %d", route);
+  if (o->route < 1 || o->route > 3)
+    return fail(SLM_ERR_BAD_ARG, "route must be 1 (split pass), 2 (covariance) or 3 (split pass, X^T R on the fp32 image), got %d", o->route);
+  const bool image = o->route == 3;
   if (B < 1 || B > kMaxLanes) return fail(SLM_ERR_BAD_ARG, "between 1 and %d lanes, got %d", kMaxLanes, B);
   if (o->flags & ~(SLM_WSL_GATHER_X | SLM_WSL_XTY)) return fail(SLM_ERR_BAD_ARG, "unknown flags %#x", o->flags);
   if (xty != (xty_out != nullptr)) return fail(SLM_ERR_BAD_ARG, "xty_out goes with SLM_WSL_XTY");
@@ -1589,7 +1657,34 @@
   HIP_TRY(hipMemsetAsync(ds->z, 0, sizeof(double) * (size_t)slots * ld, s));
   HIP_TRY(hipMemcpy2DAsync(ds->z, sizeof(double) * ld, o->Z, sizeof(double) * p, sizeof(double) * p, B, hipMemcpyHostToDevice, s));
   GradNames gn;
-  if (route == 1) {
+  bool on_image = false;
+  if (image && !kn.pass_f64) {
+    if (o->row_weights || o->n_eff) return fail(SLM_ERR_UNSUPPORTED, "route 3: the dataset's own unweighted rows only");
+    if (!(ds->XT && ds->XT_ready)) return fail(SLM_ERR_UNSUPPORTED, "route 3: no column-major copy of X");
+    SLM_TRY(ensure_x32s(ds, n, &on_image));
+    if (!on_image) return fail(SLM_ERR_UNSUPPORTED, "route 3: the dataset has no fp32 image (no memory, or entries a float cannot hold)");
+  }
+  if (route == 1 && on_image) {
+    PassF32Plan plain;
+    SLM_TRY(enqueue_gradient_split(kn, ds, ls, ds->y, nullptr, ds->ctl, &wa, nullptr, nullptr, 0, false, nullptr, &gn, &plain));
+    PfArgs pa;
+    SLM_TRY(pf_bind(ds, wa, B, &ds->gctl->done, &pa));
+    pa.patch = 1;
+    std::unique_ptr<DevCtl> hd(new DevCtl);
+    memset(hd.get(), 0, sizeof(DevCtl));
+    hd->lt.attempts = hd->lt.id = 1;
+    for (int l = 0; l < SLM_MAX_LANES; ++l) hd->lt.epoch[l] = 1;
+    hd->pf.attempts = hd->pf.stood = hd->pf.id_R = 1;
+    hd->pf.builds_seen = -1;
+    HIP_TRY(hipMemcpyAsync(&ds->dctl->lt, &hd->lt, sizeof(LightCtl), hipMemcpyHostToDevice, s));
+    HIP_TRY(hipMemcpyAsync(&ds->dctl->pf, &hd->pf, sizeof(PassF32Ctl), hipMemcpyHostToDevice, s));
+    h->k_new = 0;
+    HIP_TRY(hipMemcpyAsync(ds->ws_ctl, h, sizeof(WsCtl), hipMemcpyHostToDevice, s));
+    hipLaunchKernelGGL(pf_new_kernel, dim3(1), dim3(1024), 0, s, pa);
+    launch_pf_exact(pa, s);
+    SLM_TRY(check_launch());
+    HIP_TRY(hipStreamSynchronize(s));
+  } else if (route == 1) {
     SLM_TRY(enqueue_gradient_split(kn, ds, ls, ds->y, nullptr, ds->ctl, &wa, nullptr, nullptr, 0, false, nullptr, &gn));
   } else {
     if (!ds->cov_Z) SLM_TRY(dalloc(&ds->cov_Z, (size_t)ld * SPLIT_RSTRIDE * SPLIT_HALVES));
diff --git a/sparse-lm_amd/csrc/engine_solve.hip b/sparse-lm_amd/csrc/engine_solve.hip
--- a/sparse-lm_amd/csrc/engine_solve.hip
+++ b/sparse-lm_amd/csrc/engine_solve.hip
@@ -69,6 +69,32 @@
   }
   if (name) *name = nm;
   return yb;
+}
+
+int launch_xtr_f32(const slm_host::Knobs& kn, int cus, SplitArgs& a, const float* X32, int64_t ld32, hipStream_t s, const char** name) {
+  double per_cu = kn.xtr_wgs_per_cu;
+  const bool wide = a.lane_slots > SPLIT_LANES;
+  if (wide) per_cu = 1.0;
+  const slm_host::XtrGrid g = slm_host::xtr_grid(a.n, a.ld, XTR_CB, (int64_t)(xtr_max_row_blocks(cus, a.ld) * per_cu / 2.0));
+  a.xrows = g.rows;
+  PassF32Args pa;
+  pa.s = a; pa.X32 = X32; pa.ld32 = ld32;
+  const dim3 grid(g.xb, g.yb), block(XTR_WAVES * 64);
+  const int extra = wide ? a.n_lanes - SPLIT_LANES : 0;
+  const char* nm;
+  if (wide && extra >= 1 && extra <= 2) { hipLaunchKernelGGL(xtr18_f32_mfma_kernel, grid, block, 0, s, pa); nm = "xtr18_f32_mfma_kernel"; }
+  else if (wide && extra >= 3 && extra <= 4) { hipLaunchKernelGGL(xtr20_f32_mfma_kernel, grid, block, 0, s, pa); nm = "xtr20_f32_mfma_kernel"; }
+  else if (wide) { hipLaunchKernelGGL(xtr32_f32_mfma_kernel, grid, block, 0, s, pa); nm = "xtr32_f32_mfma_kernel"; }
+  else { hipLaunchKernelGGL(xtr_f32_mfma_kernel, grid, block, 0, s, pa); nm = "xtr_f32_mfma_kernel"; }
+  if (name) *name = nm;
+  return g.yb;
+}
+
+void launch_pf_exact(const PfArgs& pa, hipStream_t s) {
+  const dim3 grid(PF_LIST / (16 * PF_WAVES), (unsigned)pa.yb);
+  if (pa.slots > SPLIT_LANES) hipLaunchKernelGGL(pf_exact32_kernel, grid, dim3(PF_WAVES * 64), 0, s, pa);
+  else hipLaunchKernelGGL(pf_exact_kernel, grid, dim3(PF_WAVES * 64), 0, s, pa);
+  hipLaunchKernelGGL(pf_apply_kernel, dim3((unsigned)(PF_LIST * pa.slots / 256)), dim3(256), 0, s, pa);
 }
 
 static int launch_cov_gz(int cus, SplitArgs& a, hipStream_t s, const CovBatch& cb, int n_sets, GradNames* names) {
@@ -202,7 +228,7 @@
 
 int enqueue_gradient_split(const slm_host::Knobs& kn, slm_dataset* ds, const LaneSetup& ls, const double* y, const int* done,
                            const PathCtl* ctl, const WsArgs* wa, hipEvent_t ev_start,
-                           hipEvent_t ev_stop, int64_t n_rows, bool unit_bracket, const int* skip, GradNames* names) {
+                           hipEvent_t ev_stop, int64_t n_rows, bool unit_bracket, const int* skip, GradNames* names, const PassF32Plan* f32) {
   hipStream_t s = ds->eng->stream;
   const SplitKernel* sk = ds->sk;
   const int nblk = ds->split_nblk;
@@ -232,18 +258,12 @@
     else { hipLaunchKernelGGL(resid_mfma_kernel, dim3(nblk, halves), dim3(RM_WAVES * 64), 0, s, a); nm = "resid_mfma_kernel"; }
     if (names) names->ws_resid = nm;
   }
-  if (ev_start && !unit) HIP_TRY(hipEventRecord(ev_start, s));
-  const int xblk = launch_xtr(kn, ds->eng->cus, a, s, n_rows > 0 && ctl != nullptr,
-                              names ? &names->product : nullptr);
-  if (ev_stop) HIP_TRY(hipEventRecord(ev_stop, s));
   ReduceArgs ra;
   ra.partial = ds->partial;
   ra.loss_partial = ds->loss_partial;
   ra.g = ds->g;
   ra.done = done;
-  ra.nblk = xblk;
   ra.nblk_loss = nblk;
-  ra.skip = skip;
   ra.n_lanes = a.lane_slots;
   ra.ld = ds->ld;
   for (int l = 0; l < kMaxLanes; ++l) {
@@ -251,7 +271,29 @@
     ra.scale[l] = 1.0 / ne;
     ra.loss_scale[l] = 0.5 / ne;
   }
-  hipLaunchKernelGGL(reduce_partials_kernel, dim3((unsigned)(ds->ld / 16 + 1), ls.B), dim3(256), 0, s, ra);
+  const dim3 rgrid((unsigned)(ds->ld / 16 + 1), ls.B);
+  if (f32) {
+    if (f32->certify) hipLaunchKernelGGL(pf_prepare_kernel, dim3(1), dim3(1024), 0, s, f32->pa);
+    SplitArgs a32 = a;
+    a32.skip = f32->certify ? &f32->pa.pf->off : nullptr;
+    if (ev_start && !unit) HIP_TRY(hipEventRecord(ev_start, s));
+    ra.nblk = launch_xtr_f32(kn, ds->eng->cus, a32, ds->X32s, ds->ld32, s, names ? &names->product : nullptr);
+    if (ev_stop) HIP_TRY(hipEventRecord(ev_stop, s));
+    ra.skip = a32.skip;
+    hipLaunchKernelGGL(reduce_partials_kernel, rgrid, dim3(256), 0, s, ra);
+    if (!f32->certify) return SLM_OK;
+    hipLaunchKernelGGL(pf_select_kernel, dim3(1), dim3(1024), 0, s, f32->pa);
+    launch_pf_exact(f32->pa, s);
+    a.skip = &f32->pa.lt->ok;
+    ev_start = ev_stop = nullptr;
+  }
+  if (ev_start && !unit) HIP_TRY(hipEventRecord(ev_start, s));
+  const int xblk = launch_xtr(kn, ds->eng->cus, a, s, n_rows > 0 && ctl != nullptr,
+                              names && !f32 ? &names->product : nullptr);
+  if (ev_stop) HIP_TRY(hipEventRecord(ev_stop, s));
+  ra.nblk = xblk;
+  ra.skip = a.skip;
+  hipLaunchKernelGGL(reduce_partials_kernel, rgrid, dim3(256), 0, s, ra);
   if (row_sharded(ds))
     SLM_TRY(all_reduce_sum(ds->eng, ds->g, (size_t)ls.B * (size_t)(ds->ld + 16)));
   return SLM_OK;
@@ -567,7 +609,8 @@
                                   const double* n_eff, const int32_t* cov_index, int64_t n_rows, double* G_out, double* loss_out,
                                   char* kernels_out, int32_t kernels_len) {
   if (!ds || !Z || !G_out) return fail(SLM_ERR_BAD_ARG, "NULL argument");
-  if (route < 0 || route > 2) return fail(SLM_ERR_BAD_ARG, "route must be 0 (fused), 1 (split pass) or 2 (covariance), got %d", route);
+  if (route < 0 || route > 3)
+    return fail(SLM_ERR_BAD_ARG, "route must be 0 (fused), 1 (split pass), 2 (covariance) or 3 (split pass, X^T R on the fp32 image), got %d", route);
   if (n_lanes < 1 || n_lanes > kMaxLanes) return fail(SLM_ERR_BAD_ARG, "between 1 and %d lanes, got %d", kMaxLanes, n_lanes);
   if (n_rows < 0 || n_rows > ds->n) return fail(SLM_ERR_BAD_ARG, "n_rows = %lld outside [0, %lld]", (long long)n_rows, (long long)ds->n);
   if (row_sharded(ds)) return fail(SLM_ERR_UNSUPPORTED, "slm_gradient_lanes: row-sharded datasets");
@@ -595,11 +638,19 @@
   HIP_TRY(hipSetDevice(ds->eng->device));
   hipStream_t s = ds->eng->stream;
   if (route == 0 && !ds->gk[B - 1]) return fail(SLM_ERR_UNSUPPORTED, "route 0: no %d-lane kernel covers p = %lld", B, (long long)p);
-  if (route == 1) {
-    if (!ds->sk) return fail(SLM_ERR_UNSUPPORTED, "route 1: no split pass for p = %lld", (long long)p);
+  if (route == 1 || route == 3) {
+    if (!ds->sk) return fail(SLM_ERR_UNSUPPORTED, "route %d: no split pass for p = %lld", route, (long long)p);
     SLM_TRY(ensure_xt(kn, ds));
     if (!split_usable(kn, ds) || (B > SPLIT_LANES && !(ds->XT && ds->XT_ready)))
-      return fail(SLM_ERR_UNSUPPORTED, "route 1: no residual kernel for %d lanes at p = %lld without the column-major copy", B, (long long)p);
+      return fail(SLM_ERR_UNSUPPORTED, "route %d: no residual kernel for %d lanes at p = %lld without the column-major copy", route, B, (long long)p);
+  }
+  bool on_image = false;
+  if (route == 3) {
+    if (n_rows > 0) return fail(SLM_ERR_UNSUPPORTED, "route 3 reads all rows: no n_rows");
+    if (!kn.pass_f64) {
+      SLM_TRY(ensure_x32s(ds, n, &on_image));
+      if (!on_image) return fail(SLM_ERR_UNSUPPORTED, "route 3: the dataset has no fp32 image (no memory, or entries a float cannot hold)");
+    }
   }
   const int slots = route == 0 ? B : SPLIT_LANES * ((B + SPLIT_LANES - 1) / SPLIT_LANES);
   HIP_TRY(hipMemsetAsync(ds->z, 0, sizeof(double) * (size_t)slots * ld, s));
@@ -616,8 +667,10 @@
   GradNames names;
   if (route == 0) {
     SLM_TRY(enqueue_gradient(ds, ls, ds->y, nullptr, nullptr, nullptr, n_rows, nullptr, &names));
-  } else if (route == 1) {
-    SLM_TRY(enqueue_gradient_split(kn, ds, ls, ds->y, nullptr, nullptr, nullptr, nullptr, nullptr, n_rows, false, nullptr, &names));
+  } else if (route == 1 || route == 3) {
+    PassF32Plan plain;
+    SLM_TRY(enqueue_gradient_split(kn, ds, ls, ds->y, nullptr, nullptr, nullptr, nullptr, nullptr, n_rows, false, nullptr, &names,
+                                   on_image ? &plain : nullptr));
   } else {
     if (!ds->cov_Z) SLM_TRY(dalloc(&ds->cov_Z, (size_t)ld * SPLIT_RSTRIDE * SPLIT_HALVES));
     SLM_TRY(enqueue_gradient_cov(ds, B, cov_index, nullptr, nullptr, nullptr, nullptr, nullptr, &names));
@@ -780,7 +833,7 @@
     const dim3 grid((unsigned)row_tiles, (unsigned)((ld + 31) / 32));
     hipLaunchKernelGGL(tile_columns_kernel, grid, dim3(256), 0, s, (const double*)ds->X, n, ld, ds->XT);
   }
-  if (ds->XT && ds->XT_ready && !ds->colnorm_ready && !ds->rw && !row_sharded(ds) && kn.light_pass) {
+  if (ds->XT && ds->XT_ready && !ds->colnorm_ready && !ds->rw && !row_sharded(ds) && (kn.light_pass || !kn.pass_f64)) {
     if (!ds->colnorm && pool_malloc((void**)&ds->colnorm, sizeof(double) * (size_t)ld) != hipSuccess) {
       (void)hipGetLastError();
       ds->colnorm = nullptr;
diff --git a/sparse-lm_amd/csrc/host_logic.hpp b/sparse-lm_amd/csrc/host_logic.hpp
--- a/sparse-lm_amd/csrc/host_logic.hpp
+++ b/sparse-lm_amd/csrc/host_logic.hpp
@@ -194,6 +194,23 @@
   g.rows = std::max<int64_t>(kSampleMinRows, (n_s + want - 1) / want);
   g.yb = (int)((n_s + g.rows - 1) / g.rows);
   return g;
+}
+
+constexpr int64_t kPassF32MaxRows = (int64_t)1 << 24;
+struct PassF32Facts {
+  bool pass_f64;
+  int64_t min_rows;
+  int64_t n;
+  bool shared_path, use_ws, ws_late, cov_on, sharded, split;
+  bool row_weights, custom_scale;
+  bool singleton;
+  bool xt_ready, colnorm_ready;
+};
+inline bool pass_f32_eligible(const PassF32Facts& f) {
+  if (f.pass_f64 || f.n < f.min_rows || f.n > kPassF32MaxRows) return false;
+  if (!f.shared_path || !f.use_ws || f.ws_late || f.cov_on || f.sharded || !f.split) return false;
+  if (f.row_weights || f.custom_scale || !f.singleton) return false;
+  return f.xt_ready && f.colnorm_ready;
 }
 
 template <typename Entry>
@@ -258,6 +275,8 @@
   int64_t sample_min_rows = 65536;
   int sample_div = 4;
   bool sample_f64 = false;
+  bool pass_f64 = false;
+  int64_t pass_f32_min_rows = 65536;
   int mg = -1;
   bool handover = true;
   bool light_pass = true;
@@ -315,6 +334,8 @@
     if (const char* e = text("SLM_SAMPLE_START_MIN_ROWS")) k.sample_min_rows = std::max<int64_t>(64, atoll(e));
     as_int("SLM_SAMPLE_DIV", 1, 64, &k.sample_div);
     k.sample_f64 = first("SLM_SAMPLE_F64") == '1';
+    k.pass_f64 = first("SLM_PASS_F64") == '1';
+    if (const char* e = text("SLM_PASS_F32_MIN_ROWS")) k.pass_f32_min_rows = std::max<int64_t>(64, atoll(e));
     if (const char c = first("SLM_MG")) k.mg = c == '0' ? 0 : (c == '2' ? 2 : -1);
     k.handover = !is_set("SLM_NO_HANDOVER");
     k.light_pass = !is_set("SLM_NO_LIGHT_PASS");
diff --git a/sparse-lm_amd/csrc/light_ctl.hpp b/sparse-lm_amd/csrc/light_ctl.hpp
--- a/sparse-lm_amd/csrc/light_ctl.hpp
+++ b/sparse-lm_amd/csrc/light_ctl.hpp
@@ -25,4 +25,17 @@
   double slack[SLM_MAX_LANES];
 };
 
+struct PassF32Ctl {
+  int32_t off;
+  int32_t attempts;
+  int32_t stood;
+  int32_t cols_total;
+  int32_t n_cols;
+  int32_t n_list;
+  int32_t why;
+  int32_t id_R;
+  int32_t builds_seen;
+  int32_t why_seen;
+};
+
 }
diff --git a/sparse-lm_amd/csrc/pass_f32_kernels.hpp b/sparse-lm_amd/csrc/pass_f32_kernels.hpp
--- /dev/null
+++ b/sparse-lm_amd/csrc/pass_f32_kernels.hpp
@@ -0,0 +1,447 @@
+#pragma once
+#include <hip/hip_runtime.h>
+#include <stdint.h>
+
+#include "light_ctl.hpp"
+#include "split_kernels.hpp"
+#include "tail_kernels.hpp"
+#include "ws_kernels.hpp"
+
+namespace slm {
+
+struct PassF32Args {
+  SplitArgs s;
+  const float* X32;
+  int64_t ld32;
+};
+
+typedef float slm_f4 __attribute__((ext_vector_type(4)));
+constexpr int XTF_U = 4;
+
+template <int H, int E = 0>
+__device__ __forceinline__ void xtr_f32_body(const PassF32Args& pa) {
+  static_assert(SPLIT_RSTRIDE == 16 && SPLIT_LANES <= 16, "a row of a plane of R is the 16-wide B operand");
+  static_assert(H == 1 || H == 2, "one or two planes of R");
+  static_assert(E == 0 || (H == 1 && (E == 2 || E == 4)), "extras: pairs of slots of plane 1 beside the sixteen of plane 0");
+  constexpr int E2 = E > 0 ? E / 2 : 1;
+  const SplitArgs& a = pa.s;
+  if (split_off(a)) return;
+  const int lane = threadIdx.x & 63;
+  const int wave = __builtin_amdgcn_readfirstlane((int)threadIdx.x >> 6);
+  int bx = (int)blockIdx.x, by = (int)blockIdx.y;
+  {
+    const int total = (int)(gridDim.x * gridDim.y), lin = bx + (int)gridDim.x * by;
+    const int xcd = lin & 7, slot = lin >> 3, base = total >> 3, rem = total & 7;
+    const int m = xcd * base + (xcd < rem ? xcd : rem) + slot;
+    bx = m % (int)gridDim.x;
+    by = m / (int)gridDim.x;
+  }
+  const int col0 = (bx * XTR_WAVES + wave) * XTR_CW;
+  const int ld = (int)a.ld, ld32 = (int)pa.ld32;
+  if (col0 >= ld) return;
+  const int64_t r0 = (int64_t)by * a.xrows;
+  const int64_t r1 = r0 + a.xrows < a.n ? r0 + a.xrows : a.n;
+  const int kq = lane >> 4, i16 = lane & 15;
+  int coff[2];
+#pragma unroll
+  for (int c = 0; c < 2; ++c) {
+    const int col = col0 + 64 * c + 4 * i16;
+    coff[c] = col < ld32 - 4 ? col : ld32 - 4;
+  }
+  slm_d4 acc[H][8];
+#pragma unroll
+  for (int h = 0; h < H; ++h)
+#pragma unroll
+    for (int t = 0; t < 8; ++t) acc[h][t] = slm_d4{0.0, 0.0, 0.0, 0.0};
+  const int nb = (int)((r1 - r0) / (4 * XTF_U));
+  const float* xp = pa.X32 + (r0 + kq) * pa.ld32;
+  const double* rp = a.R + (r0 + kq) * SPLIT_RSTRIDE + i16;
+  const double* rp1 = a.R + a.r_plane + (r0 + kq) * SPLIT_RSTRIDE;
+  slm_f4 xa[XTF_U][2], xb[XTF_U][2];
+  double ra[H][XTF_U], rb[H][XTF_U];
+  d2 ea[E2][XTF_U], eb[E2][XTF_U];
+  double ex[2 * E2][8];
+#pragma unroll
+  for (int e = 0; e < 2 * E2; ++e)
+#pragma unroll
+    for (int c = 0; c < 8; ++c) ex[e][c] = 0.0;
+  auto load = [&](slm_f4(&xv)[XTF_U][2], double(&rv)[H][XTF_U], d2(&ev)[E2][XTF_U], int b) {
+    const float* xq = xp + (int64_t)b * (4 * XTF_U) * pa.ld32;
+    const double* rq = rp + (int64_t)b * (4 * XTF_U) * SPLIT_RSTRIDE;
+#pragma unroll
+    for (int u = 0; u < XTF_U; ++u) {
+#pragma unroll
+      for (int c = 0; c < 2; ++c) {
+        const slm_f4* src = reinterpret_cast<const slm_f4*>(xq + (int64_t)u * 4 * pa.ld32 + coff[c]);
+        xv[u][c] = SLM_NT_LOADS ? __builtin_nontemporal_load(src) : *src;
+      }
+#pragma unroll
+      for (int h = 0; h < H; ++h) rv[h][u] = rq[(int64_t)h * a.r_plane + u * 4 * SPLIT_RSTRIDE];
+      if constexpr (E > 0) {
+        const d2* eq = reinterpret_cast<const d2*>(rp1 + ((int64_t)b * (4 * XTF_U) + u * 4) * SPLIT_RSTRIDE);
+#pragma unroll
+        for (int q = 0; q < E2; ++q) ev[q][u] = eq[q];
+      }
+    }
+  };
+  auto step = [&](const slm_f4(&x)[2], const double(&rv)[H], const d2(&ev)[E2]) {
+#pragma unroll
+    for (int c = 0; c < 2; ++c) {
+      const double xd[4] = {(double)x[c][0], (double)x[c][1], (double)x[c][2], (double)x[c][3]};
+#pragma unroll
+      for (int e = 0; e < 4; ++e) {
+#pragma unroll
+        for (int h = 0; h < H; ++h) acc[h][4 * c + e] = __builtin_amdgcn_mfma_f64_16x16x4f64(xd[e], rv[h], acc[h][4 * c + e], 0, 0, 0);
+        if constexpr (E > 0) {
+#pragma unroll
+          for (int q = 0; q < E2; ++q) {
+            ex[2 * q][4 * c + e] = __builtin_fma(xd[e], ev[q].x, ex[2 * q][4 * c + e]);
+            ex[2 * q + 1][4 * c + e] = __builtin_fma(xd[e], ev[q].y, ex[2 * q + 1][4 * c + e]);
+          }
+        }
+      }
+    }
+  };
+  auto compute = [&](const slm_f4(&xv)[XTF_U][2], const double(&rv)[H][XTF_U], const d2(&ev)[E2][XTF_U]) {
+#pragma unroll
+    for (int u = 0; u < XTF_U; ++u) {
+      double ru[H];
+      d2 eu[E2];
+#pragma unroll
+      for (int h = 0; h < H; ++h) ru[h] = rv[h][u];
+#pragma unroll
+      for (int q = 0; q < E2; ++q) eu[q] = ev[q][u];
+      step(xv[u], ru, eu);
+    }
+  };
+  if (nb > 0) {
+    load(xa, ra, ea, 0);
+    const int pairs = (nb - 1) >> 1;
+    for (int k = 0; k < pairs; ++k) {
+      load(xb, rb, eb, 2 * k + 1);
+      compute(xa, ra, ea);
+      load(xa, ra, ea, 2 * k + 2);
+      compute(xb, rb, eb);
+    }
+    if ((nb - 1) & 1) {
+      load(xb, rb, eb, nb - 1);
+      compute(xa, ra, ea);
+      compute(xb, rb, eb);
+    } else {
+      compute(xa, ra, ea);
+    }
+  }
+  for (int64_t row = r0 + (int64_t)nb * (4 * XTF_U); row < r1; row += 4) {
+    const bool ok = row + kq < r1;
+    const int64_t rr = ok ? row + kq : r1 - 1;
+    double rv[H];
+#pragma unroll
+    for (int h = 0; h < H; ++h) rv[h] = ok ? a.R[(int64_t)h * a.r_plane + rr * SPLIT_RSTRIDE + i16] : 0.0;
+    slm_f4 x[2];
+#pragma unroll
+    for (int c = 0; c < 2; ++c) x[c] = *reinterpret_cast<const slm_f4*>(pa.X32 + rr * pa.ld32 + coff[c]);
+    d2 eu[E2];
+#pragma unroll
+    for (int q = 0; q < E2; ++q) eu[q] = d2{0.0, 0.0};
+    if constexpr (E > 0) {
+#pragma unroll
+      for (int q = 0; q < E2; ++q)
+        if (ok) eu[q] = reinterpret_cast<const d2*>(a.R + a.r_plane + rr * SPLIT_RSTRIDE)[q];
+    }
+    step(x, rv, eu);
+  }
+  constexpr int SLOTS = E > 0 ? 2 * SPLIT_LANES : SPLIT_LANES * H;
+  if constexpr (E > 0) {
+#pragma unroll
+    for (int e = 0; e < E; ++e) {
+      double* out = a.partial + ((int64_t)by * SLOTS + SPLIT_LANES + e) * a.ld;
+#pragma unroll
+      for (int c = 0; c < 2; ++c) {
+        double v[4];
+#pragma unroll
+        for (int k = 0; k < 4; ++k) {
+          v[k] = ex[e][4 * c + k];
+          v[k] += __shfl_xor(v[k], 16, 64);
+          v[k] += __shfl_xor(v[k], 32, 64);
+        }
+        const int col = col0 + 64 * c + 4 * i16;
+        if (kq == 0 && col < ld) {
+          const bool in = col < ld32;
+          *reinterpret_cast<d2*>(out + col) = in ? d2{v[0], v[1]} : d2{0.0, 0.0};
+          *reinterpret_cast<d2*>(out + col + 2) = in ? d2{v[2], v[3]} : d2{0.0, 0.0};
+        }
+      }
+    }
+  }
+#pragma unroll
+  for (int h = 0; h < H; ++h) {
+    double* out = a.partial + ((int64_t)by * SLOTS + SPLIT_LANES * h + i16) * a.ld;
+#pragma unroll
+    for (int c = 0; c < 2; ++c)
+#pragma unroll
+      for (int r = 0; r < 4; ++r) {
+        const int col = col0 + 64 * c + 4 * (kq + 4 * r);
+        if (col < ld) {
+          const bool in = col < ld32;
+          *reinterpret_cast<d2*>(out + col) = in ? d2{acc[h][4 * c][r], acc[h][4 * c + 1][r]} : d2{0.0, 0.0};
+          *reinterpret_cast<d2*>(out + col + 2) = in ? d2{acc[h][4 * c + 2][r], acc[h][4 * c + 3][r]} : d2{0.0, 0.0};
+        }
+      }
+  }
+}
+
+static __global__ __launch_bounds__(XTR_WAVES * 64, 2) void xtr_f32_mfma_kernel(PassF32Args a) { xtr_f32_body<1>(a); }
+static __global__ __launch_bounds__(XTR_WAVES * 64, 1) void xtr18_f32_mfma_kernel(PassF32Args a) { xtr_f32_body<1, 2>(a); }
+static __global__ __launch_bounds__(XTR_WAVES * 64, 1) void xtr20_f32_mfma_kernel(PassF32Args a) { xtr_f32_body<1, 4>(a); }
+static __global__ __launch_bounds__(XTR_WAVES * 64, 1) void xtr32_f32_mfma_kernel(PassF32Args a) { xtr_f32_body<2>(a); }
+
+constexpr int PF_CAP = 256;
+constexpr int PF_LIST = WS_KCAP + PF_CAP;
+constexpr int PF_WAVES = 4;
+static_assert(PF_LIST % (16 * PF_WAVES) == 0, "pf_exact_kernel's grid covers the list in whole workgroups");
+
+struct PfArgs {
+  LightCtl* lt;
+  PassF32Ctl* pf;
+  const PathCtl* ctl;
+  const int* done;
+  const slm_path_point* pts;
+  const WsCtl* ws;
+  const int32_t* idx;
+  const int32_t* pos;
+  const double* XT;
+  const double* R;
+  int64_t r_plane;
+  const double* colnorm;
+  const double *a0, *b0;
+  double* g;
+  double* gprev;
+  int32_t* list;
+  int32_t* stamp;
+  double* part;
+  int64_t n, ld;
+  int p, n_lanes, slots, yb, rows;
+  double inv_n;
+  int patch;
+};
+
+static __global__ __launch_bounds__(1024) void pf_prepare_kernel(PfArgs a) {
+  __shared__ double red[1][TAIL_WAVES];
+  __shared__ int live_s[SLM_MAX_LANES];
+  LightCtl* lt = a.lt;
+  PassF32Ctl* pf = a.pf;
+  const int tid = threadIdx.x;
+  if (*a.done != 0) {
+    if (tid == 0) {
+      lt->ok = 0;
+      pf->off = 1;
+      pf->id_R = 0;
+    }
+    return;
+  }
+  if (tid < SLM_MAX_LANES) live_s[tid] = (tid < a.n_lanes && !a.ctl[tid].done && !a.ctl[tid].idle) ? 1 : 0;
+  __syncthreads();
+  int n_live = 0, why = 0;
+  for (int l = 0; l < a.n_lanes; ++l) n_live += live_s[l];
+  if (n_live == 0) why = 1;
+  if (!(a.ws->valid && !a.ws->building && !a.ws->disabled)) why = 2;
+  for (int l = 0; l < a.n_lanes && why == 0; ++l)
+    if (live_s[l] && (!a.ctl[l].zsup || a.ctl[l].mode != 1)) why = 2;
+  if (why == 0) {
+    const int K = a.ws->K;
+    double bad[1] = {0.0};
+    for (int l = 0; l < a.n_lanes; ++l) {
+      if (!live_s[l] || lt->epoch[l] == 0) continue;
+      for (int k = tid; k < K; k += 1024) {
+        const int j = a.idx[k];
+        if (j >= 0 && a.stamp[j] != lt->epoch[l]) bad[0] += 1.0;
+      }
+    }
+    block_sum<1>(bad, red);
+    if (bad[0] != 0.0) why = 4;
+  }
+  if (tid == 0) {
+    lt->attempts += 1;
+    lt->id = lt->attempts;
+    lt->why = why;
+    lt->ok = why == 0 ? 1 : 0;
+    lt->n_cols = 0;
+    lt->n_live = 0;
+    pf->attempts += 1;
+    pf->off = why == 0 ? 0 : 1;
+    pf->why = why;
+    if (why != 0) pf->why_seen |= 1 << why;
+    pf->n_cols = 0;
+    pf->n_list = 0;
+    pf->id_R = 0;
+  }
+}
+
+static __global__ __launch_bounds__(1024) void pf_select_kernel(PfArgs a) {
+  LightCtl* lt = a.lt;
+  PassF32Ctl* pf = a.pf;
+  if (pf->off) return;
+  __shared__ double slack_s[SLM_MAX_LANES], sa_s[SLM_MAX_LANES], sb_s[SLM_MAX_LANES];
+  __shared__ int lane_s[SLM_MAX_LANES];
+  __shared__ int n_live_s;
+  __shared__ int wave_tot[TAIL_WAVES];
+  const int tid = threadIdx.x;
+  if (tid == 0) {
+    int s = 0;
+    for (int l = 0; l < a.n_lanes && l < SLM_MAX_LANES; ++l) {
+      const PathCtl* c = a.ctl + l;
+      if (c->done || c->idle) continue;
+      const slm_path_point pt = a.pts[c->pt_off + c->point];
+      const double loss = a.g[(int64_t)l * (a.ld + 16) + a.ld];
+      lane_s[s] = l;
+      sa_s[s] = pt.sa;
+      sb_s[s] = pt.sb;
+      slack_s[s] = 0x1p-24 * (1.0 + 0x1p-4) * sqrt(2.0 * loss);
+      ++s;
+    }
+    n_live_s = s;
+  }
+  __syncthreads();
+  const int n_live = n_live_s;
+  const int K = a.ws->K;
+  int wj = -1;
+  if (tid < K) wj = a.idx[tid];
+  int n_w = 0;
+  const int w_at = block_excl_scan(wj >= 0 ? 1 : 0, wave_tot, &n_w);
+  if (wj >= 0) a.list[w_at] = wj;
+  __syncthreads();
+  const int per = (a.p + 1023) / 1024;
+  const int j0 = tid * per, j1 = min(j0 + per, a.p);
+  unsigned long long pick = 0ull;
+  int mine = 0;
+  for (int j = j0; j < j1; ++j) {
+    if (a.pos[j] >= 0) continue;
+    const double cj = a.colnorm[j] * (1.0 + 1e-9) + 1e-300;
+    bool near = false;
+    for (int sl = 0; sl < n_live; ++sl) {
+      const int l = lane_s[sl];
+      const int64_t o = (int64_t)l * a.ld + j;
+      const double thr = sa_s[sl] * a.a0[o] + sb_s[sl] * a.b0[o];
+      near = near || !(fabs(a.g[(int64_t)l * (a.ld + 16) + j]) + cj * slack_s[sl] < thr * (1.0 - 1e-12));
+    }
+    if (near) {
+      pick |= 1ull << (j - j0);
+      mine += 1;
+    }
+  }
+  int total = 0;
+  int at = n_w + block_excl_scan(mine, wave_tot, &total);
+  const bool fits = total <= PF_CAP;
+  if (fits)
+    for (int j = j0; j < j1; ++j)
+      if ((pick >> (j - j0)) & 1ull) a.list[at++] = j;
+  if (tid == 0) {
+    if (fits) {
+      pf->n_cols = total;
+      pf->n_list = n_w + total;
+      pf->stood += 1;
+      pf->cols_total += total;
+      pf->id_R = lt->id;
+      pf->builds_seen = a.ws->builds + a.ws->appends;
+      lt->n_cols = total;
+      for (int sl = 0; sl < n_live; ++sl) {
+        lt->pend_slack[lane_s[sl]] = slack_s[sl];
+        lt->pend_epoch[lane_s[sl]] = lt->id;
+      }
+    } else {
+      lt->ok = 0;
+      lt->why = 3;
+      pf->off = 1;
+      pf->why = 3;
+      pf->why_seen |= 1 << 3;
+      pf->n_cols = total;
+    }
+  }
+}
+
+static __global__ __launch_bounds__(1024) void pf_new_kernel(PfArgs a) {
+  PassF32Ctl* pf = a.pf;
+  __shared__ int wave_tot[TAIL_WAVES];
+  const int tid = threadIdx.x;
+  const int built = a.ws->builds + a.ws->appends;
+  const bool on = *a.done == 0 && pf->id_R != 0 && built != pf->builds_seen && a.ws->valid;
+  int wj = -1;
+  if (on && tid >= a.ws->k_new && tid < a.ws->K) wj = a.idx[tid];
+  int total = 0;
+  const int at = block_excl_scan(wj >= 0 ? 1 : 0, wave_tot, &total);
+  if (wj >= 0) a.list[at] = wj;
+  if (tid == 0) {
+    pf->n_list = on ? total : 0;
+    if (on) pf->builds_seen = built;
+  }
+}
+
+template <int P>
+__device__ __forceinline__ void pf_exact_body(const PfArgs& a) {
+  const PassF32Ctl* pf = a.pf;
+  if (*a.done != 0) return;
+  if (a.patch ? pf->n_list == 0 : pf->off != 0) return;
+  const int n_list = pf->n_list;
+  const int lane = threadIdx.x & 63;
+  const int wave = __builtin_amdgcn_readfirstlane((int)threadIdx.x >> 6);
+  const int group = (int)blockIdx.x * PF_WAVES + wave;
+  if (16 * group >= n_list) return;
+  const int i16 = lane & 15, q = lane >> 4;
+  const int c = 16 * group + i16;
+  const int64_t j = a.list[c < n_list ? c : n_list - 1];
+  const int64_t r0 = (int64_t)blockIdx.y * a.rows;
+  const int64_t r1 = r0 + a.rows < a.n ? r0 + a.rows : a.n;
+  slm_d4 acc[P];
+#pragma unroll
+  for (int h = 0; h < P; ++h) acc[h] = slm_d4{0.0, 0.0, 0.0, 0.0};
+  const int64_t t1 = (r1 + 31) >> 5;
+#pragma unroll 2
+  for (int64_t t = r0 >> 5; t < t1; ++t) {
+    const d2* xp = reinterpret_cast<const d2*>(a.XT + (((t * a.ld + j) << 5) + 8 * q));
+    d2 x[4];
+#pragma unroll
+    for (int u = 0; u < 4; ++u) x[u] = xp[u];
+    double r[P][8];
+    const int64_t row = (t << 5) + 8 * q;
+#pragma unroll
+    for (int s = 0; s < 8; ++s)
+#pragma unroll
+      for (int h = 0; h < P; ++h) r[h][s] = row + s < r1 ? a.R[(int64_t)h * a.r_plane + (row + s) * SPLIT_RSTRIDE + i16] : 0.0;
+#pragma unroll
+    for (int s = 0; s < 8; ++s)
+#pragma unroll
+      for (int h = 0; h < P; ++h) acc[h] = __builtin_amdgcn_mfma_f64_16x16x4f64(s & 1 ? x[s >> 1].y : x[s >> 1].x, r[h][s], acc[h], 0, 0, 0);
+  }
+#pragma unroll
+  for (int h = 0; h < P; ++h)
+#pragma unroll
+    for (int r = 0; r < 4; ++r) {
+      const int cc = 16 * group + q + 4 * r;
+      if (cc < n_list) a.part[((int64_t)blockIdx.y * PF_LIST + cc) * a.slots + SPLIT_LANES * h + i16] = acc[h][r];
+    }
+}
+static __global__ __launch_bounds__(PF_WAVES * 64) void pf_exact_kernel(PfArgs a) { pf_exact_body<1>(a); }
+static __global__ __launch_bounds__(PF_WAVES * 64) void pf_exact32_kernel(PfArgs a) { pf_exact_body<2>(a); }
+
+static __global__ __launch_bounds__(256) void pf_apply_kernel(PfArgs a) {
+  const PassF32Ctl* pf = a.pf;
+  if (*a.done != 0) return;
+  if (a.patch ? pf->n_list == 0 : pf->off != 0) return;
+  const int e = (int)blockIdx.x * 256 + (int)threadIdx.x;
+  const int c = e / a.slots, slot = e - c * a.slots;
+  if (c >= pf->n_list || slot >= a.n_lanes) return;
+  const int id = pf->id_R;
+  if (a.patch && a.lt->epoch[slot] != id) {
+    if (slot == 0) a.stamp[a.list[c]] = id;
+    return;
+  }
+  double s4[4] = {0.0, 0.0, 0.0, 0.0};
+  for (int b = 0; b < a.yb; ++b) s4[b & 3] += a.part[((int64_t)b * PF_LIST + c) * a.slots + slot];
+  const double v = ((s4[0] + s4[1]) + (s4[2] + s4[3])) * a.inv_n;
+  const int64_t j = a.list[c];
+  a.g[(int64_t)slot * (a.ld + 16) + j] = v;
+  if (a.patch) a.gprev[(int64_t)slot * a.ld + j] = v;
+  if (slot == 0) a.stamp[j] = id;
+}
+
+}
diff --git a/sparse-lm_amd/sparselm_amd/_engine.py b/sparse-lm_amd/sparselm_amd/_engine.py
--- a/sparse-lm_amd/sparselm_amd/_engine.py
+++ b/sparse-lm_amd/sparselm_amd/_engine.py
@@ -779,6 +779,12 @@
                                             _ptr(G), _ptr(loss), names, len(names)))
         return G, loss, names.value.decode()
 
+    def pass_f32_lanes(self, Z):
+        return self.gradient_lanes(Z, route=3)
+
+    def working_set_pass_f32(self, Z, cols, k_end):
+        return self.working_set_lanes(Z, cols, k_end, on_ws=1, route=3)
+
     def working_set_lanes(self, Z, cols, k_end, on_ws=None, row_weights=None, n_eff=None, route: int = 1, cov_index=None,
                           gather_from_x: bool = False, xty: bool = False, want_xw: bool = False):
         import types
```

Result: slower. 15780 (-7.7%).
